# jandrewrfarrell/RUFUS

Hardware: AMD Instinct MI355X
Metric: reads/sec through k-mer count+filter at k=25 (higher is better)
Workload: dtype u64; 1 GPU; synthetic 30x WGS trio (BASELINE configs[2]): genome 3100000000 bp, 620000000/620000000/620000000 x 150 bp reads per sample, on each of 1 GPU(s) 19 resident blocks of the subject (92 GB of packed reads in HBM, generated on the device in 0.5 s), 1000 SNVs, seed 12345, k=25, -s 8G -L 2, MinCov 5, MaxHashDepth 1200, MinQ 15, thresh 1; 2 minimizer-shard pass(es) per step (per-shard (pos,key)-sorted re; parallelism=read-block shard x1, mutant_kmers=24567, pulled_pairs=11560, passes=2, hbm_total=309220868096, hbm_free_at_start=308400881664, resident_read_bytes=92219805240, read_blocks=compact, run_map_budget_bytes=39836680704, checked=False, hbm_mapped_bytes=271656681472

## Files before the change

include/rufus_hip.h:

```cpp
#ifndef RUFUS_HIP_H
#define RUFUS_HIP_H

#include <stddef.h>
#include <stdint.h>

#ifdef __cplusplus
extern "C" {
#endif

#define RFX_OK 0
#define RFX_E_NODEVICE (-1)
#define RFX_E_INVAL (-2)
#define RFX_E_NOMEM (-3)
#define RFX_E_FULL (-4)
#define RFX_E_HIP (-5)
#define RFX_E_MIXEDCASE (-6)
#define RFX_E_RANGE (-7)
#define RFX_E_FORMAT (-8)

#define RFX_HISTO_BINS 10002

typedef struct rfx_ctx rfx_ctx;
typedef struct rfx_reads rfx_reads;
typedef struct rfx_table rfx_table;
// ... 106 lines not shown
#define RFX_COUNT_MSP 3
int rfx_count_set_mode(rfx_table*, int mode);
int rfx_count_set_shard(rfx_table*, int shard, int n_shards);
int rfx_count_set_early(rfx_table*, int on);
int rfx_count_early_segments(const rfx_table*);
int rfx_count_adopt_early(rfx_table* next_shard, rfx_table* from);
typedef struct rfx_runmaps rfx_runmaps;
rfx_runmaps* rfx_runmaps_create(rfx_ctx*, uint64_t budget_bytes);
rfx_runmaps* rfx_runmaps_create_pooled(rfx_ctx*, uint64_t pool_bytes);
void rfx_runmaps_free(rfx_runmaps*);
uint64_t rfx_runmaps_bytes(const rfx_runmaps*);
int rfx_runmaps_blocks(const rfx_runmaps*);
int rfx_runmaps_drop(rfx_runmaps*, const rfx_reads*);
int rfx_runmaps_clear(rfx_runmaps*);
int rfx_count_set_runmaps(rfx_table*, rfx_runmaps*);
int rfx_count_prepare_maps(rfx_table*, rfx_reads* const* blocks, int n);
int rfx_count_prefetch_maps(rfx_table*, rfx_reads* const* blocks, int n);
uint64_t rfx_count_replayed(const rfx_table*);
int rfx_count_set_passes(rfx_table*, int passes);
int rfx_count_add(rfx_table*, const rfx_reads*);
typedef struct rfx_peers rfx_peers;
int rfx_ctx_allow_peers(rfx_ctx*, const int* devices, int n);
rfx_peers* rfx_peers_create(int n);
void rfx_peers_free(rfx_peers*);
int rfx_count_set_peers(rfx_table*, rfx_peers*, int index);
int rfx_count_add_pairs_dev(rfx_table*, const uint64_t* d_keys, const uint32_t* d_counts, uint64_t n);
int rfx_count_stats(rfx_table*, uint64_t* distinct, uint64_t* capacity, uint64_t* max_displacement);

int rfx_count_segments(rfx_table*);
int rfx_count_segment_get(rfx_table*, int i, const uint64_t** d_records, const uint64_t** d_bin_start, uint32_t* bins,
                          uint64_t* n_records);
int rfx_count_add_records_dev(rfx_table*, const uint64_t* d_records, uint64_t n_records, const uint64_t* d_bin_start,
                              uint32_t bins);
int rfx_count_adopt_records_dev(rfx_table*, const uint64_t* d_records, const uint32_t* d_ext, uint64_t n_records,
                                const uint64_t* d_bin_start, uint32_t bins);
int rfx_count_segment_ext(rfx_table*, int i, const uint32_t** d_ext);
int rfx_count_add_records_ext_dev(rfx_table*, const uint64_t* d_records, const uint32_t* d_ext, uint64_t n_records,
                                  const uint64_t* d_bin_start, uint32_t bins);
void rfx_count_free(rfx_table*);

rfx_records* rfx_count_finish(rfx_table*, uint64_t lower, uint64_t upper, uint64_t* histo );
typedef struct rfx_finish rfx_finish;
rfx_finish* rfx_count_finish_begin(rfx_table*, uint64_t lower, uint64_t upper, uint64_t* histo );
rfx_records* rfx_count_finish_end(rfx_finish*);

uint64_t rfx_records_size(const rfx_records*);
int rfx_records_k(const rfx_records*);
int rfx_records_lsize(const rfx_records*);
int rfx_records_payload(const rfx_records*, void* out, size_t cap_bytes, int counter_len);
int rfx_records_payload_range(const rfx_records*, uint64_t first, uint64_t n, void* out, size_t cap_bytes,
                              int counter_len);
int rfx_records_get(const rfx_records*, uint64_t* keys, uint32_t* counts, uint64_t* pos);
rfx_records* rfx_records_load(rfx_ctx*, int k, int lsize, const uint64_t* cols, const void* payload, uint64_t n,
                              int counter_len);
rfx_records* rfx_records_load_fd(rfx_ctx*, int k, int lsize, const uint64_t* cols, int fd, uint64_t offset, uint64_t n,
                                 int counter_len);
rfx_records* rfx_records_from_dev(rfx_ctx*, int k, int lsize, const uint64_t* cols, const uint64_t* d_keys,
                                  const uint32_t* d_counts, uint64_t n);
const uint64_t* rfx_records_dev_keys(const rfx_records*);
const uint32_t* rfx_records_dev_counts(const rfx_records*);
const uint64_t* rfx_records_dev_pos(const rfx_records*);
int rfx_records_histo(const rfx_records*, uint64_t* histo );
int rfx_records_verify(const rfx_records*, uint32_t min_count, uint32_t max_count, uint64_t out[4]);
int rfx_records_checksum(const rfx_records*, uint64_t out[2]);
void rfx_records_free(rfx_records*);

int rfx_merge_unique(rfx_ctx*, const rfx_records* const* files, int n_files, uint32_t min_count, uint64_t* keys_out,
                     uint32_t* counts_out, uint64_t cap, uint64_t* n_out);
int rfx_query(const rfx_records* db, const uint64_t* keys, uint64_t n, uint32_t* counts_out);
int rfx_unique_to_subject(rfx_ctx*, const rfx_records* subject, const rfx_records* const* others, int n_others,
                          uint32_t min_count, uint32_t min_cov, uint32_t max_cov, uint64_t* keys_out,
                          uint32_t* counts_out, uint64_t cap, uint64_t* n_out);
rfx_records* rfx_records_subtract(rfx_ctx*, const rfx_records* a, const rfx_records* const* others, int n_others,
                                  uint32_t min_count, uint32_t max_count);

typedef struct rfx_binned rfx_binned;
typedef struct rfx_candidates rfx_candidates;
rfx_binned* rfx_count_finish_binned(rfx_table*, uint64_t lower, uint64_t upper, uint64_t* histo );
uint64_t rfx_binned_size(const rfx_binned*);
int rfx_binned_bits(const rfx_binned*);
void rfx_binned_free(rfx_binned*);
rfx_candidates* rfx_binned_strike(rfx_ctx*, rfx_binned* subject, const rfx_binned* control, uint32_t min_count,
                                  uint32_t max_count);
int rfx_candidates_strike(rfx_candidates*, const rfx_binned* control);
uint64_t rfx_candidates_size(const rfx_candidates*);
int rfx_candidates_get(const rfx_candidates*, uint64_t* keys_out);
int rfx_candidates_get_counts(const rfx_candidates*, uint32_t* counts_out);
int rfx_candidates_strike_records(rfx_candidates*, const rfx_records* exclude);
void rfx_candidates_free(rfx_candidates*);
int rfx_binned_get(const rfx_binned*, uint64_t* keys_out, uint32_t* counts_out, uint32_t* bins_out, uint64_t* at_out,
                   uint64_t cap, uint64_t* n_out);
int rfx_binned_checksum(const rfx_binned*, uint64_t out[2]);
int rfx_binned_verify(const rfx_binned*, uint64_t lower, uint64_t upper, uint64_t out[5]);
int rfx_binned_query(const rfx_binned*, const uint64_t* canonical_keys, uint64_t n, uint32_t* counts_out);
const uint64_t* rfx_binned_dev_keys(const rfx_binned*);
const uint32_t* rfx_binned_dev_counts(const rfx_binned*);

rfx_set* rfx_set_build(rfx_ctx*, const uint64_t* fwd_keys, uint64_t n, int k);
uint64_t rfx_set_size(const rfx_set*);
void rfx_set_free(rfx_set*);
int rfx_filter(rfx_set*, const rfx_reads*, int thresh, int last_base_skipped, uint32_t* hits_out,
               uint64_t* hitmask_out, uint64_t* n_hit_reads);
int rfx_filter_many(rfx_set*, const rfx_reads* const* blocks, int n, int thresh, int last_base_skipped,
                    uint64_t* const* hitmask_out, uint64_t* n_hit_reads);

#define RFX_SELECT_READS 0
#define RFX_SELECT_PAIRS 1
rfx_reads* rfx_reads_select(rfx_ctx*, const rfx_reads* src, const uint64_t* hitmask , int mode);
int rfx_reads_origin(const rfx_reads*, uint32_t* block_out, uint32_t* read_out);
rfx_reads* rfx_filter_pull(rfx_set*, const rfx_reads* const* blocks, int n, int thresh, int last_base_skipped, int mode,
                           uint64_t* const* hitmask_out, uint64_t* n_hit_reads);

typedef struct rfx_model_params {
  double sc, stdev, factor, skew, power;
} rfx_model_params;
int rfx_model_residuals(rfx_ctx*, const int64_t* histo, uint32_t n, const rfx_model_params* cand, int n_cand,
                        int log_resid, int inflection, int max_copy, double* resid_out);
int rfx_model_tables(rfx_ctx*, uint32_t n, const rfx_model_params* model, uint32_t* n_cols, double* dist,
                     size_t dist_cap, double* rowtot);

#define RFX_OVL_SAM 0
#define RFX_OVL_CONTIG 1
#define RFX_OVL_REGION 2
int rfx_overlap_score(rfx_ctx*, const char* a, int alen, const char* const* b, const int* blen, int nb, float min_pct,
                      int min_ovl, int variant, int* out );
typedef struct rfx_ovl_pool rfx_ovl_pool;
rfx_ovl_pool* rfx_ovl_pool_create(rfx_ctx*, const char* const* seqs, const int* lens, int n);
int rfx_ovl_pool_set(rfx_ovl_pool*, int idx, const char* seq, int len);
int rfx_ovl_pool_score(rfx_ovl_pool*, int query, const char* a_explicit, int a_len, const int* cand, int nb,
                       float min_pct, int min_ovl, int variant, int strands, int* out);
void rfx_ovl_pool_free(rfx_ovl_pool*);
int rfx_annotate(rfx_set*, const rfx_reads*, uint32_t* cov_out);

#ifdef __cplusplus
}
#endif
#endif
```

profiles/summarize_pmc.py:

```python
#!/usr/bin/env python3
import collections
import csv
import json
import re
import sys


NOT_CHAIN = frozenset((
    "k_synth_reads", "k_copy16",
    "k_flag_absent", "k_flag_absent_tiled", "k_fa_bounds", "k_flag_gather", "k_flag_range", "k_flag_rank", "k_flag_present",
    "k_compact_count", "k_compact_scatter", "k_scan_u64", "k_query", "k_strike_bins", "k_strike_cands",
    "k_strike_query", "k_binned_sizes", "k_binned_scan", "k_binned_gather", "k_binned_checksum", "k_binned_verify", "k_binned_query",
    "k_filter", "k_filter_q", "k_filter_p", "k_filter_fast", "k_filter_big", "k_hits_mask", "k_mask_count", "k_set_bitmap",
    "k_set_bitmap_big", "k_set_bitmap_q", "k_set_bitmap_p",
    "k_set_insert", "k_set_bitmap_packed", "k_records_checksum", "k_records_verify", "k_check_sorted",
    "k_parse_records", "k_format_records", "k_txt_count", "k_txt_lines", "k_txt_reads", "k_txt_pack", "k_txt_nth", "k_bgzf_inflate", "k_reads_tile_count", "k_reads_tile_table", "k_reads_tile", "k_select_words", "k_select_table", "k_select_copy", "k_gather_sizes", "k_gather_table", "k_gather_copy", "k_compute_pos", "k_annotate", "k_overlap_pool", "k_overlap_score",
    "k_model_colsum", "k_model_dist", "k_model_rowtot", "k_model_sum", "k_model_terms", "k_model_weights",
))
CHAIN_KNOWN = frozenset((
    "k_msp_part1", "k_msp_replay", "k_msp_count", "k_col_sums", "k_bin_group_sums", "k_bin_offsets", "k_scan_tail", "k_scan_sums",
    "k_scan_apply", "k_part2", "k_flag_if_gt", "k_slice_tag", "k_bin_hist", "k_bin_hist_stamp", "k_bin_hist_multi", "k_msp_leaf",
    "k_surv_place", "k_surv_hist", "k_surv_sort", "k_histo_bins", "k_histo_staged", "k_bin_count", "k_part1", "k_leaf", "k_leaf_compact", "k_bin_scatter",
    "k_tmp_start", "k_split_bins", "k_coarse_counts", "k_histo", "k_count_reads", "k_count_pairs", "k_table_pairs", "k_tile_count",
    "k_tile_scan", "k_tile_emit",
))


def kname(s):
    m = re.search(r"(k_[a-z0-9_]+|__amd_rocclr_[A-Za-z]+)", s)
    return m.group(1) if m else s[:40]


def load(path, counter):
    agg = collections.defaultdict(lambda: [0, 0.0])
    for r in csv.DictReader(open(path)):
        if r["Counter_Name"] == counter:
            a = agg[kname(r["Kernel_Name"])]
            a[0] += 1
            a[1] += float(r["Counter_Value"])
    return {k: (n, v / n) for k, (n, v) in agg.items()}


def main():
    f, w = load(sys.argv[1], "FETCH_SIZE"), load(sys.argv[2], "WRITE_SIZE")
    out = {}
    for k in sorted(set(f) | set(w)):
        fn, fv = f.get(k, (0, 0.0))
        wn, wv = w.get(k, (0, 0.0))
        out[k] = {"launches": max(fn, wn), "FETCH_SIZE_KB_avg": round(fv, 1), "WRITE_SIZE_KB_avg": round(wv, 1),
                  "hbm_bytes_per_launch": int((2 * fv + wv) * 1024)}
    chain = [k for k in sorted(out) if k.startswith("k_") and k not in NOT_CHAIN]
    samples = int(sys.argv[4]) if len(sys.argv) > 4 else max(
        out.get("k_msp_part1", {}).get("launches", 0), out.get("k_part1", {}).get("launches", 0),
        out.get("k_bin_scatter", {}).get("launches", 0))
    if samples:
        tot = sum(out[k]["hbm_bytes_per_launch"] * out[k]["launches"] for k in chain if k in out)
        out["_chain"] = {"kernels": [k for k in chain if k in out], "samples": samples,
                         "hbm_bytes_per_sample": int(tot / samples),
                         "source": "rocprofv3 --pmc FETCH_SIZE / WRITE_SIZE (separate passes), (2*FETCH+WRITE)*1024, all "
                                   "launches of the count chain of the profiled bench command / sample chains"}
        if len(sys.argv) > 5:
            out["genome"] = int(sys.argv[5])
    import os
    sys.path.insert(0, os.path.dirname(os.path.dirname(os.path.abspath(__file__))))
    import bench
    out["kernel_sources_sha16"] = bench.kernel_source_fingerprint()
    out["commit"] = os.environ.get("RFX_COMMIT", "unknown (set RFX_COMMIT=$(git rev-parse HEAD) when profiling)")
    json.dump(out, open(sys.argv[3], "w"), indent=1, sort_keys=True)
    if "_chain" in out:
        print(f"count chain: {out['_chain']['hbm_bytes_per_sample'] / 1e6:.1f} MB per sample over {samples} samples")
    for k, v in sorted(((k, v) for k, v in out.items() if isinstance(v, dict) and "launches" in v), key=lambda kv: -kv[1]["hbm_bytes_per_launch"]):
        print(f"{k:26s} {v['launches']:4d} {v['FETCH_SIZE_KB_avg']:14.1f} {v['WRITE_SIZE_KB_avg']:14.1f} "
              f"{v['hbm_bytes_per_launch'] / 1e6:10.1f} MB")


if __name__ == "__main__":
    main()
```

rufus_amd/capi.py:

```python
from __future__ import annotations

import ctypes as C
import os
import sys

import numpy as np

_HERE = os.path.dirname(os.path.abspath(__file__))
LIB_PATH = os.environ.get("RFX_LIB") or os.path.join(_HERE, "librufus_hip.so")

HISTO_BINS = 10002
PACK_COUNT, PACK_FILTER = 1, 2
COUNT_AUTO, COUNT_TABLE, COUNT_P2L, COUNT_MSP = 0, 1, 2, 3
E_FULL, E_RANGE, E_MIXEDCASE = -4, -7, -6
E_INVAL, E_FORMAT = -2, -8
SELECT_READS, SELECT_PAIRS = 0, 1

u8p, u32p, u64p = C.POINTER(C.c_uint8), C.POINTER(C.c_uint32), C.POINTER(C.c_uint64)

SIGNATURES = {
    "rfx_version": (C.c_char_p, []),
    "rfx_strerror": (C.c_char_p, [C.c_int]),
    "rfx_last_error": (C.c_char_p, []),
    "rfx_jf_matrix": (C.c_int, [C.c_int, C.c_int, u64p]),
    "rfx_jf_pos": (C.c_uint64, [u64p, C.c_int, C.c_int, C.c_uint64]),
    "rfx_pack_words": (C.c_uint64, [u64p, C.c_uint32]),
    "rfx_pack_reads": (C.c_int, [C.c_char_p, C.c_char_p, u64p, C.c_uint32, C.c_int, C.c_int, u64p, u32p, u32p, u32p,
                                 u32p]),
    "rfx_pack_spans": (C.c_int, [C.c_void_p, u64p, u32p, u64p, C.c_uint32, C.c_int, C.c_int, u64p, u32p, u32p, u32p, u32p]),
    "rfx_hashlist_keys": (C.c_long, [C.c_char_p, C.c_size_t, C.c_int, C.c_int, u64p, C.c_size_t]),
    "rfx_jhash_header": (C.c_long, [C.c_int, C.c_int, u64p, C.c_int, C.c_int, C.c_int, C.POINTER(C.c_char_p),
                                    C.c_char_p, C.c_size_t]),
    "rfx_open": (C.c_void_p, [C.c_int, C.c_size_t]),
    "rfx_close": (None, [C.c_void_p]),
    "rfx_sync": (C.c_int, [C.c_void_p]),
    "rfx_host_alloc": (C.c_void_p, [C.c_size_t]),
    "rfx_host_alloc_lazy": (C.c_void_p, [C.c_size_t]),
    "rfx_host_pin": (C.c_int, [C.c_void_p]),
    "rfx_host_cpus": (C.c_uint, []),
    "rfx_host_free": (None, [C.c_void_p]),
    "rfx_stream": (C.c_void_p, [C.c_void_p]),
    "rfx_mem_stats": (C.c_int, [C.c_void_p, u64p, u64p, u64p]),
    "rfx_memcpy_dev": (C.c_int, [C.c_void_p, C.c_void_p, C.c_void_p, C.c_size_t]),
    "rfx_prof_enable": (C.c_int, [C.c_void_p, C.c_int]),
    "rfx_prof_filter": (C.c_int, [C.c_void_p, C.c_char_p]),
    "rfx_prof_reset": (C.c_int, [C.c_void_p]),
    "rfx_prof_query": (C.c_int, [C.c_void_p, C.c_char_p, C.POINTER(C.c_double), u64p]),
    "rfx_prof_names": (C.c_int, [C.c_void_p, C.c_char_p, C.c_size_t]),
    "rfx_reads_device_bytes": (C.c_uint64, [C.c_void_p]),
    "rfx_records_subtract": (C.c_void_p, [C.c_void_p, C.c_void_p, C.POINTER(C.c_void_p), C.c_int, C.c_uint32, C.c_uint32]),
    "rfx_count_finish_binned": (C.c_void_p, [C.c_void_p, C.c_uint64, C.c_uint64, u64p]),
    "rfx_binned_size": (C.c_uint64, [C.c_void_p]),
    "rfx_binned_bits": (C.c_int, [C.c_void_p]),
    "rfx_binned_free": (None, [C.c_void_p]),
    "rfx_binned_strike": (C.c_void_p, [C.c_void_p, C.c_void_p, C.c_void_p, C.c_uint32, C.c_uint32]),
    "rfx_candidates_strike": (C.c_int, [C.c_void_p, C.c_void_p]),
    "rfx_candidates_size": (C.c_uint64, [C.c_void_p]),
    "rfx_candidates_get": (C.c_int, [C.c_void_p, u64p]),
    "rfx_candidates_free": (None, [C.c_void_p]),
    "rfx_candidates_get_counts": (C.c_int, [C.c_void_p, u32p]),
    "rfx_candidates_strike_records": (C.c_int, [C.c_void_p, C.c_void_p]),
    "rfx_binned_get": (C.c_int, [C.c_void_p, u64p, u32p, u32p, u64p, C.c_uint64, u64p]),
    "rfx_binned_checksum": (C.c_int, [C.c_void_p, u64p]),
    "rfx_binned_verify": (C.c_int, [C.c_void_p, C.c_uint64, C.c_uint64, u64p]),
    "rfx_binned_query": (C.c_int, [C.c_void_p, u64p, C.c_uint64, u32p]),
    "rfx_binned_dev_keys": (C.c_void_p, [C.c_void_p]),
    "rfx_binned_dev_counts": (C.c_void_p, [C.c_void_p]),
    "rfx_reads_upload": (C.c_void_p, [C.c_void_p, u64p, u32p, u32p, u32p, u32p, C.c_uint32]),
    "rfx_reads_free": (None, [C.c_void_p]),
    "rfx_reads_count": (C.c_uint32, [C.c_void_p]),
    "rfx_reads_bases": (C.c_uint64, [C.c_void_p]),
    "rfx_reads_words": (C.c_uint64, [C.c_void_p]),
    "rfx_reads_get": (C.c_int, [C.c_void_p, u64p, u32p, u32p, u32p, u32p]),
    "rfx_tile_plan": (C.c_int, [C.c_uint64, C.c_int, C.c_uint32, u64p, u32p]),
    "rfx_reads_tile": (C.c_void_p, [C.c_void_p, C.c_void_p, C.c_int, C.c_uint32]),
    "rfx_reads_select": (C.c_void_p, [C.c_void_p, C.c_void_p, u64p, C.c_int]),
    "rfx_reads_origin": (C.c_int, [C.c_void_p, u32p, u32p]),
    "rfx_filter_pull": (C.c_void_p, [C.c_void_p, C.POINTER(C.c_void_p), C.c_int, C.c_int, C.c_int, C.c_int, C.POINTER(u64p), u64p]),
    "rfx_synth_reads": (C.c_void_p, [C.c_void_p, C.c_void_p, C.c_uint64, C.c_uint32, C.c_int, C.c_int]),
    "rfx_text_open": (C.c_void_p, [C.c_void_p, C.c_uint64]),
    "rfx_text_close": (None, [C.c_void_p]),
    "rfx_text_room": (C.c_uint64, [C.c_void_p]),
    "rfx_text_bytes": (C.c_uint64, [C.c_void_p]),
    "rfx_text_append": (C.c_long, [C.c_void_p, C.c_char_p, C.c_uint64]),
    "rfx_text_copied": (C.c_int, [C.c_void_p, C.c_long]),
    "rfx_text_wait": (C.c_int, [C.c_void_p, C.c_long]),
    "rfx_text_parse": (C.c_void_p, [C.c_void_p, C.c_int, C.c_int, C.POINTER(C.c_int)]),
    "rfx_text_fetch": (C.c_int, [C.c_void_p, C.c_char_p]),
    "rfx_text_reset": (None, [C.c_void_p]),
    "rfx_bgzf_scan": (C.c_int, [C.c_char_p, C.c_uint64, C.c_uint32, u32p, u64p, u64p]),
    "rfx_text_append_bgzf": (C.c_long, [C.c_void_p, C.c_char_p, C.c_uint64]),
    "rfx_text_settle": (C.c_int, [C.c_void_p, C.c_void_p, u64p]),
    "rfx_text_records": (C.c_int, [C.c_void_p, u64p]),
    "rfx_text_settle_records": (C.c_int, [C.c_void_p, C.c_void_p, C.c_uint64, u64p, u64p]),
    "rfx_text_gather": (C.c_int, [C.c_void_p, u64p, C.c_uint64, C.c_void_p, C.c_uint64, u64p, u64p]),
    "rfx_reads_of_length": (C.c_uint64, [C.c_void_p, C.c_uint32]),
    "rfx_synth_text": (C.c_int, [C.c_void_p, C.c_uint64, C.c_uint32, C.c_void_p, C.c_void_p]),
    "rfx_synth_snv": (C.c_int, [C.c_void_p, C.c_uint32, u64p, C.c_char_p, C.c_char_p]),
    "rfx_synth_genome": (C.c_int, [C.c_void_p, C.c_uint64, C.c_uint64, C.c_void_p]),
    "rfx_count_begin": (C.c_void_p, [C.c_void_p, C.c_int, C.c_int, C.c_int, C.c_uint64, C.c_uint64, C.c_uint64]),
    "rfx_count_set_mode": (C.c_int, [C.c_void_p, C.c_int]),
    "rfx_count_set_passes": (C.c_int, [C.c_void_p, C.c_int]),
    "rfx_count_add": (C.c_int, [C.c_void_p, C.c_void_p]),
    "rfx_count_add_pairs_dev": (C.c_int, [C.c_void_p, C.c_void_p, C.c_void_p, C.c_uint64]),
    "rfx_count_stats": (C.c_int, [C.c_void_p, u64p, u64p, u64p]),
    "rfx_count_finish_begin": (C.c_void_p, [C.c_void_p, C.c_uint64, C.c_uint64, u64p]),
    "rfx_count_finish_end": (C.c_void_p, [C.c_void_p]),
    "rfx_count_set_shard": (C.c_int, [C.c_void_p, C.c_int, C.c_int]),
    "rfx_count_set_early": (C.c_int, [C.c_void_p, C.c_int]),
    "rfx_count_early_segments": (C.c_int, [C.c_void_p]),
    "rfx_count_adopt_early": (C.c_int, [C.c_void_p, C.c_void_p]),
    "rfx_mem_reserve": (C.c_int, [C.c_void_p, C.c_uint64]),
    "rfx_runmaps_create": (C.c_void_p, [C.c_void_p, C.c_uint64]),
    "rfx_runmaps_create_pooled": (C.c_void_p, [C.c_void_p, C.c_uint64]),
    "rfx_runmaps_free": (None, [C.c_void_p]),
    "rfx_runmaps_bytes": (C.c_uint64, [C.c_void_p]),
    "rfx_runmaps_blocks": (C.c_int, [C.c_void_p]),
    "rfx_runmaps_drop": (C.c_int, [C.c_void_p, C.c_void_p]),
    "rfx_runmaps_clear": (C.c_int, [C.c_void_p]),
    "rfx_count_set_runmaps": (C.c_int, [C.c_void_p, C.c_void_p]),
    "rfx_count_prepare_maps": (C.c_int, [C.c_void_p, C.POINTER(C.c_void_p), C.c_int]),
    "rfx_count_prefetch_maps": (C.c_int, [C.c_void_p, C.POINTER(C.c_void_p), C.c_int]),
    "rfx_count_replayed": (C.c_uint64, [C.c_void_p]),
    "rfx_count_segments": (C.c_int, [C.c_void_p]),
    "rfx_count_segment_get": (C.c_int, [C.c_void_p, C.c_int, C.POINTER(C.c_void_p), C.POINTER(C.c_void_p),
                                        C.POINTER(C.c_uint32), u64p]),
    "rfx_count_add_records_dev": (C.c_int, [C.c_void_p, C.c_void_p, C.c_uint64, C.c_void_p, C.c_uint32]),
    "rfx_count_segment_ext": (C.c_int, [C.c_void_p, C.c_int, C.POINTER(C.c_void_p)]),
    "rfx_count_add_records_ext_dev": (C.c_int, [C.c_void_p, C.c_void_p, C.c_void_p, C.c_uint64, C.c_void_p, C.c_uint32]),
    "rfx_count_free": (None, [C.c_void_p]),
    "rfx_count_finish": (C.c_void_p, [C.c_void_p, C.c_uint64, C.c_uint64, u64p]),
    "rfx_records_size": (C.c_uint64, [C.c_void_p]),
    "rfx_records_k": (C.c_int, [C.c_void_p]),
    "rfx_records_lsize": (C.c_int, [C.c_void_p]),
    "rfx_records_payload": (C.c_int, [C.c_void_p, C.c_void_p, C.c_size_t, C.c_int]),
    "rfx_records_payload_range": (C.c_int, [C.c_void_p, C.c_uint64, C.c_uint64, C.c_void_p, C.c_size_t, C.c_int]),
    "rfx_records_get": (C.c_int, [C.c_void_p, u64p, u32p, u64p]),
    "rfx_records_load": (C.c_void_p, [C.c_void_p, C.c_int, C.c_int, u64p, C.c_void_p, C.c_uint64, C.c_int]),
# ... 120 lines not shown
                   carrier=1 if which == 0 else 0)

    def text(self, first_pair: int, n_pairs: int):
        seq = np.zeros((2 * n_pairs, self.read_len), dtype=np.uint8)
        qual = np.zeros_like(seq)
        _check(lib().rfx_synth_text(C.byref(self), first_pair, n_pairs, seq.ctypes.data, qual.ctypes.data),
               "rfx_synth_text")
        return seq, qual

    def snvs(self):
        out = []
        for i in range(self.n_snv):
            pos, ref, alt = C.c_uint64(0), C.create_string_buffer(1), C.create_string_buffer(1)
            _check(lib().rfx_synth_snv(C.byref(self), i, C.byref(pos), ref, alt), "rfx_synth_snv")
            out.append((pos.value, ref.raw, alt.raw))
        return out

    def genome(self, first: int, n: int) -> bytes:
        buf = np.zeros(max(n, 1), dtype=np.uint8)
        _check(lib().rfx_synth_genome(C.byref(self), first, n, buf.ctypes.data), "rfx_synth_genome")
        return buf[:n].tobytes()


def tile_plan(length: int, k: int, tile_len: int = 150):
    if length < 0 or not 0 <= tile_len < 2**32:
        raise RufusError(f"rfx_tile_plan: {lib().rfx_strerror(E_INVAL).decode()} (code {E_INVAL})")
    nt, step = C.c_uint64(0), C.c_uint32(0)
    _check(lib().rfx_tile_plan(length, k, tile_len, C.byref(nt), C.byref(step)), "rfx_tile_plan")
    return int(nt.value), int(step.value)


def bgzf_scan(data: bytes, max_blocks: int = 0xFFFFFFFF):
    nb, used, inf = C.c_uint32(0), C.c_uint64(0), C.c_uint64(0)
    _check(lib().rfx_bgzf_scan(data, len(data), max_blocks, C.byref(nb), C.byref(used), C.byref(inf)), "rfx_bgzf_scan")
    return int(nb.value), int(used.value), int(inf.value)


class PackedReads:

    def __init__(self, seq: bytes, off: np.ndarray, qual: bytes | None = None, min_q: int = 0,
                 flags: int = PACK_COUNT):
        off = np.ascontiguousarray(off, dtype=np.uint64)
        n = len(off) - 1
        L = lib()
        nw = int(L.rfx_pack_words(_p(off, u64p), n))
        self.n = n
        self.codes = np.zeros(max(nw, 1), dtype=np.uint64)
        self.acgt = np.zeros(max(nw, 1), dtype=np.uint32) if flags & PACK_COUNT else None
        self.good = np.zeros(max(nw, 1), dtype=np.uint32) if flags & PACK_FILTER else None
        self.word_off = np.zeros(n + 1, dtype=np.uint32)
        self.len = np.zeros(max(n, 1), dtype=np.uint32)
        _check(L.rfx_pack_reads(seq, qual, _p(off, u64p), n, min_q, flags, _p(self.codes, u64p), _p(self.acgt, u32p),
                                _p(self.good, u32p), _p(self.word_off, u32p), _p(self.len, u32p)), "rfx_pack_reads")

    @classmethod
    def from_reads(cls, seqs, quals=None, min_q: int = 0, flags: int = PACK_COUNT):
        lens = np.fromiter((len(s) for s in seqs), dtype=np.uint64, count=len(seqs))
        off = np.zeros(len(seqs) + 1, dtype=np.uint64)
        np.cumsum(lens, out=off[1:])
        q = None
        if quals is not None:
            q = b"".join((qq + b"\0" * (len(s) - len(qq)))[:len(s)] for s, qq in zip(seqs, quals))
        return cls(b"".join(seqs), off, q, min_q, flags)


class Context:
    def __init__(self, device: int = 0, hbm_budget: int = 0):
        self._h = lib().rfx_open(device, hbm_budget)
        if not self._h:
            raise RufusError("rfx_open failed (no CPU fallback): " + lib().rfx_last_error().decode())

    def close(self):
        if self._h:
            self._pin_arr = None
            for p in getattr(self, "_pin_ptrs", ()):
                lib().rfx_host_free(p)
            self._pin_ptrs = []
            lib().rfx_close(self._h)
            self._h = None

    def sync(self):
        _check(lib().rfx_sync(self._h), "rfx_sync")

    def mem_stats(self) -> dict:
        u, pk, m = C.c_uint64(0), C.c_uint64(0), C.c_uint64(0)
        _check(lib().rfx_mem_stats(self._h, C.byref(u), C.byref(pk), C.byref(m)), "rfx_mem_stats")
        return {"used": u.value, "peak": pk.value, "mapped": m.value}

    def memcpy_dev(self, dst: int, src: int, nbytes: int):
        _check(lib().rfx_memcpy_dev(self._h, dst, src, nbytes), "rfx_memcpy_dev")

    def prof(self, on: bool):
        _check(lib().rfx_prof_enable(self._h, int(on)), "rfx_prof_enable")

    def prof_filter(self, names=()):
        _check(lib().rfx_prof_filter(self._h, ",".join(names).encode()), "rfx_prof_filter")

    def prof_reset(self):
        _check(lib().rfx_prof_reset(self._h), "rfx_prof_reset")

    def prof_dict(self) -> dict:
        buf = C.create_string_buffer(8192)
        _check(lib().rfx_prof_names(self._h, buf, len(buf)), "rfx_prof_names")
        out = {}
        for name in buf.value.decode().split("\n"):
            if not name:
                continue
            ms, n = C.c_double(0), C.c_uint64(0)
            _check(lib().rfx_prof_query(self._h, name.encode(), C.byref(ms), C.byref(n)), "rfx_prof_query")
            out[name] = (ms.value, n.value)
        return out

    def upload(self, p: PackedReads) -> "ReadBlock":
        return ReadBlock(self, p)

    def synth_reads(self, sy: Synth, first_pair: int, n_pairs: int, min_q: int = 15, want_good: bool = True,
                    compact: bool = False):
        h = lib().rfx_synth_reads(self._h, C.byref(sy), first_pair, n_pairs, min_q, int(want_good) | (2 if compact else 0))
        if not h:
            raise RufusError("rfx_synth_reads failed: " + lib().rfx_last_error().decode())
        return ReadBlock.from_handle(self, h)

    def pinned_u64(self, n_words: int) -> np.ndarray:
        have = getattr(self, "_pin_arr", None)
        if have is None or len(have) < n_words:
            p = lib().rfx_host_alloc(max(n_words, 1) * 8)
            if not p:
                raise RufusError("rfx_host_alloc failed")
            self._pin_ptrs = getattr(self, "_pin_ptrs", []) + [p]
            self._pin_arr = np.ctypeslib.as_array((C.c_uint64 * max(n_words, 1)).from_address(p))
        return self._pin_arr[:max(n_words, 1)]

    def __enter__(self):
        return self

    def __exit__(self, *a):
        self.close()


class TextArena:

    def __init__(self, ctx: Context, cap_bytes: int):
        self.ctx = ctx
        self._h = lib().rfx_text_open(ctx._h, cap_bytes)
        if not self._h:
            raise RufusError("rfx_text_open failed: " + lib().rfx_last_error().decode())

    def append(self, data: bytes) -> int:
        t = lib().rfx_text_append(self._h, data, len(data))
        if t < 0:
            _check(int(t), "rfx_text_append")
        _check(lib().rfx_text_wait(self._h, t), "rfx_text_wait")
        return int(t)

    def append_bgzf(self, data: bytes) -> int:
        t = lib().rfx_text_append_bgzf(self._h, data, len(data))
        if t < 0:
            _check(int(t), "rfx_text_append_bgzf")
        _check(lib().rfx_text_wait(self._h, t), "rfx_text_wait")
        return int(t)

    def settle(self, next: "TextArena | None" = None) -> int:
        carried = C.c_uint64(0)
        _check(lib().rfx_text_settle(self._h, next._h if next is not None else None, C.byref(carried)), "rfx_text_settle")
        return int(carried.value)

# ... 254 lines not shown
        _check(lib().rfx_count_set_passes(self._h, passes), "rfx_count_set_passes")

    def set_peers(self, peers: int, index: int):
        _check(lib().rfx_count_set_peers(self._h, peers, index), "rfx_count_set_peers")

    def set_shard(self, shard: int, n_shards: int):
        _check(lib().rfx_count_set_shard(self._h, shard, n_shards), "rfx_count_set_shard")

    def set_early(self, on: bool = True):
        _check(lib().rfx_count_set_early(self._h, int(on)), "rfx_count_set_early")

    def early_segments(self) -> int:
        return int(lib().rfx_count_early_segments(self._h))

    def adopt_early(self, other: "CountTable"):
        _check(lib().rfx_count_adopt_early(self._h, other._h), "rfx_count_adopt_early")

    def set_runmaps(self, store: "RunMaps"):
        _check(lib().rfx_count_set_runmaps(self._h, store._h if store is not None else None), "rfx_count_set_runmaps")

    def prepare_maps(self, blocks) -> None:
        arr = (C.c_void_p * max(1, len(blocks)))(*[b._h for b in blocks])
        _check(lib().rfx_count_prepare_maps(self._h, arr, len(blocks)), "rfx_count_prepare_maps")

    def prefetch_maps(self, blocks) -> int:
        arr = (C.c_void_p * max(1, len(blocks)))(*[b._h for b in blocks])
        n = int(lib().rfx_count_prefetch_maps(self._h, arr, len(blocks)))
        if n < 0:
            _check(n, "rfx_count_prefetch_maps")
        return n

    def replayed(self) -> int:
        return int(lib().rfx_count_replayed(self._h))

    def segments(self):
        n = lib().rfx_count_segments(self._h)
        if n < 0:
            _check(n, "rfx_count_segments")
        out = []
        for i in range(n):
            dr, db, bins, nr = C.c_void_p(0), C.c_void_p(0), C.c_uint32(0), C.c_uint64(0)
            _check(lib().rfx_count_segment_get(self._h, i, C.byref(dr), C.byref(db), C.byref(bins), C.byref(nr)),
                   "rfx_count_segment_get")
            out.append((dr.value or 0, db.value or 0, bins.value, nr.value))
        return out

    def n_segments(self) -> int:
        n = lib().rfx_count_segments(self._h)
        if n < 0:
            _check(n, "rfx_count_segments")
        return n

    def segment(self, i: int):
        dr, db, bins, nr = C.c_void_p(0), C.c_void_p(0), C.c_uint32(0), C.c_uint64(0)
        _check(lib().rfx_count_segment_get(self._h, i, C.byref(dr), C.byref(db), C.byref(bins), C.byref(nr)),
               "rfx_count_segment_get")
        return (dr.value or 0, db.value or 0, bins.value, nr.value)

    def add_records_dev(self, d_records: int, n_records: int, d_bin_start: int, bins: int, d_ext: int = 0):
        _check(lib().rfx_count_add_records_ext_dev(self._h, d_records, d_ext or None, n_records, d_bin_start, bins),
               "rfx_count_add_records_dev")

    def adopt_records_dev(self, d_records: int, n_records: int, d_bin_start: int, bins: int, d_ext: int = 0):
        _check(lib().rfx_count_adopt_records_dev(self._h, d_records, d_ext or None, n_records, d_bin_start, bins),
               "rfx_count_adopt_records_dev")

    def segment_ext(self, i: int) -> int:
        p = C.c_void_p(0)
        _check(lib().rfx_count_segment_ext(self._h, i, C.byref(p)), "rfx_count_segment_ext")
        return p.value or 0

    def stats(self):
        d, c, m = C.c_uint64(0), C.c_uint64(0), C.c_uint64(0)
        _check(lib().rfx_count_stats(self._h, C.byref(d), C.byref(c), C.byref(m)), "rfx_count_stats")
        return {"distinct": d.value, "capacity": c.value, "max_displacement": m.value}

    def finish(self, lower: int = 0, upper: int = 2**64 - 1, want_histo: bool = False):
        h = np.zeros(HISTO_BINS, dtype=np.uint64) if want_histo else None
        rec = Records(self.ctx, lib().rfx_count_finish(self._h, lower, upper, _p(h, u64p)))
        return (rec, h) if want_histo else rec

    def finish_binned(self, lower: int = 0, upper: int = 2**64 - 1, want_histo: bool = False):
        h = np.zeros(HISTO_BINS, dtype=np.uint64) if want_histo else None
        b = Binned(self.ctx, lib().rfx_count_finish_binned(self._h, lower, upper, _p(h, u64p)))
        return (b, h) if want_histo else b

    def finish_begin(self, lower: int = 0, upper: int = 2**64 - 1, want_histo: bool = False):
        h = np.zeros(HISTO_BINS, dtype=np.uint64) if want_histo else None
        return (lib().rfx_count_finish_begin(self._h, lower, upper, _p(h, u64p)), h)

    def finish_end(self, handle):
        f, h = handle
        rec = Records(self.ctx, lib().rfx_count_finish_end(f))
        return (rec, h) if h is not None else rec

    def free(self):
        if self._h:
            lib().rfx_count_free(self._h)
            self._h = None


def merge_unique(ctx: Context, files, min_count: int = 5):
    arr = (C.c_void_p * len(files))(*[f._h for f in files])
    n = C.c_uint64(0)
    rc = lib().rfx_merge_unique(ctx._h, arr, len(files), min_count, None, None, 0, C.byref(n))
    if rc not in (0, E_RANGE):
        _check(rc, "rfx_merge_unique")
    keys, counts = np.zeros(max(n.value, 1), np.uint64), np.zeros(max(n.value, 1), np.uint32)
    _check(lib().rfx_merge_unique(ctx._h, arr, len(files), min_count, _p(keys, u64p), _p(counts, u32p), len(keys),
                                  C.byref(n)), "rfx_merge_unique")
    return keys[:n.value], counts[:n.value]


_uniq_buf = {}


def unique_to_subject(ctx: Context, subject: Records, others, min_cov: int, max_cov: int, min_count: int = 5):
    arr = (C.c_void_p * max(1, len(others)))(*[f._h for f in others])
    cap = _uniq_buf.get("cap", 1 << 16)
    while True:
        if _uniq_buf.get("cap") != cap or "k" not in _uniq_buf:
            _uniq_buf.update(cap=cap, k=np.zeros(cap, np.uint64), c=np.zeros(cap, np.uint32))
        keys, counts = _uniq_buf["k"], _uniq_buf["c"]
        n = C.c_uint64(0)
        rc = lib().rfx_unique_to_subject(ctx._h, subject._h, arr, len(others), min_count, min_cov, max_cov,
                                         _p(keys, u64p), _p(counts, u32p), cap, C.byref(n))
        if rc == E_RANGE and n.value > cap:
            cap = int(n.value)
            continue
        _check(rc, "rfx_unique_to_subject")
        return keys[:n.value].copy(), counts[:n.value].copy()


def records_subtract(ctx: Context, a: Records, others, min_count: int = 0, max_count: int = 0xFFFFFFFF) -> Records:
    arr = (C.c_void_p * max(1, len(others)))(*[f._h for f in others])
    return Records(ctx, lib().rfx_records_subtract(ctx._h, a._h, arr, len(others), min_count, max_count))


class Binned:

    def __init__(self, ctx: Context, handle):
        if not handle:
            raise RufusError("binned records: " + lib().rfx_last_error().decode())
        self.ctx, self._h = ctx, handle

    def __len__(self):
        return int(lib().rfx_binned_size(self._h))

    @property
    def bits(self):
        return lib().rfx_binned_bits(self._h)

    def _live(self):
        if not self._h:
            raise RufusError("binned records: freed")
        return self._h

    def get(self):
        h = self._live()
        n = len(self)
        keys, counts = np.zeros(n, np.uint64), np.zeros(n, np.uint32)
        bins, at = np.zeros(n, np.uint32), np.zeros(n, np.uint64)
        got = C.c_uint64(0)
        _check(lib().rfx_binned_get(h, _p(keys, u64p), _p(counts, u32p), _p(bins, u32p), _p(at, u64p), n, C.byref(got)),
               "rfx_binned_get")
        if got.value != n:
            raise RufusError(f"rfx_binned_get: {got.value} survivors in the bins, {n} counted by the finish")
        return keys, counts, bins, at

    def checksum(self) -> tuple:
        o = np.zeros(2, dtype=np.uint64)
        _check(lib().rfx_binned_checksum(self._live(), _p(o, u64p)), "rfx_binned_checksum")
        return int(o[0]), int(o[1])

    def verify(self, lower: int = 0, upper: int = 2**64 - 1) -> dict:
        if not 0 <= lower <= upper < 2**64:
            raise ValueError("verify: 0 <= lower <= upper < 2^64")
        o = np.zeros(5, dtype=np.uint64)
        _check(lib().rfx_binned_verify(self._live(), lower, upper, _p(o, u64p)), "rfx_binned_verify")
        return {"bad_bin": int(o[0]), "bad_count": int(o[1]), "not_canonical": int(o[2]), "duplicate": int(o[3]),
                "sum_counts": int(o[4])}

    def query(self, keys: np.ndarray) -> np.ndarray:
        keys = np.ascontiguousarray(keys, dtype=np.uint64)
        if keys.ndim != 1:
            raise ValueError("query: a flat array of keys")
        out = np.zeros(len(keys), dtype=np.uint32)
        _check(lib().rfx_binned_query(self._live(), _p(keys, u64p), len(keys), _p(out, u32p)), "rfx_binned_query")
        return out

    def dev_ptrs(self):
        L = lib()
        return L.rfx_binned_dev_keys(self._live()), L.rfx_binned_dev_counts(self._live())

    def free(self):
        if self._h:
            lib().rfx_binned_free(self._h)
            self._h = None


class Candidates:

    def __init__(self, ctx: Context, handle):
        if not handle:
            raise RufusError("candidates: " + lib().rfx_last_error().decode())
        self.ctx, self._h = ctx, handle

    def __len__(self):
        return int(lib().rfx_candidates_size(self._h))

    def strike(self, control: Binned):
        _check(lib().rfx_candidates_strike(self._h, control._h), "rfx_candidates_strike")

    def strike_records(self, records: "Records"):
        if not isinstance(records, Records) or not records._h:
            raise TypeError("strike_records: a live capi.Records")
        _check(lib().rfx_candidates_strike_records(self._h, records._h), "rfx_candidates_strike_records")

    def _raw_keys(self) -> np.ndarray:
        k = np.zeros(len(self), np.uint64)
        _check(lib().rfx_candidates_get(self._h, _p(k, u64p)), "rfx_candidates_get")
        return k

    def keys(self) -> np.ndarray:
        k = self._raw_keys()
        return k[k != np.uint64(0xFFFFFFFFFFFFFFFF)]

    def counts(self, raw_keys=None) -> np.ndarray:
        c = np.zeros(len(self), np.uint32)
        _check(lib().rfx_candidates_get_counts(self._h, _p(c, u32p)), "rfx_candidates_get_counts")
        k = self._raw_keys() if raw_keys is None else raw_keys
        return c[k != np.uint64(0xFFFFFFFFFFFFFFFF)]

    def keys_counts(self):
        k = self._raw_keys()
        return k[k != np.uint64(0xFFFFFFFFFFFFFFFF)], self.counts(k)

    def free(self):
        if self._h:
            lib().rfx_candidates_free(self._h)
            self._h = None


def binned_strike(ctx: Context, subject: Binned, control, min_count: int = 0, max_count: int = 0xFFFFFFFF) -> Candidates:
    return Candidates(ctx, lib().rfx_binned_strike(ctx._h, subject._h, control._h if control is not None else None,
                                                   min_count, max_count))


OVL_SAM, OVL_CONTIG, OVL_REGION = 0, 1, 2


def overlap_score(ctx: Context, a: bytes, cands, min_pct: float, min_ovl: int, variant: int = OVL_SAM) -> np.ndarray:
    nb = len(cands)
    arr = (C.c_char_p * max(nb, 1))(*cands)
    lens = (C.c_int * max(nb, 1))(*[len(x) for x in cands])
    out = np.zeros((max(nb, 1), 5), dtype=np.int32)
    _check(lib().rfx_overlap_score(ctx._h, a, len(a), arr, lens, nb, min_pct, min_ovl, variant,
                                   out.ctypes.data_as(C.POINTER(C.c_int))), "rfx_overlap_score")
    return out[:nb]


def model_residuals(ctx: Context, histo, cands, log_resid: bool, inflection: int, max_copy: int = 5) -> np.ndarray:
    histo = np.ascontiguousarray(histo, dtype=np.int64)
    cands = np.ascontiguousarray(cands, dtype=np.float64).reshape(-1, 5)
    out = np.zeros(len(cands), dtype=np.float64)
    _check(lib().rfx_model_residuals(ctx._h, _p(histo, C.POINTER(C.c_int64)), len(histo), cands.ctypes.data, len(cands),
                                     int(bool(log_resid)), inflection, max_copy, _p(out, C.POINTER(C.c_double))),
           "rfx_model_residuals")
    return out


def model_tables(ctx: Context, n: int, model):
    model = np.ascontiguousarray(model, dtype=np.float64).reshape(5)
    cols = C.c_uint32(0)
    rc = lib().rfx_model_tables(ctx._h, n, model.ctypes.data, C.byref(cols), None, 0, None)
    if rc != -7:
        _check(rc, "rfx_model_tables")
    dist = np.zeros((n, cols.value + 1), dtype=np.float64)
    rowtot = np.zeros(n, dtype=np.float64)
    _check(lib().rfx_model_tables(ctx._h, n, model.ctypes.data, C.byref(cols), _p(dist, C.POINTER(C.c_double)), dist.size,
# ... 62 lines not shown
```

rufus_amd/csrc/rfx_api.hip:

```cpp
#include <algorithm>
#include <condition_variable>
#include <mutex>
#include <cstdio>
#include <cstdlib>
#include <cstring>
#include <sys/mman.h>

#include <atomic>
#include <cerrno>
#include <chrono>
#include <queue>
#include <thread>
#include <vector>

#include <unistd.h>

#include "rfx_internal.h"

namespace {

thread_local char g_err[512] = "";

int hip_fail(hipError_t e, const char* what) {
  snprintf(g_err, sizeof g_err, "%s: %s", what, hipGetErrorString(e));
// ... 1641 lines not shown
  }
  rfxk::bin_totals(c, cnt, rows, P, bin_start);
  rfxk::part2(c, (const uint64_t*)buf_a0, inst, bin_start, fine_cur, P2, 32 - g.bin_bits, cur, (uint32_t)cap_a, nullptr, ext, cap_b,
              "k_part2", nullptr, 0, cap_b, g.rec_mode, t->k);
  rfxk::flag_if_gt(c, bin_start + P, cap_b, cur + g.ncur);
  drop();
  t->segs->push_back(rfx_segment{inst, cap_b, bin_start, (uint64_t)((double)g.windows * share) + 1, P, ext});
  t->seg_kind = RFX_COUNT_MSP;
  if (t->pend->empty()) c->pend_tables.push_back(t);
  t->pend->push_back(rfx_pending_add{r, cur, t->segs->size() - 1, g.ncur});
  return RFX_OK;
}

static int msp_settle(rfx_table* t, const std::vector<unsigned int>& flags) {
  rfx_ctx* c = t->ctx;
  int rc = RFX_OK;
  for (size_t i = 0; i < t->pend->size() && rc == RFX_OK; ++i) {
    if (!flags[i]) continue;
    const rfx_pending_add& p = (*t->pend)[i];
    rfx_segment& sg = (*t->segs)[p.seg];
    if (!sg.borrowed) dfree(c, sg.inst);
    dfree(c, sg.bin_start);
    if (!sg.borrowed) dfree(c, sg.ext);
    sg.inst = sg.bin_start = nullptr;
    sg.ext = nullptr;
    rfx_segment fresh{};
    rc = msp_partition_exact(t, p.r, &fresh);
    if (rc == RFX_OK) sg = fresh;
  }
  msp_forget_pending(t);
  return rc;
}

static int msp_resolve(rfx_table* t) {
  rfx_ctx* c = t->ctx;
  if (t->pend->empty()) return RFX_OK;
  std::vector<unsigned int> flags(t->pend->size(), 1u);
  for (size_t i = 0; i < t->pend->size(); ++i)
    if (queue_read(c, &flags[i], (*t->pend)[i].cur + (*t->pend)[i].ncur, 4) != hipSuccess) return RFX_E_HIP;
  if (ctx_sync(c) != hipSuccess) return RFX_E_HIP;
  return msp_settle(t, flags);
}

static void rfx_reads_release_pending(const rfx_reads* r) {
  rfx_ctx* c = r->ctx;
  std::vector<rfx_table*> hit;
  for (rfx_table* t : c->pend_tables)
    for (auto& p : *t->pend)
      if (p.r == r) {
        hit.push_back(t);
        break;
      }
  for (rfx_table* t : hit) {
    const int rc = msp_resolve(t);
    if (rc) t->pend_error = rc;
  }
}

constexpr size_t RFX_CUR_TAIL = 3;

struct rfx_finish {
  rfx_table* t = nullptr;
  uint32_t stage_extra = 0;
  uint64_t lower = 0, upper = 0;
  uint64_t* histo = nullptr;
  rfx_records* ready = nullptr;
  bool failed = false;
  bool queued = false;
  uint64_t cap = 0, room = 0, kmers = 0, total_out = 0;
  const uint64_t** d_inst = nullptr;
  uint64_t *aw = nullptr, *bw = nullptr, *bsq = nullptr, *bs1 = nullptr;
  uint32_t *ac = nullptr, *bc = nullptr;
  bool segs_dropped = false;
  uint32_t cb_lo = 0;
  rfx_records* big = nullptr;
  std::vector<const uint64_t*> h_ptrs;
  std::vector<uint32_t> h_cur;
  std::vector<unsigned int> pflags;
  bool binned = false;
  rfxk::msp_stage bstage;
  uint2* bin_at = nullptr;
  uint32_t bin_lo = 0, bin_hi = 0;
  int bin_bits = 0;
};

static uint64_t msp_surv_key(uint64_t lower, uint64_t kmers) { return (kmers >> 24) | ((uint64_t)(lower >= 2 ? 1 : 0) << 62); }
static double msp_surv_guess(rfx_ctx* c, uint64_t lower, uint64_t kmers, double margin = 1.3) {
  double seen = c->msp_surv_frac[lower >= 2 ? 1 : 0];
  if (kmers >= (1ull << 28)) {
    auto it = c->msp_surv_by_size.find(msp_surv_key(lower, kmers));
    if (it != c->msp_surv_by_size.end()) seen = it->second;
  }
  double frac = seen > 0 ? seen * margin : (lower >= 2 ? (kmers > (1ull << 32) ? 0.08 : 0.25) : 0.6);
  if (const char* ev = getenv("RFX_MSP_SURV_FRAC")) frac = atof(ev);
  return frac;
}

static int leaf_stage_alloc(rfx_ctx* c, uint32_t chunk, uint32_t n_chunks, uint32_t launches, rfxk::msp_stage* st,
                            bool binned = false) {
  const size_t n_fill = (size_t)n_chunks * (binned ? 2 : 1);
  st->chunk = chunk;
  st->n_chunks = n_chunks;
  st->keys = (uint64_t*)dmalloc(c, (size_t)n_chunks * chunk * 8);
  st->counts = (uint32_t*)dmalloc(c, (size_t)n_chunks * chunk * 4);
  st->fill = (uint32_t*)dmalloc(c, (n_fill + launches) * 4);
  st->more = st->fill ? st->fill + n_fill : nullptr;
  if (!st->keys || !st->counts || !st->fill) return RFX_E_NOMEM;
  HIPCHK(hipMemsetAsync(st->fill, 0, (n_fill + launches) * 4, c->stream));
  return RFX_OK;
}
static void leaf_stage_free(rfx_ctx* c, rfxk::msp_stage* st) {
  dfree(c, st->keys); dfree(c, st->counts); dfree(c, st->fill);
  *st = rfxk::msp_stage{};
}

static void msp_emit_drop(rfx_finish* f) {
  rfx_ctx* c = f->t->ctx;
  dfree(c, f->d_inst); dfree(c, f->aw); dfree(c, f->ac); dfree(c, f->bw); dfree(c, f->bc); dfree(c, f->bsq);
  dfree(c, f->bs1);
  f->d_inst = nullptr;
  f->aw = f->bw = f->bsq = f->bs1 = nullptr;
  f->ac = f->bc = nullptr;
  f->queued = false;
}

static int msp_leaf_refined(rfx_finish* f, int to_bits, const std::vector<std::vector<uint64_t>>& h_bs, int sel_bits,
                            uint32_t* cur, size_t ncur) {
  rfx_table* t = f->t;
  rfx_ctx* c = t->ctx;
  const int rec_mode = t->canonical ? 1 : 2;
  struct group {
    uint32_t b = 0;
    int from_bits = 0, f1bits = 0, f2bits = 0;
    std::vector<size_t> segs;
    uint64_t *cb1 = nullptr, *cb2 = nullptr, *fine1 = nullptr, *fine2 = nullptr;
    uint32_t *ce1 = nullptr, *ce2 = nullptr;
    uint64_t max_chunk = 0;
    const uint64_t** d_seg = nullptr;
  };
  const bool wide = rfxk::msp_wide(t->k);
  std::map<uint32_t, group> groups;
  uint64_t kmers = 0;
  for (size_t i = 0; i < t->segs->size(); ++i) {
    group& g = groups[(*t->segs)[i].bins];
    g.b = (*t->segs)[i].bins;
    g.segs.push_back(i);
    kmers += (*t->segs)[i].kmers;
  }
  const uint32_t bmin = groups.begin()->first;
  const uint32_t Ftot = (1u << to_bits) / bmin;
  for (auto& kv : groups) {
    group& g = kv.second;
    g.from_bits = ceil_log2(g.b);
    const int fbits = to_bits - g.from_bits;
    if (fbits > 16) {
      snprintf(g_err, sizeof g_err, "MSP: partition would need %d more bits", fbits);
      return RFX_E_FULL;
    }
    g.f1bits = std::min(8, fbits);
    g.f2bits = fbits - g.f1bits;
  }
  std::vector<uint64_t> sz(bmin, 0);
  uint64_t R = 0;
  for (auto& kv : groups)
    for (size_t si : kv.second.segs) {
      const uint32_t r = kv.second.b / bmin;
// ... 22 lines not shown
    for (auto& kv : groups) {
      dfree(c, kv.second.cb1); dfree(c, kv.second.cb2); dfree(c, kv.second.fine1); dfree(c, kv.second.fine2);
      dfree(c, kv.second.ce1); dfree(c, kv.second.ce2); dfree(c, kv.second.d_seg);
    }
  };
  size_t nleaf = 0;
  for (auto& kv : groups) {
    group& g = kv.second;
    if (g.f1bits == 0) {
      nleaf += g.segs.size();
      continue;
    }
    ++nleaf;
    const uint32_t r = g.b / bmin;
    for (size_t ci = 0; ci + 1 < cut.size(); ++ci) {
      uint64_t ch = 0;
      for (size_t si : g.segs) ch += h_bs[si][(size_t)cut[ci + 1] * r] - h_bs[si][(size_t)cut[ci] * r];
      g.max_chunk = std::max(g.max_chunk, ch);
    }
    const size_t n1max = (size_t)max_np * r << g.f1bits, n2max = (size_t)max_np * Ftot;
    g.cb1 = (uint64_t*)dmalloc(c, std::max<uint64_t>(g.max_chunk, 1) * 8);
    g.fine1 = (uint64_t*)dmalloc(c, (n1max + 1) * 8 + n1max * 4);
    if (wide) g.ce1 = (uint32_t*)dmalloc(c, std::max<uint64_t>(g.max_chunk, 1) * 4);
    if (g.f2bits) {
      g.cb2 = (uint64_t*)dmalloc(c, std::max<uint64_t>(g.max_chunk, 1) * 8);
      g.fine2 = (uint64_t*)dmalloc(c, (n2max + 1) * 8 + n2max * 4);
      if (wide) g.ce2 = (uint32_t*)dmalloc(c, std::max<uint64_t>(g.max_chunk, 1) * 4);
    }
    if (!g.cb1 || !g.fine1 || (g.f2bits && (!g.cb2 || !g.fine2)) || (wide && (!g.ce1 || (g.f2bits && !g.ce2)))) {
      drop();
      return RFX_E_NOMEM;
    }
    if (g.segs.size() > 1 && g.segs.size() <= (size_t)rfxk::part2_max_segs && !getenv("RFX_PART3_PER_SEG")) {
      const size_t ns = g.segs.size();
      std::vector<const uint64_t*> hp(3 * ns, nullptr);
      for (size_t x = 0; x < ns; ++x) {
        const rfx_segment& sg = (*t->segs)[g.segs[x]];
        hp[x] = sg.inst;
        hp[ns + x] = sg.bin_start;
        hp[2 * ns + x] = (const uint64_t*)sg.ext;
      }
      g.d_seg = (const uint64_t**)dmalloc(c, 3 * ns * sizeof(void*));
      if (!g.d_seg) { drop(); return RFX_E_NOMEM; }
      const hipError_t e = upload(c, g.d_seg, hp.data(), 3 * ns * sizeof(void*));
      if (e != hipSuccess) { drop(); return hip_fail(e, "msp_leaf_refined"); }
    }
  }
  const uint64_t** d_ptrs = (const uint64_t**)dmalloc(c, 3 * nleaf * sizeof(void*) * (cut.size() - 1));
  if (!d_ptrs) { drop(); return RFX_E_NOMEM; }
  int geo = (kmers * (uint64_t)(t->n_shards > 1 ? t->n_shards : 1)) >> to_bits <= 12288 ? 1 : 0;
  if (const char* ev = getenv("RFX_MSP_GEO")) geo = atoi(ev) != 0;
  uint64_t max_chunk_all = 0;
  for (size_t ci = 0; ci + 1 < cut.size(); ++ci) {
    uint64_t ch = 0;
    for (auto& kv : groups)
      for (size_t si : kv.second.segs)
        ch += h_bs[si][(size_t)cut[ci + 1] * (kv.second.b / bmin)] - h_bs[si][(size_t)cut[ci] * (kv.second.b / bmin)];
    max_chunk_all = std::max(max_chunk_all, ch);
  }
  uint32_t lgrid = 1, lchunk = 1, lpool = 1;
  const uint64_t est_surv = R ? (uint64_t)((double)kmers * msp_surv_guess(c, f->lower, kmers) * (double)max_chunk_all / (double)R) : 0;
  rfxk::msp_leaf_plan(c, (uint32_t)std::min<size_t>((size_t)max_np * Ftot, 1u << 30), geo, max_chunk_all, est_surv, f->stage_extra,
                      &lgrid, &lchunk, &lpool);
  if (f->binned) {
    lchunk = rfxk::msp_leaf_chunk_kept(lchunk);
    const uint64_t est_all = (uint64_t)((double)kmers * msp_surv_guess(c, f->lower, kmers, 1.12));
    uint64_t more = est_all / rfxk::msp_leaf_chunk_room(geo, lchunk) + 16 + f->stage_extra;
    if (getenv("RFX_LEAF_STAGE_TEST")) more = f->stage_extra;
    lpool = (uint32_t)std::min<uint64_t>((uint64_t)lgrid + more, 1u << 30);
    f->bin_bits = to_bits;
    f->bin_lo = p_first * Ftot;
    f->bin_hi = p_end * Ftot;
    const size_t at_bytes = ((size_t)(f->bin_hi - f->bin_lo) + lgrid) * 2 * sizeof(uint2);
    f->bin_at = (uint2*)dmalloc(c, at_bytes);
    if (!f->bin_at) { drop(); dfree(c, d_ptrs); return RFX_E_NOMEM; }
    HIPCHK(hipMemsetAsync(f->bin_at, 0xFF, at_bytes, c->stream));
  }
  rfxk::msp_stage stage;
  {
    const int src = leaf_stage_alloc(c, lchunk, lpool, f->binned ? 1 : (uint32_t)cut.size(), &stage, f->binned);
    if (src) { drop(); dfree(c, d_ptrs); leaf_stage_free(c, &stage); return src; }
  }
  if (f->binned) f->bstage = stage;
  for (size_t ci = 0; ci + 1 < cut.size(); ++ci) {
    const uint32_t p0 = cut[ci], np = cut[ci + 1] - cut[ci];
    const size_t n2 = (size_t)np * Ftot;
    std::vector<const uint64_t*> ptrs(3 * nleaf, nullptr);
    size_t li = 0;
    uint64_t chunk_all = 0;
    for (auto& kv : groups) {
      group& g = kv.second;
      const uint32_t r = g.b / bmin, gp0 = p0 * r, gnp = np * r;
      if (g.f1bits == 0) {
        for (size_t si : g.segs) {
          ptrs[li] = (*t->segs)[si].inst;
          ptrs[nleaf + li] = (*t->segs)[si].bin_start + gp0;
          ptrs[2 * nleaf + li] = (const uint64_t*)(*t->segs)[si].ext;
          ++li;
          chunk_all += h_bs[si][(size_t)gp0 + gnp] - h_bs[si][gp0];
        }
        continue;
      }
      uint64_t chunk = 0;
      for (size_t si : g.segs) chunk += h_bs[si][(size_t)gp0 + gnp] - h_bs[si][gp0];
      chunk_all += chunk;
      const uint32_t F1 = 1u << g.f1bits, F2 = 1u << g.f2bits;
      const int shift1 = 32 - (g.from_bits + g.f1bits), shift2 = 32 - to_bits;
      const size_t n1 = (size_t)gnp * F1;
      uint32_t* fcur1 = (uint32_t*)(g.fine1 + n1 + 1);
      HIPCHK(hipMemsetAsync(g.fine1, 0, (n1 + 1) * 8 + n1 * 4, c->stream));
      if (chunk) {
        if (g.d_seg) {
          const size_t ns = g.segs.size();
          bool planes = true;
          for (size_t si : g.segs) planes = planes && (*t->segs)[si].ext != nullptr;
          rfxk::bin_hist_multi(c, g.d_seg, g.d_seg + ns, planes ? (const uint32_t* const*)(g.d_seg + 2 * ns) : nullptr, (int)ns, gp0,
                               gnp, chunk, F1, shift1, rec_mode, t->k, g.fine1);
        } else {
          for (size_t si : g.segs)
            rfxk::bin_hist(c, (*t->segs)[si].inst, (*t->segs)[si].bin_start + gp0, gnp, chunk, F1, shift1, rec_mode, t->k,
                           g.fine1, (*t->segs)[si].ext);
        }
        rfxk::scan_tail(c, g.fine1, n1);
        if (g.d_seg) {
          const size_t ns = g.segs.size();
          rfxk::part2_multi(c, g.d_seg, g.d_seg + ns, wide ? (const uint32_t* const*)(g.d_seg + 2 * ns) : nullptr, (int)ns,
                            gp0, gnp, chunk, g.cb1, g.fine1, fcur1, F1, shift1, g.ce1, rec_mode, t->k, "k_part3");
        } else {
          for (size_t si : g.segs)
            rfxk::part2(c, (*t->segs)[si].inst, g.cb1, g.fine1, fcur1, F1, shift1, nullptr, 0, (*t->segs)[si].ext, g.ce1,
                        ~0ull, "k_part3", (*t->segs)[si].bin_start + gp0, gnp, 0, rec_mode, t->k);
        }
      }
      const uint64_t *leaf_src = g.cb1, *leaf_bs = g.fine1;
      const uint32_t* leaf_ext = g.ce1;
      if (g.f2bits) {
        uint32_t* fcur2 = (uint32_t*)(g.fine2 + n2 + 1);
        HIPCHK(hipMemsetAsync(g.fine2, 0, (n2 + 1) * 8 + n2 * 4, c->stream));
        if (chunk) {
          rfxk::bin_hist(c, g.cb1, g.fine1, (uint32_t)n1, chunk, F2, shift2, rec_mode, t->k, g.fine2, g.ce1);
          rfxk::scan_tail(c, g.fine2, n2);
          rfxk::part2(c, g.cb1, g.cb2, g.fine2, fcur2, F2, shift2, nullptr, 0, g.ce1, g.ce2, ~0ull, "k_part4", g.fine1,
                      (uint32_t)n1, 0, rec_mode, t->k);
        }
        leaf_src = g.cb2;
        leaf_bs = g.fine2;
        leaf_ext = g.ce2;
      }
      ptrs[li] = leaf_src;
      ptrs[nleaf + li] = leaf_bs;
      ptrs[2 * nleaf + li] = (const uint64_t*)leaf_ext;
      ++li;
    }
    if (!chunk_all) continue;
    const uint64_t** d = d_ptrs + 3 * nleaf * ci;
    const hipError_t e = upload(c, d, ptrs.data(), 3 * nleaf * sizeof(void*));
    if (e != hipSuccess) {
      drop();
      dfree(c, d_ptrs);
      if (!f->binned) leaf_stage_free(c, &stage);
      return hip_fail(e, "msp_leaf_refined");
    }
    rfxk::msp_leaf(c, d, d + nleaf, (int)nleaf, ptrs[0], ptrs[nleaf], (uint32_t)n2, t->k, t->canonical, t->lut_t, t->ntab,
                   sel_bits, 2 * t->k - 7, t->pos_lo, t->pos_hi, f->lower, f->upper, f->aw, f->ac, cur, (uint32_t)f->cap,
                   cur + ncur, cur + ncur + 1, cur + ncur + 2, geo, (const uint32_t* const*)(d + 2 * nleaf),
                   (const uint32_t*)ptrs[2 * nleaf], stage, (uint32_t)ci, std::min<uint32_t>(lgrid, (uint32_t)n2),
                   f->binned ? f->bin_at + 2 * ((size_t)p0 * Ftot - f->bin_lo) : nullptr);
  }
  if (getenv("RFX_STAGE_DEBUG")) {
    std::vector<uint32_t> more(cut.size(), 0);
    if (ctx_sync(c) == hipSuccess && hipMemcpy(more.data(), stage.more, cut.size() * 4, hipMemcpyDeviceToHost) == hipSuccess) {
      uint64_t tot = 0;
      for (uint32_t m : more) tot += m;
      fprintf(stderr, "[rfx stage] geo %d grid %u chunk %u pool %u launches %zu: extra chunks taken %llu (first launch %u), est survivors per launch %llu\n",
              geo, lgrid, lchunk, lpool, cut.size() - 1, (unsigned long long)tot, more[0], (unsigned long long)est_surv);
    }
  }
  drop();
  dfree(c, d_ptrs);
  if (!f->binned) leaf_stage_free(c, &stage);
  return RFX_OK;
}

static int msp_prepare_leaf(rfx_table* t, int* to_bits_out, bool* refine_out, std::vector<std::vector<uint64_t>>& h_bs,
                            uint64_t* kmers_out, bool force_refine) {
  rfx_ctx* c = t->ctx;
  uint64_t kmers = 0;
  uint32_t pmax = 0, pmin = ~0u;
  for (auto& sg : *t->segs) {
    kmers += sg.kmers;
    pmax = std::max(pmax, sg.bins);
    pmin = std::min(pmin, sg.bins);
  }
  int to_bits = ceil_log2(pmax);
  const uint64_t kfull = kmers * (uint64_t)(t->n_shards > 1 ? t->n_shards : 1);
  const uint64_t per_bin = 24576;
  while (to_bits < 28 && (kfull >> to_bits) > per_bin) ++to_bits;
  if (!getenv("RFX_MSP_NO_HALF") && pmin < (1u << to_bits) && to_bits < 28) {
    const int lo = ceil_log2(pmin), hi = ceil_log2(pmax);
    auto levels = [](int d) { return d <= 0 ? 0 : (d + 7) / 8; };
    if (levels(to_bits + 1 - lo) == levels(to_bits - lo) && levels(to_bits + 1 - hi) == std::max(levels(to_bits - hi), 1))
      ++to_bits;
  }
  if (getenv("RFX_MSP_REFINE_BITS")) to_bits = std::max(to_bits, atoi(getenv("RFX_MSP_REFINE_BITS")));
  const bool refine = force_refine || pmin < (1u << to_bits);
  h_bs.clear();
  if (refine) {
    int rc = msp_resolve(t);
    if (rc) return rc;
    h_bs.resize(t->segs->size());
    for (size_t i = 0; i < t->segs->size(); ++i) {
      const rfx_segment& sg = (*t->segs)[i];
      h_bs[i].assign((size_t)sg.bins + 1, 0);
      HIPCHK(hipMemcpyAsync(h_bs[i].data(), sg.bin_start, ((size_t)sg.bins + 1) * 8, hipMemcpyDeviceToHost, c->stream));
    }
    HIPCHK(ctx_sync(c));
  }
  *to_bits_out = to_bits;
  *refine_out = refine;
  *kmers_out = kmers;
  return RFX_OK;
}

static int msp_add(rfx_table* t, const rfx_reads* r);

struct rfx_peers {
  int n = 0;
  bool sharded = true;
  std::mutex mu;
  std::condition_variable cv;
  int arrived = 0;
  uint64_t gen = 0;
  bool failed = false;
  struct Seg {
    const uint64_t* inst = nullptr;
    const uint32_t* ext = nullptr;
    uint32_t bins = 0;
    uint64_t kmers = 0;
    std::vector<uint64_t> bs;
  };
  struct Slot {
    int device = 0;
    const uint64_t* aw = nullptr;
    const uint32_t* ac = nullptr;
    uint64_t cap = 0;
    std::vector<uint32_t> fill;
    int passes = 0;
    std::vector<Seg> segs;
  };
  std::vector<Slot> slot;
  bool barrier() {
    std::unique_lock<std::mutex> g(mu);
    if (failed) return false;
    const uint64_t my = gen;
    if (++arrived == n) {
      arrived = 0;
      ++gen;
      cv.notify_all();
      return true;
    }
    cv.wait(g, [&] { return gen != my || failed; });
    return gen != my;
// ... 575 lines not shown
  f->big = nullptr;
  if (e != hipSuccess) { hip_fail(e, "msp_emit"); rfx_records_free(big); return RFX_E_HIP; }
  bool redo = false;
  for (unsigned int x : f->pflags) redo |= x != 0;
  if (!t->pend->empty() && f->pflags.size() == t->pend->size()) {
    const int rc = msp_settle(t, f->pflags);
    if (rc) { rfx_records_free(big); return rc; }
  }
  if (redo) {
    rfx_records_free(big);
    return 1;
  }
  if (f->h_cur[ncur + 1]) {
    snprintf(g_err, sizeof g_err, "MSP: a bin could not be split far enough to fit LDS");
    rfx_records_free(big);
    return RFX_E_FULL;
  }
  if (f->h_cur[ncur]) {
    const uint64_t had = f->cap;
    f->cap = 1;
    for (uint32_t cb = 0; cb < P1; ++cb)
      f->cap = std::max<uint64_t>(f->cap, f->h_cur[(size_t)cb * rfxk::p1_cur_stride()]);
    if (const uint32_t short_by = f->h_cur[ncur + 2]) {
      f->stage_extra += short_by + short_by / 4 + 64;
      f->cap = std::max(f->cap, had);
    }
    rfx_records_free(big);
    return 1;
  }
  const uint64_t total_out = f->total_out;
  big->n = total_out;
  if (f->kmers) {
    c->msp_surv_frac[f->lower >= 2 ? 1 : 0] = (double)total_out / (double)f->kmers;
    if (c->msp_surv_by_size.size() > 256) c->msp_surv_by_size.clear();
    c->msp_surv_by_size[msp_surv_key(f->lower, f->kmers)] = (double)total_out / (double)f->kmers;
  }
  if ((f->room - total_out) * 20 > (2ull << 30)) {
    rfx_records* fit = records_alloc(c, t->k, t->lsize, t->cols, total_out);
    if (fit) {
      hipError_t e2 = rfxk::copy_bytes(c, fit->keys, big->keys, total_out * 8);
      if (e2 == hipSuccess) e2 = rfxk::copy_bytes(c, fit->counts, big->counts, total_out * 4);
      if (e2 == hipSuccess) e2 = rfxk::copy_bytes(c, fit->pos, big->pos, total_out * 8);
      if (e2 == hipSuccess) {
        rfx_records_free(big);
        big = fit;
      } else {
        rfx_records_free(fit);
      }
    }
  }
  *out = big;
  return 0;
}

static rfx_records* msp_emit_finish(rfx_finish* f) {
  rfx_records* rec = nullptr;
  for (int attempt = 0; attempt < 4; ++attempt) {
    if (!f->queued && msp_emit_queue(f) != RFX_OK) return nullptr;
    const int rc = msp_emit_collect(f, &rec);
    if (rc == 0) return rec;
    if (rc < 0) return nullptr;
  }
  snprintf(g_err, sizeof g_err, "MSP: emit did not converge (internal error)");
  return nullptr;
}

static rfx_records* msp_emit(rfx_table* t, uint64_t lower, uint64_t upper, uint64_t* histo) {
  rfx_finish f;
  f.t = t;
  f.lower = lower;
  f.upper = upper;
  f.histo = histo;
  return msp_emit_finish(&f);
}

struct rfx_binned {
  rfx_ctx* ctx = nullptr;
  int k = 0, canonical = 1;
  rfxk::msp_stage st;
  uint2* bin_at = nullptr;
  uint32_t bin_lo = 0, bin_hi = 0;
  int bits = 0;
  uint64_t n = 0;
};
struct rfx_candidates {
  rfx_ctx* ctx = nullptr;
  int k = 0, bits = 0;
  uint64_t* keys = nullptr;
  uint32_t* bins = nullptr;
  uint32_t* counts = nullptr;
  uint32_t n = 0;
};

static rfxk::binned_view binned_view_of(const rfx_binned* b) {
  rfxk::binned_view v;
  if (!b) return v;
  v.keys = b->st.keys;
  v.counts = b->st.counts;
  v.fill = b->st.fill;
  v.bin_at = b->bin_at;
  v.chunk = b->st.chunk;
  v.n_chunks = b->st.n_chunks;
  v.bin_lo = b->bin_lo;
  v.bin_hi = b->bin_hi;
  v.bits = b->bits;
  return v;
}

static void msp_binned_drop(rfx_finish* f) {
  rfx_ctx* c = f->t->ctx;
  leaf_stage_free(c, &f->bstage);
  dfree(c, f->bin_at);
  f->bin_at = nullptr;
  dfree(c, f->bsq);
  f->bsq = nullptr;
}

rfx_binned* rfx_count_finish_binned(rfx_table* t, uint64_t lower, uint64_t upper, uint64_t* histo) {
  if (!t) return nullptr;
  rfx_ctx* c = t->ctx;
  (void)hipSetDevice(c->device);
  if (t->pend_error) {
    snprintf(g_err, sizeof g_err, "a deferred MSP re-partition failed (%s); the table is incomplete", rfx_strerror(t->pend_error));
    return nullptr;
  }
  if (!t->table_active && t->segs->empty() && t->deferred->empty() && !t->peers) {
    rfx_binned* b = new rfx_binned();
    b->ctx = c;
    b->k = t->k;
    b->canonical = t->canonical;
    if (histo) memset(histo, 0, RFX_HISTO_BINS * 8);
    return b;
  }
  if (t->table_active || t->segs->empty() || t->seg_kind != RFX_COUNT_MSP || !t->deferred->empty() || t->peers ||
      t->pos_lo != 0 || t->pos_hi != (1ull << t->lsize)) {
    snprintf(g_err, sizeof g_err, "rfx_count_finish_binned: an MSP table with read blocks of its own, over all positions, on one device");
    return nullptr;
  }
  rfx_finish f;
  f.t = t;
  f.lower = lower;
  f.upper = upper;
  f.binned = true;
  const uint32_t P1 = (uint32_t)rfxk::p1_bins();
  const size_t ncur = (size_t)P1 * rfxk::p1_cur_stride();
  const rfx_ord_cfg cfg0 = ord_cfg(t, 7);
  for (int attempt = 0; attempt < 4; ++attempt) {
    int to_bits = 0;
    bool refine = false;
    uint64_t kmers = 0;
    std::vector<std::vector<uint64_t>> h_bs;
    if (msp_prepare_leaf(t, &to_bits, &refine, h_bs, &kmers, true) != RFX_OK) return nullptr;
    f.kmers = kmers;
    const size_t zero_bytes = ((size_t)RFX_HISTO_BINS + 1) * 8 + (ncur + RFX_CUR_TAIL) * 4;
    f.bsq = (uint64_t*)dmalloc(c, zero_bytes);
    if (!f.bsq) { snprintf(g_err, sizeof g_err, "rfx_count_finish_binned: out of device memory"); return nullptr; }
    unsigned long long* d_histo = (unsigned long long*)f.bsq;
    uint32_t* cur = (uint32_t*)(d_histo + RFX_HISTO_BINS + 1);
    hipError_t e = hipMemsetAsync(f.bsq, 0, zero_bytes, c->stream);
    if (e != hipSuccess) { hip_fail(e, "rfx_count_finish_binned"); msp_binned_drop(&f); return nullptr; }
    const int rc = msp_leaf_refined(&f, to_bits, h_bs, cfg0.sel_bits, cur, ncur);
    if (rc) {
      (void)ctx_sync(c);
      msp_binned_drop(&f);
      if (rc == RFX_E_NOMEM) snprintf(g_err, sizeof g_err, "rfx_count_finish_binned: out of device memory");
      return nullptr;
    }
    rfxk::histo_staged(c, f.bstage, d_histo, d_histo + RFX_HISTO_BINS);
    uint32_t tail[RFX_CUR_TAIL] = {0, 0, 0};
    uint64_t total = 0;
    std::vector<uint64_t> h(RFX_HISTO_BINS, 0);
    e = queue_read(c, tail, cur + ncur, sizeof tail);
    if (e == hipSuccess) e = queue_read(c, &total, d_histo + RFX_HISTO_BINS, 8);
    if (e == hipSuccess && histo) e = queue_read(c, h.data(), d_histo, RFX_HISTO_BINS * 8);
    if (e == hipSuccess) e = ctx_sync(c);
    if (e != hipSuccess) { hip_fail(e, "rfx_count_finish_binned"); (void)ctx_sync(c); msp_binned_drop(&f); return nullptr; }
    if (tail[1]) {
      msp_binned_drop(&f);
      snprintf(g_err, sizeof g_err, "MSP: a bin could not be split far enough to fit LDS");
      return nullptr;
    }
    if (tail[0]) {
      f.stage_extra += tail[2] + tail[2] / 4 + 64;
      msp_binned_drop(&f);
      continue;
    }
    rfx_binned* b = new rfx_binned();
    b->ctx = c;
    b->k = t->k;
    b->canonical = t->canonical;
    b->st = f.bstage;
    b->bin_at = f.bin_at;
    b->bin_lo = f.bin_lo;
    b->bin_hi = f.bin_hi;
    b->bits = f.bin_bits;
    b->n = total;
    f.bstage = rfxk::msp_stage{};
    f.bin_at = nullptr;
    msp_binned_drop(&f);
    if (histo) memcpy(histo, h.data(), RFX_HISTO_BINS * 8);
    if (kmers) {
      c->msp_surv_frac[lower >= 2 ? 1 : 0] = (double)total / (double)kmers;
      if (c->msp_surv_by_size.size() > 256) c->msp_surv_by_size.clear();
      c->msp_surv_by_size[msp_surv_key(lower, kmers)] = (double)total / (double)kmers;
    }
    uint64_t rec_bytes = 0;
    for (auto& sg : *t->segs) rec_bytes += sg.n * 8;
    if (rec_bytes > (4ull << 30)) p2l_drop_segments(t);
    return b;
  }
  snprintf(g_err, sizeof g_err, "MSP: the staging pool did not converge (internal error)");
  return nullptr;
}

uint64_t rfx_binned_size(const rfx_binned* b) { return b ? b->n : 0; }
int rfx_binned_bits(const rfx_binned* b) { return b ? b->bits : 0; }
void rfx_binned_free(rfx_binned* b) {
  if (!b) return;
  (void)hipSetDevice(b->ctx->device);
  leaf_stage_free(b->ctx, &b->st);
  dfree(b->ctx, b->bin_at);
  delete b;
}

rfx_candidates* rfx_binned_strike(rfx_ctx* c, rfx_binned* subject, const rfx_binned* control, uint32_t min_count,
                                  uint32_t max_count) {
  if (!c || !subject || subject->ctx != c || (control && (control->ctx != c || control->k != subject->k))) {
    snprintf(g_err, sizeof g_err, "rfx_binned_strike: bad argument");
    return nullptr;
  }
  (void)hipSetDevice(c->device);
  const rfxk::binned_view S = binned_view_of(subject), C = binned_view_of(control);
  uint64_t cap = std::max<uint64_t>(1u << 16, subject->n / 256);
  if (!control) cap = std::max<uint64_t>(cap, subject->n / 4);
  for (int attempt = 0; attempt < 2; ++attempt) {
    cap = std::min<uint64_t>(std::max<uint64_t>(cap, 1), 0xFFFFFFFFull);
    uint64_t* keys = (uint64_t*)dmalloc(c, cap * 8);
    uint32_t* bins = (uint32_t*)dmalloc(c, cap * 4);
    uint32_t* counts = (uint32_t*)dmalloc(c, cap * 4);
    uint32_t* d_n = (uint32_t*)dmalloc(c, 4);
    auto drop = [&] { dfree(c, keys); dfree(c, bins); dfree(c, counts); dfree(c, d_n); };
    if (!keys || !bins || !counts || !d_n) { drop(); snprintf(g_err, sizeof g_err, "rfx_binned_strike: out of device memory"); return nullptr; }
    hipError_t e = hipMemsetAsync(d_n, 0, 4, c->stream);
    uint32_t n = 0;
    if (e == hipSuccess) {
      rfxk::strike_bins(c, S, C, min_count, max_count, keys, bins, counts, (uint32_t)cap, d_n);
      e = queue_read(c, &n, d_n, 4);
    }
    if (e == hipSuccess) e = ctx_sync(c);
    if (e != hipSuccess) { hip_fail(e, "rfx_binned_strike"); (void)ctx_sync(c); drop(); return nullptr; }
    dfree(c, d_n);
    if (n > cap) {
      dfree(c, keys);
      dfree(c, bins);
      dfree(c, counts);
      cap = n;
      continue;
    }
    rfx_candidates* r = new rfx_candidates();
    r->ctx = c;
    r->k = subject->k;
    r->bits = subject->bits;
    r->keys = keys;
    r->bins = bins;
    r->counts = counts;
    r->n = n;
    return r;
  }
  snprintf(g_err, sizeof g_err, "rfx_binned_strike: the candidate list did not converge (internal error)");
  return nullptr;
}

int rfx_candidates_strike(rfx_candidates* a, const rfx_binned* control) {
  if (!a || !control || a->ctx != control->ctx || a->k != control->k) return RFX_E_INVAL;
  rfx_ctx* c = a->ctx;
  (void)hipSetDevice(c->device);
  rfxk::strike_cands(c, a->keys, a->bins, a->n, a->bits, binned_view_of(control));
  HIPCHK(ctx_sync(c));
  return RFX_OK;
}

uint64_t rfx_candidates_size(const rfx_candidates* a) { return a ? a->n : 0; }
int rfx_candidates_get(const rfx_candidates* a, uint64_t* keys_out) {
  if (!a || (a->n && !keys_out)) return RFX_E_INVAL;
  if (!a->n) return RFX_OK;
  (void)hipSetDevice(a->ctx->device);
  HIPCHK(ctx_sync(a->ctx));
  HIPCHK(hipMemcpy(keys_out, a->keys, (size_t)a->n * 8, hipMemcpyDeviceToHost));
  return RFX_OK;
}
int rfx_candidates_get_counts(const rfx_candidates* a, uint32_t* counts_out) {
  if (!a || (a->n && !counts_out)) return RFX_E_INVAL;
  if (!a->n) return RFX_OK;
  (void)hipSetDevice(a->ctx->device);
  HIPCHK(ctx_sync(a->ctx));
  HIPCHK(hipMemcpy(counts_out, a->counts, (size_t)a->n * 4, hipMemcpyDeviceToHost));
  return RFX_OK;
}

int rfx_candidates_strike_records(rfx_candidates* a, const rfx_records* exclude) {
  if (!a || !exclude || a->ctx != exclude->ctx) return RFX_E_INVAL;
  if (a->k != exclude->k) {
    snprintf(g_err, sizeof g_err, "rfx_candidates_strike_records: the records hold %d-mers, the candidates %d-mers", exclude->k, a->k);
    return RFX_E_FORMAT;
  }
  rfx_ctx* c = a->ctx;
  (void)hipSetDevice(c->device);
  rfxk::strike_query(c, a->keys, a->n, exclude->lut, exclude->ntab, exclude->keys, exclude->pos, exclude->n);
  HIPCHK(ctx_sync(c));
  return RFX_OK;
}

int rfx_binned_get(const rfx_binned* b, uint64_t* keys_out, uint32_t* counts_out, uint32_t* bins_out, uint64_t* at_out,
                   uint64_t cap, uint64_t* n_out) {
  if (!b || !n_out) return RFX_E_INVAL;
  *n_out = 0;
  const uint32_t nb = b->bin_hi - b->bin_lo;
  if (!b->bin_at || !nb) return RFX_OK;
  rfx_ctx* c = b->ctx;
  (void)hipSetDevice(c->device);
  const rfxk::binned_view v = binned_view_of(b);
  unsigned long long* d_offs = (unsigned long long*)dmalloc(c, ((size_t)nb + 1) * 8);
  if (!d_offs) return RFX_E_NOMEM;
  uint64_t n = 0;
  rfxk::binned_offsets(c, v, d_offs);
  hipError_t e = queue_read(c, &n, d_offs + nb, 8);
  if (e == hipSuccess) e = ctx_sync(c);
  if (e != hipSuccess) { (void)ctx_sync(c); dfree(c, d_offs); return hip_fail(e, "rfx_binned_get"); }
  *n_out = n;
// ... 1495 lines not shown
```

rufus_amd/csrc/rfx_internal.h:

```cpp
#pragma once
#include <hip/hip_runtime.h>
#include <stdint.h>

#include <atomic>
#include <map>
#include <string>
#include <vector>

#include "../../include/rufus_hip.h"

#define RFX_EMPTY 0xFFFFFFFFFFFFFFFFull
#define RFX_TILE 1024u
#define RFX_TABLE_MARGIN 65536u
#define RFX_PROBE_LIMIT 2048u

struct rfx_prof_span {
  std::string name;
  hipEvent_t e0, e1;
};
struct rfx_prof_acc {
  double ms = 0;
  uint64_t launches = 0;
};

struct rfx_hash_consts {
  uint64_t cols[64];
  int ntab = 0;
  uint64_t* lut = nullptr;
  uint64_t* lut_t = nullptr;
  uint64_t* lut_tinv = nullptr;
};

struct rfx_ctx {
  int device = 0;
  hipStream_t stream = nullptr;
  hipStream_t aux = nullptr;
  size_t budget = 0, used = 0;
  int n_cu = 256;
  bool prof = false;
  std::string prof_filter;
  std::vector<rfx_prof_span> spans;
  std::vector<hipEvent_t> free_events;
  std::map<std::string, rfx_prof_acc> acc;
  std::map<void*, size_t> allocs;
  std::multimap<size_t, void*> pool;
  char* arena = nullptr;
  size_t arena_reserved = 0, arena_mapped = 0, arena_gran = 0;
  std::vector<void*> arena_handles;
  std::map<size_t, size_t> arena_free;
  bool arena_off = false;
  size_t peak_used = 0;
  std::vector<int> peer_devices;
  uint32_t lds_opt_in = 0;
  hipError_t launch_error = hipSuccess;
  std::vector<struct rfx_table*> pend_tables;
  double msp_surv_frac[2] = {0, 0};
  std::map<uint64_t, double> msp_surv_by_size;
  char* pin = nullptr;
  size_t pin_cap = 0, pin_used = 0;
  uint8_t* load_pin[3] = {nullptr, nullptr, nullptr};
  size_t load_pin_bytes = 0;
  struct pin_read { void* dst; size_t off, n; };
  std::vector<pin_read> pin_reads;
  std::map<std::pair<int, uint64_t>, rfx_hash_consts> consts;
  std::map<int, std::vector<uint64_t>> std_cols;
};

struct rfx_table_stats {
  unsigned long long distinct;
  unsigned int max_disp;
  unsigned int overflow;
};

struct rfx_count_ctl {
  unsigned int ticket;
  unsigned int stop;
  unsigned int lost;
  unsigned int pad;
  unsigned long long ovf_n;
};

struct rfx_table_view {
  uint64_t* keys;
  uint32_t* counts;
  uint64_t slots;
  uint64_t cap;
  int rshift, lshift;
  uint64_t pos_lo, pos_hi;
  int ntab;
  int kshift;
};

struct rfx_ord_cfg {
  int c_bits;
  int sel_bits;
  int bin_shift;
};

struct rfx_segment {
  uint64_t* inst;
  uint64_t n;
  uint64_t* bin_start;
  uint64_t kmers;
  uint32_t bins;
  uint32_t* ext = nullptr;
  bool borrowed = false;
};

struct rfx_reads;
struct rfx_runmap_entry {
  void* map = nullptr;
  uint32_t* ovf = nullptr;
  uint32_t n_ovf = 0;
  uint32_t n_reads = 0;
  const uint64_t* codes = nullptr;
  uint64_t gen = 0;
  int k = 0, canonical = 0;
  size_t bytes = 0, map_bytes = 0, ovf_bytes = 0;
};
struct runmap_ahead;
struct rfx_runmaps {
  rfx_ctx* ctx = nullptr;
  runmap_ahead* ahead = nullptr;
  uint64_t budget = 0;
  uint64_t bytes = 0;
  uint64_t pending_bytes = 0;
  std::map<const rfx_reads*, rfx_runmap_entry> m;
  char* pool = nullptr;
  std::map<size_t, size_t> pool_free;
};
struct rfx_pending_add {
  const rfx_reads* r;
  uint32_t* cur;
  size_t seg;
  size_t ncur;
};

struct rfx_reads_view {
  const uint64_t* codes;
  const uint32_t* acgt;
// ... 171 lines not shown
void filter_big(rfx_ctx*, const rfx_reads_view&, const uint64_t* slots, int bits, int has_all_ones, const uint32_t* bm,
                int k, int thresh, int last_base_skipped, uint32_t* hits, uint64_t* hitmask, unsigned long long* d_nhit);
int filter_q_bits(uint64_t n_keys, int k);
void set_bitmap_q(rfx_ctx*, const uint64_t* keys, uint64_t n, uint32_t* bm , int bm_bits, int k);
void filter_q(rfx_ctx*, const rfx_reads_view&, const uint64_t* slots, int bits, int has_all_ones, const uint32_t* bm,
              int bm_bits, int k, int thresh, int last_base_skipped, uint32_t* hits, uint64_t* hitmask,
              unsigned long long* d_nhit);
int filter_p_applies(uint64_t n_keys, int k);
size_t filter_p_table_bytes();
void set_bitmap_p(rfx_ctx*, const uint64_t* keys, uint64_t n, uint32_t* bm , int k, int three);
void filter_p(rfx_ctx*, const rfx_reads_view&, const uint64_t* slots, int bits, int has_all_ones, const uint32_t* bm, int three,
              int k, int thresh, int last_base_skipped, uint32_t* hits , uint64_t* hitmask,
              unsigned long long* d_nhit);
void filter(rfx_ctx*, const rfx_reads_view&, const uint64_t* slots, int bits, int has_all_ones, const uint32_t* bm,
            int bm_bits, int bm_shift, int k, int thresh, int last_base_skipped, uint32_t* hits, uint64_t* hitmask,
            unsigned long long* d_nhit);
void overlap_score(rfx_ctx*, const char* d_a, int alen, const char* d_bcat, const uint32_t* d_boff, int nb, int max_blen,
                   float min_pct, int min_ovl, int strict3, int local_init, int* d_out );
void overlap_pool(rfx_ctx*, const char* arena, const uint64_t* off, const int* len, const char* a_explicit,
                  int a_explicit_len, int query, const int* cand, int nb, int strand_lo, int strand_hi, size_t lds,
                  float min_pct, int min_ovl, int strict3, int local_init, int* d_out);
void annotate(rfx_ctx*, const rfx_reads_view&, const uint64_t* slots, int bits, int has_all_ones, int k,
              const uint64_t* base_off, uint32_t* cov);
int p2l_grid(rfx_ctx*, uint32_t n_reads);
void bin_count(rfx_ctx*, const rfx_reads_view&, const uint64_t* lut, int ntab, int k, int canonical,
               const rfx_ord_cfg&, uint32_t P, uint64_t pos_lo, uint64_t pos_hi, int grid, uint32_t* cnt);
void bin_offsets(rfx_ctx*, uint32_t* cnt, uint32_t G, uint32_t P, uint32_t* gsum ,
                 uint64_t* bin_start );
void bin_totals(rfx_ctx*, const uint32_t* cnt, uint32_t G, uint32_t P, uint64_t* bin_start );
void bin_scatter(rfx_ctx*, const rfx_reads_view&, const uint64_t* lut, int ntab, int k, int canonical,
                 const rfx_ord_cfg&, uint32_t P, uint64_t pos_lo, uint64_t pos_hi, int grid, const uint32_t* rel,
                 const uint64_t* bin_start, uint64_t* inst);
int p1_bins();
int p1_cur_stride();
void coarse_counts(rfx_ctx*, const uint32_t* cnt, uint32_t G, uint32_t P, uint32_t P2, uint32_t* cnt1);
void part1(rfx_ctx*, const rfx_reads_view&, const uint64_t* lut, int ntab, int k, int canonical, const rfx_ord_cfg&,
           uint32_t P2, uint64_t pos_lo, uint64_t pos_hi, int grid, const uint32_t* rel1, const uint64_t* fine_start,
           uint64_t* buf_a);
void part1_fused(rfx_ctx*, const rfx_reads_view&, const uint64_t* lut, int ntab, int k, int canonical,
                 const rfx_ord_cfg&, uint32_t P2, uint64_t pos_lo, uint64_t pos_hi, int grid, uint64_t* buf_a,
                 uint32_t* coarse_cur, uint32_t cap_a, uint32_t* cnt_rows, unsigned int* flag);
void part2(rfx_ctx*, const uint64_t* buf_a, uint64_t* buf_b, const uint64_t* fine_start, uint32_t* fine_cur,
           uint32_t P2, int shift2, const uint32_t* coarse_cur, uint32_t cap_a, const uint32_t* pay_a,
           uint32_t* pay_b, uint64_t cap_b , const char* span,
           const uint64_t* coarse_start = nullptr , uint32_t n_coarse = 0,
           uint64_t n_hint = 0 ,
           int rec_mode = 0 ,
           int k = 0, uint64_t fine_base = 0 );
constexpr int part2_max_segs = 64;
void part2_multi(rfx_ctx*, const uint64_t* const* seg_a, const uint64_t* const* seg_cs, const uint32_t* const* seg_pay,
                 int nseg, uint32_t cs_off, uint32_t n_coarse, uint64_t n_hint, uint64_t* buf_b, const uint64_t* fine_start,
                 uint32_t* fine_cur, uint32_t P2, int shift2, uint32_t* pay_b, int rec_mode, int k, const char* span);
void bin_hist(rfx_ctx*, const uint64_t* src, const uint64_t* parent_start, uint32_t n_parents, uint64_t n_hint,
              uint32_t P2, int shift2, int rec_mode, int k, uint64_t* fine_tot,
              const uint32_t* ext = nullptr );
void bin_hist_multi(rfx_ctx*, const uint64_t* const* seg_src, const uint64_t* const* seg_ps, const uint32_t* const* seg_ext,
                    int nseg, uint32_t cs_off, uint32_t n_parents, uint64_t n_hint, uint32_t P2, int shift2, int rec_mode, int k,
                    uint64_t* fine_tot);
int msp_k_ok(int k);
int msp_part1_block();
int msp_nmax_of(int k);
int msp_window(int k);
int msp_wide(int k);
void msp_part1(rfx_ctx*, const rfx_reads_view&, int k, int canonical, int bin_bits, uint32_t bin_lo, uint32_t bin_hi,
               int hmode, int grid, void* rec_a, uint32_t* coarse_cur, uint32_t cap_a, uint32_t* cnt_rows,
               unsigned int* flag,
               int slab_log2 = 4 ,
               void* map_out = nullptr ,
               uint32_t* map_ovf = nullptr ,
               uint32_t map_ovf_cap = 0);
int msp_replay_grid(rfx_ctx*, uint32_t n_reads);
int msp_map_grid(rfx_ctx*, uint32_t n_reads);
void msp_replay(rfx_ctx*, const rfx_reads_view&, const void* map, int k, int canonical, int bin_bits, uint32_t bin_lo,
                uint32_t bin_hi, int grid, void* rec_a, uint32_t* coarse_cur, uint32_t cap_a, uint32_t* cnt_rows,
                unsigned int* flag, int slab_log2);
inline uint64_t msp_part1_slack(int grid, int slab_log2) { return (uint64_t)grid * 3u << slab_log2; }
struct msp_stage {
  uint64_t* keys = nullptr;
  uint32_t* counts = nullptr;
  uint32_t* fill = nullptr;
  uint32_t* more = nullptr;
  uint32_t chunk = 0, n_chunks = 0;
};
void msp_leaf(rfx_ctx*, const uint64_t* const* seg_inst, const uint64_t* const* seg_bs, int nseg,
              const uint64_t* inst0, const uint64_t* bs0, uint32_t P, int k, int canonical, const uint64_t* lut,
              int ntab, int sel_bits, int shift1, uint64_t pos_lo, uint64_t pos_hi, uint64_t lower, uint64_t upper,
              uint64_t* out_w, uint32_t* out_c, uint32_t* cur, uint32_t cap, unsigned int* flag, unsigned int* err,
              unsigned int* stage_short ,
              int geo ,
              const uint32_t* const* seg_ext, const uint32_t* ext0 , const msp_stage& st,
              uint32_t launch , uint32_t grid ,
              uint2* bin_at = nullptr );
struct binned_view {
  const uint64_t* keys = nullptr;
  uint32_t* counts = nullptr;
  const uint32_t* fill = nullptr;
  const uint2* bin_at = nullptr;
  uint32_t chunk = 0, n_chunks = 0, bin_lo = 0, bin_hi = 0;
  int bits = 0;
};
uint32_t msp_leaf_chunk_room(int geo, uint32_t chunk);
uint32_t msp_leaf_chunk_kept(uint32_t chunk);
void histo_staged(rfx_ctx*, const msp_stage&, unsigned long long* d_histo, unsigned long long* d_total);
void strike_bins(rfx_ctx*, const binned_view& S, const binned_view& C, uint32_t lo, uint32_t hi, uint64_t* out_k, uint32_t* out_b,
                 uint32_t* out_c, uint32_t cap, uint32_t* out_n);
void strike_cands(rfx_ctx*, uint64_t* keys, const uint32_t* bins, uint32_t n, int bits, const binned_view& C);
void binned_offsets(rfx_ctx*, const binned_view&, unsigned long long* d_offs);
void binned_gather(rfx_ctx*, const binned_view&, const unsigned long long* d_offs, uint64_t n, uint64_t* keys_out,
                   uint32_t* counts_out, uint32_t* bins_out, uint64_t* at_out);
void binned_checksum(rfx_ctx*, const msp_stage&, unsigned long long* d_out );
void binned_verify(rfx_ctx*, const binned_view&, int k, int canonical, uint64_t lower, uint64_t upper,
                   unsigned long long* d_out);
void binned_query(rfx_ctx*, const binned_view&, int k, int canonical, const uint64_t* qkeys, uint64_t nq, uint32_t* out);
void msp_leaf_plan(rfx_ctx*, uint32_t P, int geo, uint64_t n_records, uint64_t est_survivors, uint32_t extra, uint32_t* grid,
                   uint32_t* chunk, uint32_t* n_chunks);
void surv_hist(rfx_ctx*, const uint64_t* buf_a, const uint32_t* coarse_cur, uint32_t cap_a, uint32_t P2, int shift2,
               uint64_t* fine_tot, int rec_mode = 0 , int k = 0,
               uint64_t n_hint = 0);
void flag_if_gt(rfx_ctx*, const uint64_t* d_value, uint64_t limit, unsigned int* d_flag);
void histo_bins(rfx_ctx*, const uint32_t* counts, const uint32_t* coarse_cur, uint32_t cap, unsigned long long* d_histo);
void surv_sort(rfx_ctx*, const uint64_t* bw, const uint32_t* bc, const uint64_t* bs, uint32_t P, int bin_shift,
               const uint64_t* lut_inv, int ntab, int sel_bits, uint64_t* out_keys, uint32_t* out_counts,
               uint64_t* out_pos);
void tmp_start(rfx_ctx*, const uint64_t* const* seg_bs, int nseg, uint32_t P, uint64_t* out );
void leaf(rfx_ctx*, const uint64_t* const* seg_inst, const uint64_t* const* seg_bs, int nseg, const uint64_t* inst0,
          const uint64_t* bs0, uint32_t P, const rfx_ord_cfg&, uint64_t lower, uint64_t upper,
          const uint64_t* tmp_start, uint64_t* tmp_w, uint32_t* tmp_counts, uint64_t* n_surv, unsigned int* err);
void split_bins(rfx_ctx*, uint64_t* bs, uint32_t P, uint64_t n_own, uint64_t* bs2);
void scan_tail(rfx_ctx*, uint64_t* v, uint64_t n);
void bgzf_inflate(rfx_ctx*, hipStream_t stream, const uint8_t* stage, const struct bgzf_desc* desc, uint32_t n_blocks,
                  uint32_t first_index, uint8_t* arena, uint32_t* status, uint32_t* first_bad);
void leaf_compact(rfx_ctx*, const uint64_t* tmp_w, const uint32_t* tmp_counts, const uint64_t* tmp_start,
                  const uint64_t* out_off, uint32_t P, const uint64_t* lut_inv, int ntab, int sel_bits,
                  uint64_t* out_keys, uint32_t* out_counts, uint64_t* out_pos);
}

namespace rfxi {
void* dmalloc(rfx_ctx*, size_t bytes);
void dfree(rfx_ctx*, void*);
void set_error(const char* msg);
hipError_t sync(rfx_ctx*);
hipError_t queue_read(rfx_ctx*, void* dst, const void* d_src, size_t n);
bool lds_opt_in(rfx_ctx*, const void* fn, size_t bytes, int bit, const char* name);
rfx_reads* reads_tile(rfx_ctx*, const rfx_reads* src, int k, uint32_t tile_len, int* rc);
rfx_reads* reads_select_dev(rfx_ctx*, const rfx_reads* const* blocks, const uint64_t* const* d_masks, int n_blocks, int mode,
                            const char* who);
int text_ready(rfx_text* t, rfx_ctx** c, const uint8_t** arena, uint64_t* used);
hipError_t text_count_lines(rfx_ctx*, const uint8_t* arena, uint64_t n, uint64_t* tile_off);
hipError_t text_line_starts(rfx_ctx*, const uint8_t* arena, uint64_t n, const uint64_t* tile_off, uint32_t* line_start,
                            uint64_t max_lines);
}

struct rfx_span {
  rfx_ctx* c;
  hipStream_t st;
  rfx_prof_span s;
  bool on;
  rfx_span(rfx_ctx* ctx, const char* name, hipStream_t stream = nullptr)
      : c(ctx), st(stream ? stream : ctx->stream),
        on(ctx->prof && (ctx->prof_filter.empty() ||
                         ctx->prof_filter.find(std::string(",") + name + ",") != std::string::npos)) {
    if (on) {
      s.name = name;
      auto get = [&](hipEvent_t& e) {
        if (c->free_events.empty()) (void)hipEventCreate(&e);
        else {
          e = c->free_events.back();
          c->free_events.pop_back();
        }
      };
      get(s.e0);
      get(s.e1);
      (void)hipEventRecord(s.e0, st);
    }
  }
  ~rfx_span() {
    if (on) {
      (void)hipEventRecord(s.e1, st);
      c->spans.push_back(s);
    }
  }
};
```

rufus_amd/csrc/rfx_msp.hip:

```cpp
#include <algorithm>
#include <type_traits>

#include "rfx_devutil.h"
#include "rfx_internal.h"

#ifdef RFX_TIMING
__device__ unsigned long long g_tm[2048][32];
#define TM_ROW g_tm[blockIdx.x & 2047u]
#define TM_DECL unsigned long long tm_prev = __builtin_amdgcn_s_memtime()
#define TM(i) do { if (threadIdx.x == 0) { const unsigned long long tm_now = __builtin_amdgcn_s_memtime(); atomicAdd(&TM_ROW[i], tm_now - tm_prev); tm_prev = tm_now; } } while (0)
extern "C" int rfx_debug_timing(unsigned long long* out, int reset) {
  static unsigned long long h[2048][32];
  if (out) {
    if (hipMemcpyFromSymbol(h, HIP_SYMBOL(g_tm), sizeof(g_tm)) != hipSuccess) return -1;
    for (int i = 0; i < 32; ++i) {
      out[i] = 0;
      for (int w = 0; w < 2048; ++w) out[i] += h[w][i];
    }
  }
  if (reset) {
    void* p = nullptr;
    if (hipGetSymbolAddress(&p, HIP_SYMBOL(g_tm)) != hipSuccess || hipMemset(p, 0, sizeof(g_tm)) != hipSuccess) return -1;
  }
  return 0;
// ... 671 lines not shown
          if (slot[u] < 2 * SLAB) {
            const uint64_t sb = s_slab[slot[u] >> slab_log2][coarse];
            msp_rec12_store(rec_a, sb + (slot[u] & (SLAB - 1)), w, x);
          } else {
            const uint32_t at = atomicAdd(&coarse_cur[coarse * P1_CUR_STRIDE], 1u);
            if (at < cap_a) msp_rec12_store(rec_a, (uint64_t)coarse * cap_a + at, w, x);
            else atomicExch(flag, 1u);
          }
          ++n_emit;
          const uint32_t fb = run_bin[u] - bin_lo;
          atomicAdd(&s_fine[fb >> 2], 1u << ((fb & 3u) * 8));
        }
      }
    }
    }
    __syncthreads();
    if (threadIdx.x < P1_BINS) {
      uint32_t f = s_fill[threadIdx.x];
      if (f >= SLAB) {
        if (f >= 2 * SLAB) {
          s_slab[0][threadIdx.x] = slab_at(threadIdx.x, pending);
          s_slab[1][threadIdx.x] = slab_at(threadIdx.x, reserve_raw(threadIdx.x));
          f = 0;
        } else {
          s_slab[0][threadIdx.x] = s_slab[1][threadIdx.x];
          s_slab[1][threadIdx.x] = slab_at(threadIdx.x, pending);
          f -= SLAB;
        }
        pending = reserve_raw(threadIdx.x);
        s_fill[threadIdx.x] = f;
      }
    }
    __syncthreads();
  }
  if (threadIdx.x < P1_BINS) s_slab[2][threadIdx.x] = slab_at(threadIdx.x, pending);
  if (threadIdx.x == 0) s_sum = s_emit = 0;
  __syncthreads();
  for (uint32_t i = threadIdx.x; i < 3u * P1_BINS * SLAB; i += blockDim.x) {
    const uint32_t o = i & (SLAB - 1), bw = i >> slab_log2, b = bw & (P1_BINS - 1), which = bw >> 7;
    const uint64_t sb = s_slab[which][b];
    if (sb != ~0ull && (which == 2 || which * SLAB + o >= s_fill[b])) msp_rec12_store(rec_a, sb + o, MSP_EMPTY, 0u);
  }
  uint32_t sum = 0;
  for (uint32_t b = threadIdx.x; b < P; b += blockDim.x) {
    const uint32_t fb = b - bin_lo;
    const uint32_t v = fb < bin_hi - bin_lo ? (s_fine[fb >> 2] >> ((fb & 3u) * 8)) & 0xFFu : 0u;
    cnt_rows[(uint64_t)blockIdx.x * P + b] = v;
    sum += v;
  }
  atomicAdd(&s_sum, sum);
  atomicAdd(&s_emit, n_emit);
  __syncthreads();
  if (threadIdx.x == 0 && s_sum != s_emit) atomicExch(flag, 1u);
}

__device__ __forceinline__ uint32_t split_hash(uint64_t key) {
  return (uint32_t)((key * 0xD6E8FEB86659FD93ull) >> 32);
}

#ifndef RFX_LEAF_BLK
#define RFX_LEAF_BLK 768
#endif
constexpr uint32_t MSP_LEAF_BLK(int geo) { return geo ? (uint32_t)RFX_LEAF_BLK : 1024u; }
#ifndef RFX_LEAF_WPE
#define RFX_LEAF_WPE (2 * RFX_LEAF_BLK / 256)
#endif
constexpr int MSP_LEAF_WPE(int geo) { return geo ? RFX_LEAF_WPE : 4; }
constexpr uint32_t MSP_LEAF_PASS_MAX(int geo) { return (geo ? 4096u : 8192u) * 3 / 4 + MSP_LEAF_BLK(geo); }
constexpr uint32_t MSP_LEAF_CHUNK(int geo, bool big) { return big ? (geo ? 16384u : 32768u) : MSP_LEAF_PASS_MAX(geo) + 512u; }
#ifndef MSP_ILP_OVERRIDE
#define MSP_ILP_OVERRIDE 3
#endif
constexpr int MSP_ILP = MSP_ILP_OVERRIDE;
#ifndef RFX_RC_PROBES
#define RFX_RC_PROBES 16
#endif
#ifndef RFX_RC_SHRINK
#define RFX_RC_SHRINK 2
#endif
constexpr int MSP_RC_PROBES = RFX_RC_PROBES;
constexpr unsigned long long MSP_RK_MUL = 0x9E3779B97F4A7C15ull;
constexpr uint32_t MSP_RC_UNLISTED = 0x80000000u;

template <bool CANON, int GEO>
__global__ __launch_bounds__(MSP_LEAF_BLK(GEO)) __attribute__((amdgpu_waves_per_eu(MSP_LEAF_WPE(GEO), MSP_LEAF_WPE(GEO)))) void k_msp_leaf(
    const uint64_t* const* __restrict__ seg_inst, const uint64_t* const* __restrict__ seg_bs, int nseg,
    const uint64_t* __restrict__ inst0, const uint64_t* __restrict__ bs0, const uint32_t* const* __restrict__ seg_ext,
    const uint32_t* __restrict__ ext0, uint32_t P, int k, uint64_t lower, uint64_t upper,
    uint64_t* __restrict__ stage_k, uint32_t* __restrict__ stage_c, uint32_t CH, uint32_t* __restrict__ stage_fill,
    uint32_t* __restrict__ stage_more, uint32_t n_chunks, unsigned int* __restrict__ flag, unsigned int* __restrict__ err,
    unsigned int* __restrict__ stage_short, int force_mixed, uint2* __restrict__ bin_at) {
  constexpr int TBL_LOG2 = GEO ? 12 : 13, TBL = 1 << TBL_LOG2, BLK = (int)MSP_LEAF_BLK(GEO), FILL = TBL * 3 / 4;
  static_assert(MSP_LEAF_PASS_MAX(GEO) >= (uint32_t)(FILL + BLK) && FILL + BLK <= TBL, "what a pass can leave behind fits the chunk and the table");
  constexpr int RC_LOG2 = TBL_LOG2 - (GEO ? RFX_RC_SHRINK : 2), RC = 1 << RC_LOG2, KMAP = TBL;
  static_assert(RC <= 8192, "a k-mer map entry is slot << 3 | pair in 16 bits");
  __shared__ __attribute__((aligned(16))) unsigned long long s_keys[TBL];
  __shared__ uint32_t s_cnt[TBL];
  __shared__ unsigned long long s_rk[RC];
  __shared__ uint32_t s_rc[RC], s_rmin[RC], s_rmax[RC];
  __shared__ uint32_t s_mixed[2];
  __shared__ __attribute__((aligned(16))) uint16_t s_kmap[KMAP];
  __shared__ uint32_t s_chunk;
  __shared__ uint32_t s_nd[2], s_ovf[2], s_nk[2], s_ns[2];

  uint64_t pre[MSP_ILP];
  uint32_t prex[MSP_ILP];
  uint64_t pre_a = 0, pre_e = 0;
  uint64_t nx_a = blockIdx.x < P ? bs0[blockIdx.x] : 0, nx_e = blockIdx.x < P ? bs0[blockIdx.x + 1] : 0;
  auto prefetch = [&](uint32_t b) {
    if (b >= P) return;
    pre_a = nx_a;
    pre_e = nx_e;
    if (b + gridDim.x < P) {
      nx_a = bs0[b + gridDim.x];
      nx_e = bs0[b + gridDim.x + 1];
    }
#pragma unroll
    for (int u = 0; u < MSP_ILP; ++u) {
      const uint64_t i = pre_a + threadIdx.x + (uint64_t)u * BLK;
      pre[u] = i < pre_e ? inst0[i] : MSP_EMPTY;
      prex[u] = i < pre_e ? ext0[i] : 0u;
    }
  };
  prefetch(blockIdx.x);
  for (int i = threadIdx.x; i < TBL; i += BLK) {
    s_keys[i] = RFX_EMPTY;
    s_cnt[i] = 0;
  }
  for (int i = threadIdx.x; i < RC; i += BLK) {
    s_rk[i] = MSP_EMPTY;
    s_rc[i] = 0;
    s_rmin[i] = ~0u;
    s_rmax[i] = 0;
  }
  if (threadIdx.x < 2) s_nd[threadIdx.x] = s_ovf[threadIdx.x] = s_nk[threadIdx.x] = s_ns[threadIdx.x] = s_mixed[threadIdx.x] = 0;
  if (threadIdx.x == 0) {
    uint32_t ch0 = blockIdx.x;
    if (bin_at) {
      const uint2 at0 = bin_at[2 * (size_t)blockIdx.x];
      if (at0.x < n_chunks) {
        ch0 = at0.x;
        s_ns[0] = at0.y;
      } else {
        ch0 = atomicAdd(stage_more, 1u);
        if (ch0 >= n_chunks) {
          atomicExch(flag, 1u);
          atomicMax(stage_short, ch0 - n_chunks + 1u);
          ch0 = 0;
        }
        bin_at[2 * (size_t)blockIdx.x] = make_uint2(ch0, 0u);
      }
    }
    s_chunk = ch0;
  }
  uint32_t used = 0;
  uint32_t X = 0;
  __syncthreads();

  for (uint32_t bin = blockIdx.x; bin < P; bin += gridDim.x) {
    const uint64_t a0 = pre_a, e0 = pre_e;
    bool prefetched_next = false;
    int r = 0;
    uint32_t j = 0;
    bool failed = false, nocache = false;
    TM_DECL;
    for (;;) {
      TM(15);
      auto insert_fwd = [&](uint64_t fwd, uint32_t mult) {
        uint64_t key = fwd;
        if (CANON) {
          const uint64_t rc = revcomp_bases(fwd, k);
          key = rc < fwd ? rc : fwd;
        }
        if (r > 0 && (split_hash(key) >> (32 - r)) != j) return;
        if (__hip_atomic_load(&s_nd[X], __ATOMIC_RELAXED, __HIP_MEMORY_SCOPE_WORKGROUP) >= (uint32_t)FILL) {
          s_ovf[X] = 1;
          return;
        }
        const uint32_t hk = leaf_hash32(key);
        uint32_t slot = hk >> (32 - TBL_LOG2);
        const uint32_t step = ((hk >> 3) | 1u) & (TBL - 1);
        bool fresh = false;
        for (;;) {
          const unsigned long long old = atomicCAS(&s_keys[slot], (unsigned long long)RFX_EMPTY, (unsigned long long)key);
          fresh = old == RFX_EMPTY;
          if (fresh || old == key) break;
          slot = (slot + step) & (TBL - 1);
        }
        atomicAdd(&s_cnt[slot], mult);
        if (fresh) atomicAdd(&s_nd[X], 1u);
      };
      auto insert_record = [&](uint64_t x, uint32_t xe, uint32_t mult) {
        uint64_t lo, hi;
        msp_record_run(x, xe, k, lo, hi);
        const int n = msp_record_n(x);
        for (int q = 0; q < n; ++q) insert_fwd(msp_run_kmer(lo, hi, k, n, q), mult);
      };
      for (int sg = 0; sg < nseg; ++sg) {
        const uint64_t a = sg == 0 ? a0 : seg_bs[sg][bin], e = sg == 0 ? e0 : seg_bs[sg][bin + 1];
        const uint64_t* __restrict__ src = sg == 0 ? inst0 : seg_inst[sg];
        const uint32_t* __restrict__ srcx = sg == 0 ? ext0 : seg_ext[sg];
        for (uint64_t base = a; base < e; base += (uint64_t)MSP_ILP * BLK) {
          uint64_t rec[MSP_ILP];
          uint32_t recx[MSP_ILP];
          if (sg == 0 && base == a && !prefetched_next) {
#pragma unroll
            for (int u = 0; u < MSP_ILP; ++u) {
              rec[u] = pre[u];
              recx[u] = prex[u];
            }
          } else {
#pragma unroll
            for (int u = 0; u < MSP_ILP; ++u) {
              const uint64_t i = base + threadIdx.x + (uint64_t)u * BLK;
              rec[u] = i < e ? src[i] : MSP_EMPTY;
              recx[u] = i < e ? srcx[i] : 0u;
            }
          }
#pragma unroll
          for (int u = 0; u < MSP_ILP; ++u) {
            const uint64_t x = rec[u];
            const uint32_t xe = msp_plane_bits(recx[u], k);
            if (x == MSP_EMPTY) continue;
            uint32_t h = (uint32_t)x ^ (uint32_t)(x >> 23) ^ (uint32_t)(x >> 41) ^ (xe * 0x85EBCA6Bu);
            h *= 0x9E3779B1u;
            const uint32_t hstep = ((h >> 5) | 1u) & (RC - 1);
            h >>= 32 - RC_LOG2;
            int state = 0;
            const unsigned long long ck = x ^ ((unsigned long long)xe * MSP_RK_MUL);
            if (!nocache && ck != MSP_EMPTY) {
              for (int p = 0; p < MSP_RC_PROBES; ++p) {
                const unsigned long long old = atomicCAS(&s_rk[h], (unsigned long long)MSP_EMPTY, ck);
                if (old == MSP_EMPTY || old == ck) {
                  state = old == ck ? 2 : 1;
                  break;
                }
                h = (h + hstep) & (RC - 1);
              }
            }
            if (state) {
              atomicAdd(&s_rc[h], 1u);
              atomicMin(&s_rmin[h], xe);
              atomicMax(&s_rmax[h], xe);
            }
            TMC(22, 1);
            TMC(23, state == 0);
            if (state == 1) {
              const uint32_t np = ((uint32_t)msp_record_n(x) + 1u) >> 1;
              const uint32_t kb = atomicAdd(&s_nk[X], np);
              if (kb + np <= (uint32_t)KMAP) {
#pragma unroll
                for (uint32_t q = 0; q < 8; ++q)
                  if (q < np) s_kmap[kb + q] = (uint16_t)((h << 3) | q);
              } else {
                for (uint32_t q = kb; q < (uint32_t)KMAP; ++q) s_kmap[q] = 0xFFFFu;
                atomicOr(&s_rc[h], MSP_RC_UNLISTED);
              }
            }
            if (state == 0) insert_record(x, xe, 1u);
          }
        }
      }
      if (!prefetched_next) {
        prefetch(bin + gridDim.x);
        prefetched_next = true;
      }
      TM(16);
      __syncthreads();
      TM(9);
      if (threadIdx.x == 0) s_nd[X ^ 1] = s_ovf[X ^ 1] = s_nk[X ^ 1] = s_ns[X ^ 1] = s_mixed[X ^ 1] = 0;
      const uint32_t nk_all = s_nk[X], nk = min(nk_all, (uint32_t)KMAP);
      for (uint32_t i = threadIdx.x; i < nk; i += BLK) {
        const uint32_t e = s_kmap[i];
        if (e == 0xFFFFu) continue;
        const uint32_t slot = e >> 3, q = (e & 7u) << 1;
        const uint32_t xe = s_rmax[slot];
        const uint64_t x = s_rk[slot] ^ ((uint64_t)xe * MSP_RK_MUL);
        if (q == 0 && s_rmin[slot] != xe) s_mixed[X] = 1;
        uint64_t lo, hi;
        msp_record_run(x, xe, k, lo, hi);
        const int n = msp_record_n(x);
        const uint32_t mult = s_rc[slot];
        insert_fwd(msp_run_kmer(lo, hi, k, n, (int)q), mult);
        if ((int)q + 1 < n) insert_fwd(msp_run_kmer(lo, hi, k, n, (int)q + 1), mult);
      }
      if (nk_all > (uint32_t)KMAP) {
        for (int i = threadIdx.x; i < RC; i += BLK) {
          const uint32_t c = s_rc[i];
          if (c & MSP_RC_UNLISTED) {
            const uint32_t xe = s_rmax[i];
            if (s_rmin[i] != xe) s_mixed[X] = 1;
            insert_record(s_rk[i] ^ ((uint64_t)xe * MSP_RK_MUL), xe, c & ~MSP_RC_UNLISTED);
          }
        }
      }
      TM(17);
      __syncthreads();
      TM(11);
      const bool mixed = s_mixed[X] != 0 || (force_mixed && !nocache && bin % 3u == 1u);
      const bool ovf = s_ovf[X] != 0 || mixed;
      const bool split = s_ovf[X] != 0 && !mixed;
      TMC(20, split);
      TMC(24, mixed);
      TMC(21, 1);
      uint64_t* const stk = stage_k + (size_t)s_chunk * CH;
      uint32_t* const stc = stage_c + (size_t)s_chunk * CH;
      for (int i = threadIdx.x; i < TBL; i += BLK) {
        const uint64_t key = s_keys[i];
        if (key == RFX_EMPTY) continue;
        const uint32_t c = s_cnt[i];
        s_keys[i] = RFX_EMPTY;
        s_cnt[i] = 0;
        if (!ovf && c >= lower && c <= upper) {
          const uint32_t o = used + atomicAdd(&s_ns[X], 1u);
          stk[o] = key;
          stc[o] = c;
        }
      }
      for (int i = threadIdx.x; i < RC; i += BLK) {
        s_rk[i] = MSP_EMPTY;
        s_rc[i] = 0;
        s_rmin[i] = ~0u;
        s_rmax[i] = 0;
      }
      TM(18);
      __syncthreads();
      TM(12);
      used += s_ns[X];
      X ^= 1u;
      if (used > CH && threadIdx.x == 0) atomicExch(err, 1u);
      if (used > CH - MSP_LEAF_PASS_MAX(GEO)) {
        if (threadIdx.x == 0) {
          const uint32_t mine = s_chunk;
          stage_fill[mine] = used;
          uint32_t nx = (bin_at ? 0u : gridDim.x) + atomicAdd(stage_more, 1u);
          if (nx >= n_chunks) {
            atomicExch(flag, 1u);
            atomicMax(stage_short, nx - n_chunks + 1u);
            nx = mine;
          }
          if (bin_at) stage_fill[n_chunks + mine] = nx;
          s_chunk = nx;
        }
        used = 0;
        TM(13);
      }
      if (mixed) {
        nocache = true;
        continue;
      }
      if (split) {
        if (r >= LEAF_RMAX) {
          failed = true;
          break;
        }
        ++r;
        j <<= 1;
      } else {
        while (r > 0 && (j & 1u)) {
          j >>= 1;
          --r;
        }
        if (r == 0) break;
        ++j;
      }
    }
    if (failed && threadIdx.x == 0) atomicExch(err, 1u);
    if (bin_at && threadIdx.x == 0) {
      const uint2 at = make_uint2(s_chunk, used);
      bin_at[2 * (size_t)bin + 1] = at;
      bin_at[2 * ((size_t)bin + gridDim.x)] = at;
    }
  }
  if (threadIdx.x == 0) stage_fill[s_chunk] = used;
}

#ifndef RFX_SP_BLK
#define RFX_SP_BLK 512
#endif
#ifndef RFX_SP_NE
#define RFX_SP_NE 8
#endif
constexpr int SP_BLK = RFX_SP_BLK, SP_NE = RFX_SP_NE, SP_N = SP_BLK * SP_NE;
__global__ __launch_bounds__(SP_BLK) void k_surv_place(const uint64_t* __restrict__ stage_k, const uint32_t* __restrict__ stage_c,
                                                       uint32_t CH, uint32_t* __restrict__ stage_fill,
                                                       uint32_t* __restrict__ stage_more, uint32_t n_first, uint32_t n_chunks,
                                                       const uint64_t* __restrict__ g_lut, int ntab, int sel_bits, int shift1,
                                                       uint64_t pos_lo, uint64_t pos_hi, uint64_t* __restrict__ out_w,
                                                       uint32_t* __restrict__ out_c, uint32_t* __restrict__ cur, uint32_t cap,
                                                       unsigned int* __restrict__ flag) {
  __shared__ uint64_t s_lut[8 * 256];
  __shared__ uint64_t s_w[SP_N];
  __shared__ uint32_t s_c[SP_N];
  __shared__ uint32_t s_pc[P1_BINS], s_pst[P1_BINS], s_nfl;
  __shared__ uint64_t s_pbase[P1_BINS];
  static_assert(P1_BINS == 128, "the scan below is two waves wide");
  for (int i = threadIdx.x; i < ntab * 256; i += SP_BLK) s_lut[i] = g_lut[i];
  if (threadIdx.x < P1_BINS) s_pc[threadIdx.x] = 0;
  __syncthreads();
  const uint32_t n_used = min(n_first + *stage_more, n_chunks);
  uint32_t ch = blockIdx.x, base = 0;
  uint32_t used = ch < n_used ? min(stage_fill[ch], CH) : 0u;
  uint32_t ch_n = ch + gridDim.x;
  uint32_t used_n = ch_n < n_used ? min(stage_fill[ch_n], CH) : 0u;
  auto settle = [&]() {
    while (ch < n_used && base >= used) {
      if (threadIdx.x == 0 && used) stage_fill[ch] = 0;
      ch = ch_n;
      used = used_n;
      base = 0;
      ch_n += gridDim.x;
      used_n = ch_n < n_used ? min(stage_fill[ch_n], CH) : 0u;
    }
  };
  uint64_t nk[SP_NE];
  uint32_t nc[SP_NE];
  auto fetch = [&]() {
    const bool any = ch < n_used;
    const uint32_t n_in = any ? min((uint32_t)SP_N, used - base) : 0u;
    const uint64_t* const stk = stage_k + (size_t)(any ? ch : 0u) * CH + base;
    const uint32_t* const stc = stage_c + (size_t)(any ? ch : 0u) * CH + base;
#pragma unroll
    for (int u = 0; u < SP_NE; ++u) {
      const uint32_t i = threadIdx.x + (uint32_t)u * SP_BLK;
      nk[u] = i < n_in ? stk[i] : RFX_EMPTY;
      nc[u] = i < n_in ? stc[i] : 0u;
    }
  };
  settle();
  fetch();
  while (ch < n_used) {
    uint64_t kv[SP_NE];
    uint32_t cv[SP_NE];
#pragma unroll
    for (int u = 0; u < SP_NE; ++u) {
      kv[u] = nk[u];
      cv[u] = nc[u];
    }
    base += (uint32_t)SP_N;
    settle();
    fetch();
#pragma unroll
    for (int u = 0; u < SP_NE; ++u) {
      if (kv[u] == RFX_EMPTY) continue;
      uint64_t w = 0;
#pragma unroll
      for (int t = 0; t < 8; ++t)
        if (t < ntab) w ^= s_lut[t * 256 + (uint32_t)((kv[u] >> (8 * t)) & 255u)];
      const uint64_t pos = w >> sel_bits;
      if (pos >= pos_lo && pos < pos_hi) atomicAdd(&s_pc[(uint32_t)(w >> shift1)], 1u);
      else w = RFX_EMPTY;
      kv[u] = w;
    }
    __syncthreads();
    if (threadIdx.x < P1_BINS) {
// ... 89 lines not shown
    const uint32_t c = counts[i];
    atomicAdd(&s_h[c > 10001u ? 10001u : c], 1u);
  }
  __syncthreads();
  for (int b = threadIdx.x; b < RFX_HISTO_BINS; b += blockDim.x)
    if (s_h[b]) atomicAdd(&g_histo[b], (unsigned long long)s_h[b]);
}

constexpr int SS_BLOCK = 512;
constexpr int SS_CAP = 2048;

__global__ __launch_bounds__(SS_BLOCK) void k_surv_sort(const uint64_t* __restrict__ bw,
                                                         const uint32_t* __restrict__ bc,
                                                         const uint64_t* __restrict__ bs, uint32_t P, int bin_shift,
                                                         const uint64_t* __restrict__ g_lut_inv, int ntab, int sel_bits,
                                                         uint64_t* __restrict__ out_keys,
                                                         uint32_t* __restrict__ out_counts,
                                                         uint64_t* __restrict__ out_pos) {
  __shared__ uint64_t s_lut[8 * 256];
  __shared__ uint64_t s_w2[SS_CAP];
  __shared__ uint32_t s_c2[SS_CAP];
  __shared__ uint32_t s_bstart[LEAF_BUCKETS + 1], s_bfill[LEAF_BUCKETS];
  for (int i = threadIdx.x; i < ntab * 256; i += blockDim.x) s_lut[i] = g_lut_inv[i];
  const int bsh = bin_shift > 8 ? bin_shift - 8 : 0;
  for (uint32_t bin = blockIdx.x; bin < P; bin += gridDim.x) {
    const uint64_t a = bs[bin];
    const uint64_t n = bs[bin + 1] - a;
    __syncthreads();
    if (n == 0) continue;
    if (n > (uint64_t)SS_CAP) {
      for (uint64_t i = threadIdx.x; i < n; i += SS_BLOCK) {
        const uint64_t wi = bw[a + i];
        uint64_t rank = 0;
        for (uint64_t q = 0; q < n; ++q) rank += bw[a + q] < wi;
        out_keys[a + rank] = gf2_mul(s_lut, wi, ntab);
        out_counts[a + rank] = bc[a + i];
        out_pos[a + rank] = wi >> sel_bits;
      }
      continue;
    }
    if (threadIdx.x < LEAF_BUCKETS) s_bfill[threadIdx.x] = 0;
    __syncthreads();
    constexpr int PER = SS_CAP / SS_BLOCK;
    uint64_t rw[PER];
    uint32_t rc[PER];
#pragma unroll
    for (int u = 0; u < PER; ++u) {
      const uint32_t i = threadIdx.x + (uint32_t)u * SS_BLOCK;
      rw[u] = i < (uint32_t)n ? bw[a + i] : 0;
      rc[u] = i < (uint32_t)n ? bc[a + i] : 0;
    }
#pragma unroll
    for (int u = 0; u < PER; ++u)
      if (threadIdx.x + (uint32_t)u * SS_BLOCK < (uint32_t)n)
        atomicAdd(&s_bfill[(uint32_t)(rw[u] >> bsh) & (LEAF_BUCKETS - 1)], 1u);
    __syncthreads();
    if (threadIdx.x < 64) wave_scan256(s_bfill, s_bstart, LEAF_BUCKETS);
    __syncthreads();
    if (threadIdx.x < LEAF_BUCKETS) s_bfill[threadIdx.x] = 0;
    __syncthreads();
#pragma unroll
    for (int u = 0; u < PER; ++u)
      if (threadIdx.x + (uint32_t)u * SS_BLOCK < (uint32_t)n) {
        const uint32_t bk = (uint32_t)(rw[u] >> bsh) & (LEAF_BUCKETS - 1);
        const uint32_t p = s_bstart[bk] + atomicAdd(&s_bfill[bk], 1u);
        s_w2[p] = rw[u];
        s_c2[p] = rc[u];
      }
    __syncthreads();
    for (uint32_t i = threadIdx.x; i < (uint32_t)n; i += SS_BLOCK) {
      const uint64_t wi = s_w2[i];
      const uint32_t bk = (uint32_t)(wi >> bsh) & (LEAF_BUCKETS - 1);
      const uint32_t b0 = s_bstart[bk], b1 = s_bstart[bk + 1];
      uint32_t rank = b0;
      for (uint32_t q = b0; q < b1; ++q) rank += s_w2[q] < wi;
      out_keys[a + rank] = gf2_mul(s_lut, wi, ntab);
      out_counts[a + rank] = s_c2[i];
      out_pos[a + rank] = wi >> sel_bits;
    }
  }
}


__device__ __forceinline__ uint4 binned_marks(const rfxk::binned_view& v, uint32_t gbin) {
  if (!v.bin_at || gbin < v.bin_lo || gbin >= v.bin_hi) return make_uint4(~0u, ~0u, ~0u, ~0u);
  return reinterpret_cast<const uint4*>(v.bin_at)[gbin - v.bin_lo];
}
template <class F>
__device__ __forceinline__ void binned_segments(const rfxk::binned_view& v, const uint4 m, F&& fn) {
  const uint2 a = make_uint2(m.x, m.y), e = make_uint2(m.z, m.w);
  if (e.x >= v.n_chunks) return;
  uint32_t ch = a.x, o = a.y;
  for (uint32_t hops = 0; hops <= v.n_chunks && ch < v.n_chunks; ++hops) {
    const bool last = ch == e.x;
    const uint32_t end = min(last ? e.y : v.fill[ch], v.chunk);
    if (end > o) fn((size_t)ch * v.chunk, o, end);
    if (last) break;
    ch = v.fill[v.n_chunks + ch];
    o = 0;
  }
}
template <class F>
__device__ __forceinline__ void binned_segments(const rfxk::binned_view& v, uint32_t gbin, F&& fn) {
  binned_segments(v, binned_marks(v, gbin), fn);
}
template <class F>
__device__ __forceinline__ void binned_range(const rfxk::binned_view& v, uint32_t b0, uint32_t b1, const uint4 first, F&& fn) {
  for (uint32_t b = b0; b < b1; ++b)
    binned_segments(v, b == b0 ? first : binned_marks(v, b), [&](size_t f0, uint32_t o, uint32_t e) { fn(b, f0, o, e); });
}

__device__ __forceinline__ void cand_append(bool surv, uint64_t key, uint32_t bin, uint32_t count, uint64_t* __restrict__ out_k,
                                            uint32_t* __restrict__ out_b, uint32_t* __restrict__ out_c, uint32_t cap,
                                            uint32_t* __restrict__ out_n) {
  const unsigned long long m = __ballot(surv);
  if (!m) return;
  const uint32_t lane = threadIdx.x & 63u, leader = (uint32_t)__ffsll(m) - 1u;
  uint32_t base = 0;
  if (lane == leader) base = atomicAdd(out_n, (uint32_t)__popcll(m));
  base = __shfl(base, (int)leader, 64);
  if (surv) {
    const uint32_t at = base + (uint32_t)__popcll(m & ((1ull << lane) - 1ull));
    if (at < cap) {
      out_k[at] = key;
      out_b[at] = bin;
      out_c[at] = count;
    }
  }
}

constexpr int SB_BLK = 128, SB_SET_LOG2 = 11, SB_SET = 1 << SB_SET_LOG2, SB_TILE = SB_SET / 2;
__device__ __forceinline__ uint32_t sb_hash(uint64_t key) { return (uint32_t)((key * 0x9E3779B97F4A7C15ull) >> 40); }

__global__ __launch_bounds__(SB_BLK) void k_strike_bins(const rfxk::binned_view S, const rfxk::binned_view C, int ubits, uint32_t u_lo,
                                                        uint32_t u_hi, uint32_t lo, uint32_t hi, uint64_t* __restrict__ out_k,
                                                        uint32_t* __restrict__ out_b, uint32_t* __restrict__ out_c, uint32_t cap,
                                                        uint32_t* __restrict__ out_n) {
  __shared__ unsigned long long s_set[SB_SET];
  const int ds = S.bits - ubits, dc = C.bin_at ? C.bits - ubits : 0;
  for (uint32_t u = u_lo + blockIdx.x; u < u_hi; u += gridDim.x) {
    uint32_t n_s = 0, n_c = 0;
    const uint32_t s0 = u << ds, s1 = (u + 1u) << ds, c0 = u << dc, c1 = C.bin_at ? (u + 1u) << dc : c0;
    const uint4 ms = binned_marks(S, s0), mc = binned_marks(C, c0);
    binned_range(S, s0, s1, ms, [&](uint32_t, size_t, uint32_t o, uint32_t e) { n_s += e - o; });
    if (!n_s) continue;
    binned_range(C, c0, c1, mc, [&](uint32_t, size_t, uint32_t o, uint32_t e) { n_c += e - o; });
    const uint32_t tiles = n_c ? (n_c + SB_TILE - 1u) / SB_TILE : 1u;
    const bool single = tiles == 1u;
    for (uint32_t t = 0; t < tiles; ++t) {
      const uint32_t t0 = t * SB_TILE, t1 = min(t0 + (uint32_t)SB_TILE, n_c);
      uint32_t lg = 8;
      while ((1u << lg) < 2u * (t1 - t0)) ++lg;
      const uint32_t mask = (1u << lg) - 1u;
      for (uint32_t i = threadIdx.x; i <= mask; i += SB_BLK) s_set[i] = RFX_EMPTY;
      __syncthreads();
      if (t1 > t0) {
        uint32_t idx0 = 0;
        binned_range(C, c0, c1, mc, [&](uint32_t, size_t first, uint32_t o, uint32_t e) {
            const uint32_t from = max(idx0, t0), to = min(idx0 + (e - o), t1);
            for (uint32_t i = from + threadIdx.x; i < to; i += SB_BLK) {
              const unsigned long long key = C.keys[first + o + (i - idx0)];
              uint32_t h = sb_hash(key) & mask;
              for (;;) {
                const unsigned long long old = atomicCAS(&s_set[h], (unsigned long long)RFX_EMPTY, key);
                if (old == RFX_EMPTY || old == key) break;
                h = (h + 1u) & mask;
              }
            }
            idx0 += e - o;
          });
      }
      __syncthreads();
      binned_range(S, s0, s1, ms, [&](uint32_t b, size_t first, uint32_t o, uint32_t e) {
          for (uint32_t i0 = o; i0 < e; i0 += SB_BLK) {
            const uint32_t i = i0 + threadIdx.x;
            uint64_t key = 0;
            uint32_t c = 0;
            if (i < e) {
              c = S.counts[first + i];
              key = S.keys[first + i];
              bool drop = false;
              if (t == 0 && c && (c < lo || c > hi)) drop = true;
              if (c && !drop && t1 > t0) {
                uint32_t h = sb_hash(key) & mask;
                for (;;) {
                  const unsigned long long v = s_set[h];
                  if (v == key) drop = true;
                  if (v == key || v == RFX_EMPTY) break;
                  h = (h + 1u) & mask;
                }
              }
              if (drop) {
                c = 0;
                if (!single) S.counts[first + i] = 0;
              }
            }
            if (single) cand_append(c != 0, key, b, c, out_k, out_b, out_c, cap, out_n);
          }
        });
      __syncthreads();
    }
    if (!single)
      binned_range(S, s0, s1, ms, [&](uint32_t b, size_t first, uint32_t o, uint32_t e) {
          for (uint32_t i0 = o; i0 < e; i0 += SB_BLK) {
            const uint32_t i = i0 + threadIdx.x;
            const uint32_t c = i < e ? S.counts[first + i] : 0u;
            cand_append(c != 0, c ? S.keys[first + i] : 0ull, b, c, out_k, out_b, out_c, cap, out_n);
          }
        });
  }
}

__global__ __launch_bounds__(256) void k_strike_cands(uint64_t* __restrict__ keys, const uint32_t* __restrict__ bins, uint32_t n,
                                                      int bits, const rfxk::binned_view C) {
  const uint32_t lane = threadIdx.x & 63u, wave = (blockIdx.x * 256u + threadIdx.x) >> 6, n_waves = gridDim.x * 4u;
  for (uint32_t i = wave; i < n; i += n_waves) {
    const uint64_t key = keys[i];
    if (key == RFX_EMPTY) continue;
    const uint32_t sb = bins[i];
    const uint32_t b0 = C.bits >= bits ? sb << (C.bits - bits) : sb >> (bits - C.bits);
    const uint32_t b1 = C.bits >= bits ? (sb + 1u) << (C.bits - bits) : b0 + 1u;
    bool found = false;
    for (uint32_t b = b0; b < b1; ++b)
      binned_segments(C, b, [&](size_t first, uint32_t o, uint32_t e) {
        for (uint32_t j = o + lane; j < e; j += 64u) found |= C.keys[first + j] == key;
      });
    if (__ballot(found) && lane == 0) keys[i] = RFX_EMPTY;
  }
}

__global__ __launch_bounds__(256) void k_histo_staged(const uint32_t* __restrict__ counts, const uint32_t* __restrict__ fill,
                                                       const uint32_t* __restrict__ more, uint32_t CH, uint32_t n_chunks,
                                                       unsigned long long* __restrict__ g_histo,
                                                       unsigned long long* __restrict__ g_total) {
  __shared__ uint32_t s_h[RFX_HISTO_BINS];
  for (int i = threadIdx.x; i < RFX_HISTO_BINS; i += 256) s_h[i] = 0;
  __syncthreads();
  const uint32_t n_used = min(*more, n_chunks);
  unsigned long long total = 0;
  for (uint32_t ch = blockIdx.x; ch < n_used; ch += gridDim.x) {
    const uint32_t n = min(fill[ch], CH);
    const uint32_t* const src = counts + (size_t)ch * CH;
    total += n;
    uint32_t i = threadIdx.x;
    for (; i + 3u * 256u < n; i += 4u * 256u) {
      uint32_t c[4];
#pragma unroll
      for (int q = 0; q < 4; ++q) c[q] = src[i + q * 256];
#pragma unroll
      for (int q = 0; q < 4; ++q) atomicAdd(&s_h[c[q] > 10001u ? 10001u : c[q]], 1u);
    }
    for (; i < n; i += 256u) {
      const uint32_t c = src[i];
      atomicAdd(&s_h[c > 10001u ? 10001u : c], 1u);
    }
  }
  __syncthreads();
  for (int b = threadIdx.x; b < RFX_HISTO_BINS; b += 256)
    if (s_h[b]) atomicAdd(&g_histo[b], (unsigned long long)s_h[b]);
  if (threadIdx.x == 0 && total) atomicAdd(g_total, total);
}



__global__ __launch_bounds__(256) void k_binned_sizes(const rfxk::binned_view v, unsigned long long* __restrict__ sizes) {
  const uint32_t nb = v.bin_hi - v.bin_lo;
  for (uint64_t i = (uint64_t)blockIdx.x * 256u + threadIdx.x; i < nb; i += (uint64_t)gridDim.x * 256u) {
    unsigned long long n = 0;
    binned_segments(v, v.bin_lo + (uint32_t)i, [&](size_t, uint32_t o, uint32_t e) { n += e - o; });
    sizes[i] = n;
  }
}

constexpr int BSC_BLK = 1024;
__global__ __launch_bounds__(BSC_BLK) void k_binned_scan(unsigned long long* __restrict__ a, uint32_t nb) {
  __shared__ unsigned long long s_sum[BSC_BLK];
  const uint64_t per = ((uint64_t)nb + BSC_BLK - 1) / BSC_BLK;
  const uint64_t lo = min((uint64_t)threadIdx.x * per, (uint64_t)nb), hi = min(lo + per, (uint64_t)nb);
  unsigned long long sum = 0;
  for (uint64_t i = lo; i < hi; ++i) sum += a[i];
  s_sum[threadIdx.x] = sum;
  __syncthreads();
  if (threadIdx.x == 0) {
    unsigned long long run = 0;
    for (int i = 0; i < BSC_BLK; ++i) {
      const unsigned long long t = s_sum[i];
      s_sum[i] = run;
      run += t;
    }
    a[nb] = run;
  }
  __syncthreads();
  unsigned long long run = s_sum[threadIdx.x];
  for (uint64_t i = lo; i < hi; ++i) {
    const unsigned long long t = a[i];
    a[i] = run;
    run += t;
  }
}

__global__ __launch_bounds__(256) void k_binned_gather(const rfxk::binned_view v, const unsigned long long* __restrict__ offs,
                                                        unsigned long long n_total, uint64_t* __restrict__ keys_out,
                                                        uint32_t* __restrict__ counts_out, uint32_t* __restrict__ bins_out,
                                                        uint64_t* __restrict__ at_out) {
  const uint32_t nb = v.bin_hi - v.bin_lo;
  for (uint32_t bi = blockIdx.x; bi < nb; bi += gridDim.x) {
    unsigned long long d0 = offs[bi];
    binned_segments(v, v.bin_lo + bi, [&](size_t first, uint32_t o, uint32_t e) {
      for (uint32_t j = o + threadIdx.x; j < e; j += 256u) {
        const unsigned long long d = d0 + (j - o);
        if (d >= n_total) continue;
        if (keys_out) keys_out[d] = v.keys[first + j];
        if (counts_out) counts_out[d] = v.counts[first + j];
        if (bins_out) bins_out[d] = v.bin_lo + bi;
        if (at_out) at_out[d] = first + j;
      }
      d0 += e - o;
    });
  }
}

__global__ __launch_bounds__(256) void k_binned_checksum(const uint64_t* __restrict__ keys, const uint32_t* __restrict__ counts,
                                                          const uint32_t* __restrict__ fill, const uint32_t* __restrict__ more,
                                                          uint32_t CH, uint32_t n_chunks, unsigned long long* __restrict__ out) {
  const uint32_t n_used = min(*more, n_chunks);
  unsigned long long a = 0, b = 0;
  for (uint32_t ch = blockIdx.x; ch < n_used; ch += gridDim.x) {
    const uint32_t n = min(fill[ch], CH);
    const size_t first = (size_t)ch * CH;
    for (uint32_t i = threadIdx.x; i < n; i += 256u) {
      const uint64_t m = checksum_mix(keys[first + i]);
      a += m * counts[first + i];
      b += m;
    }
  }
#pragma unroll
  for (int o = 32; o; o >>= 1) {
    a += __shfl_xor(a, o);
    b += __shfl_xor(b, o);
  }
  if ((threadIdx.x & 63u) == 0) {
    atomicAdd(&out[0], a);
    atomicAdd(&out[1], b);
  }
}
// ... 98 lines not shown

void msp_part1(rfx_ctx* c, const rfx_reads_view& rv, int k, int canonical, int bin_bits, uint32_t bin_lo, uint32_t bin_hi,
               int hmode, int grid, void* rec_a, uint32_t* coarse_cur, uint32_t cap_a, uint32_t* cnt_rows,
               unsigned int* flag, int slab_log2, void* map_out, uint32_t* map_ovf, uint32_t map_ovf_cap) {
  rfx_span sp(c, hmode == 1 ? "k_msp_count" : hmode == 4 ? "k_msp_map" : "k_msp_part1");
#define RFX_MSP_P1(CANON, HM, WL)                                                                             \
  hipLaunchKernelGGL((k_msp_part1<CANON, HM, WL>), dim3(grid), dim3(MP1_BLOCK), 0, c->stream, rv, k, bin_bits, \
                     bin_lo, bin_hi, (msp_rec12*)rec_a, coarse_cur, cap_a, cnt_rows, flag, slab_log2, (uint4*)map_out, \
                     map_ovf, map_ovf_cap)
#define RFX_MSP_P1_HM(CANON, WL)          \
  do {                                          \
    if (hmode == 0) RFX_MSP_P1(CANON, 0, WL);      \
    else if (hmode == 1) RFX_MSP_P1(CANON, 1, WL); \
    else if (hmode == 3) RFX_MSP_P1(CANON, 3, WL); \
    else if (hmode == 4) RFX_MSP_P1(CANON, 4, WL); \
    else RFX_MSP_P1(CANON, 2, WL);                 \
  } while (0)
#define RFX_MSP_P1_WL(WL)                      \
  case WL:                                     \
    if (canonical) RFX_MSP_P1_HM(true, WL);    \
    else RFX_MSP_P1_HM(false, WL);             \
    break
  switch (msp_wl(k)) {
    RFX_MSP_P1_WL(11);
    RFX_MSP_P1_WL(12);
    RFX_MSP_P1_WL(13);
    RFX_MSP_P1_WL(14);
    RFX_MSP_P1_WL(15);
    default:
      if (canonical) RFX_MSP_P1_HM(true, MSP_WL_WIDE);
      else RFX_MSP_P1_HM(false, MSP_WL_WIDE);
  }
#undef RFX_MSP_P1_WL
#undef RFX_MSP_P1_HM
#undef RFX_MSP_P1
}

int msp_map_grid(rfx_ctx* c, uint32_t n_reads) {
  const uint32_t chunks = (n_reads + MP1_BLOCK - 1) / MP1_BLOCK;
  return (int)std::max<uint32_t>(8, std::min<uint32_t>((uint32_t)c->n_cu * 3, (chunks + 7) & ~7u));
}

int msp_replay_grid(rfx_ctx* c, uint32_t n_reads) {
  const uint32_t chunks = (n_reads + MP1_BLOCK - 1) / MP1_BLOCK;
  return (int)std::max<uint32_t>(8, std::min<uint32_t>((uint32_t)c->n_cu * 2, (chunks + 7) & ~7u));
}

void msp_replay(rfx_ctx* c, const rfx_reads_view& rv, const void* map, int k, int canonical, int bin_bits, uint32_t bin_lo,
                uint32_t bin_hi, int grid, void* rec_a, uint32_t* coarse_cur, uint32_t cap_a, uint32_t* cnt_rows,
                unsigned int* flag, int slab_log2) {
  rfx_span sp(c, "k_msp_replay");
  static const bool queued = getenv("RFX_REPLAY_OLD") == nullptr;
#define RFX_REPLAY(CANON, Q)                                                                                                  \
  hipLaunchKernelGGL((k_msp_replay<CANON, Q>), dim3(grid), dim3(MP1_BLOCK), 0, c->stream, rv, (const uint4*)map, k, bin_bits, \
                     bin_lo, bin_hi, (msp_rec12*)rec_a, coarse_cur, cap_a, cnt_rows, flag, slab_log2)
  if (canonical) {
    if (queued) RFX_REPLAY(true, true);
    else RFX_REPLAY(true, false);
  } else {
    if (queued) RFX_REPLAY(false, true);
    else RFX_REPLAY(false, false);
  }
#undef RFX_REPLAY
}

void msp_leaf_plan(rfx_ctx* c, uint32_t P, int geo, uint64_t n_records, uint64_t est_survivors, uint32_t extra, uint32_t* grid,
                   uint32_t* chunk, uint32_t* n_chunks) {
  const uint32_t per_cu = geo ? 8 : 4;
  uint64_t g = std::min<uint64_t>(P, (uint64_t)c->n_cu * per_cu);
  g = std::min<uint64_t>(g, std::max<uint64_t>(1, n_records >> 12));
  *grid = (uint32_t)std::max<uint64_t>(g, 1);
  *chunk = MSP_LEAF_CHUNK(geo, n_records >= (1ull << 24));
  const uint64_t per = *chunk - MSP_LEAF_PASS_MAX(geo);
  uint64_t more = (est_survivors + est_survivors / 2) / per + 16 + extra;
  if (getenv("RFX_LEAF_STAGE_TEST")) more = extra;
  *n_chunks = (uint32_t)std::min<uint64_t>((uint64_t)*grid + more, 1u << 30);
}

void msp_leaf(rfx_ctx* c, const uint64_t* const* seg_inst, const uint64_t* const* seg_bs, int nseg,
              const uint64_t* inst0, const uint64_t* bs0, uint32_t P, int k, int canonical, const uint64_t* lut,
              int ntab, int sel_bits, int shift1, uint64_t pos_lo, uint64_t pos_hi, uint64_t lower, uint64_t upper,
              uint64_t* out_w, uint32_t* out_c, uint32_t* cur, uint32_t cap, unsigned int* flag, unsigned int* err,
              unsigned int* stage_short, int geo, const uint32_t* const* seg_ext, const uint32_t* ext0, const msp_stage& st,
              uint32_t launch, uint32_t grid, uint2* bin_at) {
  const int force_mixed = getenv("RFX_LEAF_FORCE_MIXED") != nullptr;
  uint32_t* const more = st.more + (bin_at ? 0u : launch);
  {
    rfx_span sp(c, "k_msp_leaf");
#define RFX_MSP_LEAF(CANON, GEO)                                                                                        \
  hipLaunchKernelGGL((k_msp_leaf<CANON, GEO>), dim3(grid), dim3(MSP_LEAF_BLK(GEO)), 0, c->stream, seg_inst, seg_bs, nseg, \
                     inst0, bs0, seg_ext, ext0, P, k, lower, upper, st.keys, st.counts, st.chunk, st.fill, more,           \
                     st.n_chunks, flag, err, stage_short, force_mixed, bin_at)
    if (canonical) {
      if (geo) RFX_MSP_LEAF(true, 1);
      else RFX_MSP_LEAF(true, 0);
    } else {
      if (geo) RFX_MSP_LEAF(false, 1);
      else RFX_MSP_LEAF(false, 0);
    }
#undef RFX_MSP_LEAF
  }
  if (!bin_at) {
    rfx_span sp(c, "k_surv_place");
    const uint32_t pg = std::min<uint32_t>(st.n_chunks, (uint32_t)c->n_cu * (uint32_t)std::max(1, 160 * 1024 / (16 * 1024 + SP_N * 12 + 2048)));
    hipLaunchKernelGGL(k_surv_place, dim3(pg), dim3(SP_BLK), 0, c->stream, st.keys, st.counts, st.chunk, st.fill, more, grid,
                       st.n_chunks, lut, ntab, sel_bits, shift1, pos_lo, pos_hi, out_w, out_c, cur, cap, flag);
  }
}

uint32_t msp_leaf_chunk_room(int geo, uint32_t chunk) { return chunk - MSP_LEAF_PASS_MAX(geo); }
uint32_t msp_leaf_chunk_kept(uint32_t chunk) { return chunk >= 16384u ? 65536u : chunk; }

void histo_staged(rfx_ctx* c, const msp_stage& st, unsigned long long* d_histo, unsigned long long* d_total) {
  rfx_span sp(c, "k_histo");
  const uint32_t grid = std::max<uint32_t>(1, std::min<uint32_t>(st.n_chunks, (uint32_t)c->n_cu * 4));
  hipLaunchKernelGGL(k_histo_staged, dim3(grid), dim3(256), 0, c->stream, st.counts, st.fill, st.more, st.chunk, st.n_chunks,
                     d_histo, d_total);
}

void strike_bins(rfx_ctx* c, const binned_view& S, const binned_view& C, uint32_t lo, uint32_t hi, uint64_t* out_k,
                 uint32_t* out_b, uint32_t* out_c, uint32_t cap, uint32_t* out_n) {
  rfx_span sp(c, "k_strike_bins");
  const int ubits = C.bin_at ? std::min(S.bits, C.bits) : S.bits;
  const int ds = S.bits - ubits;
  const uint32_t u_lo = S.bin_lo >> ds, u_hi = (uint32_t)((((uint64_t)S.bin_hi + (1u << ds) - 1)) >> ds);
  if (u_hi <= u_lo) return;
  const uint32_t grid = std::min<uint32_t>(u_hi - u_lo, (uint32_t)c->n_cu * 10);
  hipLaunchKernelGGL(k_strike_bins, dim3(grid), dim3(SB_BLK), 0, c->stream, S, C, ubits, u_lo, u_hi, lo, hi, out_k, out_b, out_c,
                     cap, out_n);
}

void strike_cands(rfx_ctx* c, uint64_t* keys, const uint32_t* bins, uint32_t n, int bits, const binned_view& C) {
  if (!n) return;
  rfx_span sp(c, "k_strike_cands");
  const uint32_t grid = std::min<uint32_t>((n + 3) / 4, (uint32_t)c->n_cu * 8);
  hipLaunchKernelGGL(k_strike_cands, dim3(grid), dim3(256), 0, c->stream, keys, bins, n, bits, C);
}

void binned_offsets(rfx_ctx* c, const binned_view& v, unsigned long long* d_offs) {
  rfx_span sp(c, "k_binned_get");
  const uint32_t nb = v.bin_hi - v.bin_lo;
  if (nb) {
    const uint32_t grid = std::max<uint32_t>(1, std::min<uint32_t>((nb + 255u) / 256u, (uint32_t)c->n_cu * 8));
    hipLaunchKernelGGL(k_binned_sizes, dim3(grid), dim3(256), 0, c->stream, v, d_offs);
  }
  hipLaunchKernelGGL(k_binned_scan, dim3(1), dim3(BSC_BLK), 0, c->stream, d_offs, nb);
}

void binned_gather(rfx_ctx* c, const binned_view& v, const unsigned long long* d_offs, uint64_t n, uint64_t* keys_out,
                   uint32_t* counts_out, uint32_t* bins_out, uint64_t* at_out) {
  const uint32_t nb = v.bin_hi - v.bin_lo;
  if (!nb || !n) return;
  rfx_span sp(c, "k_binned_get");
  const uint32_t grid = std::min<uint32_t>(nb, (uint32_t)c->n_cu * 8);
  hipLaunchKernelGGL(k_binned_gather, dim3(grid), dim3(256), 0, c->stream, v, d_offs, (unsigned long long)n, keys_out, counts_out,
                     bins_out, at_out);
}

void binned_checksum(rfx_ctx* c, const msp_stage& st, unsigned long long* d_out) {
  if (!st.n_chunks) return;
  rfx_span sp(c, "k_binned_checksum");
  const uint32_t grid = std::max<uint32_t>(1, std::min<uint32_t>(st.n_chunks, (uint32_t)c->n_cu * 4));
  hipLaunchKernelGGL(k_binned_checksum, dim3(grid), dim3(256), 0, c->stream, st.keys, st.counts, st.fill, st.more, st.chunk,
                     st.n_chunks, d_out);
}

void binned_verify(rfx_ctx* c, const binned_view& v, int k, int canonical, uint64_t lower, uint64_t upper,
                   unsigned long long* d_out) {
  const uint32_t nb = v.bin_hi - v.bin_lo;
  if (!nb) return;
  rfx_span sp(c, "k_binned_verify");
  const uint32_t grid = std::min<uint32_t>(nb, (uint32_t)c->n_cu * 8);
  hipLaunchKernelGGL(k_binned_verify, dim3(grid), dim3(BV_BLK), 0, c->stream, v, k, canonical, (unsigned long long)lower,
                     (unsigned long long)upper, d_out);
}

void binned_query(rfx_ctx* c, const binned_view& v, int k, int canonical, const uint64_t* qkeys, uint64_t nq, uint32_t* out) {
  if (!nq) return;
  rfx_span sp(c, "k_binned_query");
  const uint32_t grid = (uint32_t)std::min<uint64_t>((nq + 3) / 4, (uint64_t)c->n_cu * 8);
  hipLaunchKernelGGL(k_binned_query, dim3(grid), dim3(256), 0, c->stream, v, k, canonical, qkeys, nq, out);
}

void surv_hist(rfx_ctx* c, const uint64_t* buf_a, const uint32_t* coarse_cur, uint32_t cap_a, uint32_t P2, int shift2,
               uint64_t* fine_tot, int rec_mode, int k, uint64_t n_hint) {
  rfx_span sp(c, rec_mode ? "k_rec_hist" : "k_surv_hist");
  uint32_t W = 8;
  if (n_hint > (1ull << 27)) W = (uint32_t)c->n_cu * 2 / P1_BINS * 4;
#define RFX_SH(MODE)                                                                                                \
  hipLaunchKernelGGL(k_surv_hist<MODE>, dim3(P1_BINS * W), dim3(L2_BLOCK), 0, c->stream, buf_a, coarse_cur, cap_a, P2, \
                     shift2, W, k, (unsigned long long*)fine_tot)
  if (rec_mode == 0) RFX_SH(0);
  else if (rec_mode == 1) RFX_SH(1);
  else RFX_SH(2);
#undef RFX_SH
}

void flag_if_gt(rfx_ctx* c, const uint64_t* d_value, uint64_t limit, unsigned int* d_flag) {
  hipLaunchKernelGGL(k_flag_if_gt, dim3(1), dim3(1), 0, c->stream, d_value, limit, d_flag);
}

void histo_bins(rfx_ctx* c, const uint32_t* counts, const uint32_t* coarse_cur, uint32_t cap,
                unsigned long long* d_histo) {
  rfx_span sp(c, "k_histo");
  const uint32_t W = 16;
  hipLaunchKernelGGL(k_histo_bins, dim3(P1_BINS * W), dim3(256), 0, c->stream, counts, coarse_cur, cap, W, d_histo);
}

void surv_sort(rfx_ctx* c, const uint64_t* bw, const uint32_t* bc, const uint64_t* bs, uint32_t P, int bin_shift,
               const uint64_t* lut_inv, int ntab, int sel_bits, uint64_t* out_keys, uint32_t* out_counts,
               uint64_t* out_pos) {
  rfx_span sp(c, "k_surv_sort");
// ... 7 lines not shown
```

rufus_amd/wgs.py:

```python
from __future__ import annotations

import os
import time

import numpy as np

from . import capi
from .dist import revcomp_keys


class _DevMem32:

    def __init__(self, ptr: int, n: int):
        self.__cuda_array_interface__ = {"shape": (n,), "typestr": "<i4", "data": (ptr, False), "version": 3,
                                         "strides": None}


def _device_view32(ptr: int, n: int, device):
    import torch
    return torch.as_tensor(_DevMem32(ptr, n), device=device)


class _LibraryCall:

# ... 5 lines not shown
    def _run(self, fn, args):
        try:
            fn(*args)
        except Exception as e:
            self.err = e

    def start(self):
        self._t.start()

    def join(self):
        self._t.join()


class GroupFailure(capi.RufusError):

    def __init__(self, msg: str, retry: bool):
        super().__init__(msg)
        self.retry = retry


def _is_out_of_memory(e: BaseException) -> bool:
    return "memory" in str(e).lower() or type(e).__name__ == "OutOfMemoryError"


def shard_cut(q: int, n: int) -> int:
    return -(-q * 256 // n)

_EVEN = np.uint64(0x5555555555555555)


def pulled_pairs(mask: np.ndarray, n_reads: int) -> int:
    m = mask[:(n_reads + 63) // 64]
    return int(np.bitwise_count((m | (m >> np.uint64(1))) & _EVEN).sum())


def plan_passes(n_reads_total: int, read_len: int, k: int, resident_bytes: int, hbm_bytes: int, n_samples: int = 3,
                coverage_hint: float = 30.0, world: int = 1, wide: bool = False) -> int:
    windows = n_reads_total * max(read_len - k + 1, 0)
    distinct = windows / max(coverage_hint * (read_len - k + 1) / read_len, 1.0)
    for s in range(1, 257 // world):
        share = s * world
        records = (1.6 if wide else 2.2) * windows / share * (2.0 if world > 1 else 1.0)
        transient = records * 1.125 + 12.0 * distinct / share * 1.3 + (20.0 if n_samples > 1 else 0.0) * distinct / share
        if resident_bytes + transient < 0.90 * hbm_bytes:
            return s
    return max(1, 256 // world)


def plan_steps(passes: int, n_samples: int, use_maps: bool, keep_shard_records: bool) -> list:
    P, ns = passes, n_samples
    if use_maps and ns > 2:
        return [(sh, si) for sh in range(P) for si in (0, 1)] + [(sh, si) for si in range(2, ns) for sh in range(P)]
    return [(sh, si) for sh in range(P)
            for si in (list(range(ns)) if sh % 2 == 0 or keep_shard_records else [0] + list(range(ns - 1, 0, -1)))]


def plan_maps_ahead(steps) -> dict:
    first, last_of = {}, {}
    for i, (_, si) in enumerate(steps):
        first.setdefault(si, i)
        last_of[si] = i
    order = sorted(first, key=first.get)
    ahead = {}
    for n, si in enumerate(order[1:], 1):
        at = first[si] - 1
        if n >= 2 and at <= last_of[order[n - 2]]:
            continue
        ahead[steps[at]] = si
    return ahead


class _BinnedCandidates:
    entry_bytes = 12

    def __init__(self, ctx, store, min_count: int, max_count: int):
        self.ctx, self._h, self._range = ctx, store, (min_count, max_count)

    def __len__(self):
        return len(self._h)

    @property
    def raw_bytes(self) -> int:
        return len(self._h) * self.entry_bytes if self._range else 0

    def _becomes(self, struck):
        self._h.free()
        self._h, self._range = struck, None

    def strike(self, control):
        if self._range:
            self._becomes(capi.binned_strike(self.ctx, self._h, control, *self._range))
        else:
            self._h.strike(control)

    def finish(self, exclude):
        if self._range:
            self.strike(None)
        for ex in exclude:
            self._h.strike_records(ex)
        out = self._h.keys_counts()
        self.free()
        return out

    def free(self):
        if self._h is not None:
            self._h.free()
            self._h = None


class _SortedCandidates(_BinnedCandidates):
    entry_bytes = 20

    def strike(self, *controls):
        self._becomes(capi.records_subtract(self.ctx, self._h, list(controls), *(self._range or ())))

    def finish(self, exclude):
        if self._range:
            self.strike()
        if exclude:
            self.strike(*exclude)
        out = self._h.get()[:2]
        self.free()
        return out


class _Attempt:

    def __init__(self, n_samples: int, passes: int, verify):
        self.histos, self.n_rec = [np.zeros(capi.HISTO_BINS, dtype=np.uint64) for _ in range(n_samples)], [0] * n_samples
        self.keys, self.kcounts = [], []
        self.recs = {sh: [] for sh in range(passes)}
        self.cands, self.kept = {}, []
        self.ver = {"bad_order": 0, "bad_pos": 0, "bad_count": 0, "sum_counts": [0] * n_samples,
                    "probe_found": [0] * n_samples, "probe_count_out_of_range": 0,
                    "checksum": [[0, 0] for _ in range(n_samples)]}
        if verify == "binned":
            self.ver.update(bad_bin=0, duplicate=0, not_canonical=0)

    def release(self):
        held = [r for recs in list(self.recs.values()) + self.kept for r in recs] + list(self.cands.values())
        self.recs, self.kept, self.cands = {}, [], {}
        for r in held:
            r.free()


class WgsTrio:

    def __init__(self, ctx: capi.Context, k: int, size: int, lower: int, min_cov: int, max_cov: int, thresh: int,
                 passes: int = 1, group=None):
        self.ctx, self.k, self.size = ctx, k, size
        self.lsize = capi.ceil_log2(size)
        self.cols = capi.jf_matrix(self.lsize, k)
        self.lower, self.min_cov, self.max_cov, self.thresh = lower, min_cov, max_cov, thresh
        self.passes = passes
        self.group = group
        self.early_budget = 0
        self._early, self._early_left, self._early_cost = {}, 0, 0
        self._injected = False
        self.map_budget = 0
        self._store = None
        self._ahead = {}
        self.maps_ahead = 0
        self.count_wall_s = 0.0
        self.masks_are_views = False
        self.replayed_blocks = 0
        self.binned_counts = 0
# ... 250 lines not shown
                    lo = vb[me] * sper
                    full[lo:lo + off_rl[src]] = loc
                    full[lo + off_rl[src]:] = loc[-1]
                    full = full.to(dev, non_blocking=True)
                    run = rr[ro:ro + recv_l[src]]
                    run_e = re_[ro:ro + recv_l[src]] if wide else None
                    todo.append((run, full, run_e, sbins, recv_l[src]))
                    ro += recv_l[src]
                    bo += off_rl[src]
                torch.cuda.synchronize(dev)
                try:
                    for run, full, run_e, sbins, n_run in todo:
                        if n_run:
                            own.adopt_records_dev(run.data_ptr(), run.numel(), full.data_ptr(), sbins,
                                                  run_e.data_ptr() if wide else 0)
                        keep.append((run, full, run_e))
                except Exception as e:
                    err = e
                del rr
                t_ = lap("import", t_)
            if trace:
                print("[wgs] exchange of shard %d: " % shard + ", ".join(f"{k_} {v * 1e3:.0f} ms" for k_, v in tt.items()), flush=True)
            part.free()
            out = None
            if err is None:
                try:
                    self._inject("finish", shard)
                    out = own.finish(self.lower, want_histo=True)
                    self.ctx.sync()
                except Exception as e:
                    err = e
            keep.clear()
            self.checkpoint(err)
            return out
        finally:
            if helper is not None:
                helper.join()
            own.free()

    def _verify_store(self, ver, rec, si: int, probe_keys):
        v = rec.verify(self.lower)
        for k_ in v:
            if k_ != "sum_counts":
                ver[k_] += v[k_]
        ver["sum_counts"][si] += v["sum_counts"]
        ver["checksum"][si] = [(a + b) % (1 << 64) for a, b in zip(ver["checksum"][si], rec.checksum())]
        if probe_keys is not None and len(probe_keys):
            got = rec.query(np.asarray(probe_keys, dtype=np.uint64))
            ver["probe_found"][si] += int((got > 0).sum())
            if si == 0:
                ver["probe_count_out_of_range"] += int(((got > 0) & ((got < max(5, self.min_cov)) |
                                                                     (got > self.max_cov))).sum())

    def pos_of(self, keys: np.ndarray) -> np.ndarray:
        keys = np.asarray(keys, dtype=np.uint64)
        pos = np.zeros(len(keys), dtype=np.uint64)
        c = 2 * self.k
        for b in range(c):
            pos ^= np.where((keys >> np.uint64(b)) & np.uint64(1), self.cols[c - 1 - b], np.uint64(0))
        return pos & np.uint64((1 << self.lsize) - 1) if self.lsize < 64 else pos

    def _attempt(self, st, samples, keep_shard_records, verify, probe_keys, exclude, lap):
        self._drop_early()
        self._early_left = int(self.early_budget) if self.world == 1 and not keep_shard_records else 0
        self.replayed_blocks = self.binned_counts = self.maps_ahead = self.exchange_sent = self.exchange_received = 0
        self.count_wall_s = 0.0
        binned = verify == "binned" or (self._local() and not verify and not keep_shard_records and
                                        not os.environ.get("RFX_TRIO_SORTED"))
        candidates = _BinnedCandidates if binned else _SortedCandidates
        use_maps = self.map_budget > 0 and self.world == 1 and self.passes > 1 and not keep_shard_records
        if not use_maps:
            self._drop_store()
        elif self._store is None:
            try:
                self._store = capi.RunMaps(self.ctx, int(self.map_budget), pooled=True)
            except capi.RufusError:
                self.map_budget, use_maps = 0, False
        steps = plan_steps(self.passes, len(samples), use_maps, keep_shard_records)
        last_step = {sh: i for i, (sh, _) in enumerate(steps)}
        self._ahead = ({step: samples[si] for step, si in plan_maps_ahead(steps).items()}
                       if use_maps and os.environ.get("RFX_MAP_AHEAD") else {})
        for i_step, (sh, si) in enumerate(steps):
            t_c = time.perf_counter()
            rec, h = self.count_shard(samples[si], sh, si, binned)
            self.count_wall_s += time.perf_counter() - t_c
            st.recs[sh].append(rec)
            st.histos[si] += h
            st.n_rec[si] += len(rec)
            lap(f"pass {sh} sample {si} count ({len(rec)} records)")
            err = None
            try:
                if verify:
                    self._verify_store(st.ver, rec, si, probe_keys)
                    lap(f"pass {sh} sample {si} verify")
                if si == 0 and not keep_shard_records:
                    st.cands[sh] = candidates(self.ctx, st.recs[sh].pop(), max(5, self.min_cov), self.max_cov)
                    lap(f"pass {sh} sample {si} kept ({len(rec)})")
                elif not keep_shard_records:
                    cand = st.cands[sh]
                    room = cand.raw_bytes if self.passes == 2 and sh == 0 and self.early_budget > 0 else 0
                    cand.strike(rec)
                    self._early_left += room
                    st.recs[sh].pop().free()
                    lap(f"pass {sh} sample {si} candidates ({len(cand)})")
            except Exception as e:
                err = e
            self.checkpoint(err)
            if i_step != last_step[sh]:
                continue
            if keep_shard_records:
                recs = st.recs[sh]
                k_, c_ = capi.unique_to_subject(self.ctx, recs[0], recs[1:] + exclude, self.min_cov, self.max_cov)
                st.kept.append(st.recs.pop(sh))
            else:
                k_, c_ = st.cands[sh].finish(exclude)
                del st.cands[sh]
            lap(f"pass {sh} set difference ({len(k_)} k-mers)")
            st.keys.append(k_)
            st.kcounts.append(c_)

    def _gather(self, st):
        keys = np.concatenate(st.keys) if st.keys else np.zeros(0, np.uint64)
        kcounts = np.concatenate(st.kcounts).astype(np.uint32) if st.kcounts else np.zeros(0, np.uint32)
        if self.world == 1:
            return keys, kcounts, st.histos, st.n_rec
        import torch
        from .dist import all_gather_keys
        dev = torch.device("cuda", torch.cuda.current_device())
        kcounts = all_gather_keys(kcounts.astype(np.uint64), dev, self.group).astype(np.uint32)
        keys = all_gather_keys(keys, dev, self.group)
        histos = [x.astype(np.uint64) for x in self._group_sum(np.stack(st.histos))]
        return keys, kcounts, histos, self._group_sum(st.n_rec).tolist()

    def _group_sum(self, values) -> np.ndarray:
        values = np.asarray(values, dtype=np.int64)
        if self.world == 1:
            return values
        import torch
        import torch.distributed as dist
        from .dist import _wire
        t = _wire(torch.from_numpy(values).to(torch.device("cuda", torch.cuda.current_device())), self.group)
        dist.all_reduce(t, op=dist.ReduceOp.SUM, group=self.group)
        return t.cpu().numpy()

    def _filter(self, blocks, keys, pull: bool = False):
        n_pulled, masks, pulled = 0, [], None
        if len(keys) or pull:
            mset = capi.MutantSet(self.ctx, np.concatenate([keys, revcomp_keys(keys, self.k)]), self.k)
            try:
                if not len(keys):
                    pulled, res = mset.pull_many([], self.thresh, last_base_skipped=True, pairs=True)[0], []
                elif pull:
                    pulled, res = mset.pull_many(blocks, self.thresh, last_base_skipped=True, pairs=True)
                else:
                    res = mset.filter_many(blocks, self.thresh, last_base_skipped=True)
                for b, (mask, _) in zip(blocks, res):
                    n_pulled += pulled_pairs(mask, b.n)
                    masks.append(mask if self.masks_are_views else mask.copy())
            finally:
                mset.free()
        return n_pulled, masks, pulled

    def run(self, samples, keep_shard_records: bool = False, verify=False, probe_keys=None, exclude=(), pull: bool = False):
        if verify == "binned" and (not self._local() or keep_shard_records):
            raise ValueError('verify="binned": one device, no kept shard records')
        trace = os.environ.get("RFX_WGS_TRACE")
        t_last = time.perf_counter()
# ... 168 lines not shown
```

Baseline: 1.109 billion reads/s.

## Fuse subject strike into control leaf count kernel

```diff
diff --git a/include/rufus_hip.h b/include/rufus_hip.h
--- a/include/rufus_hip.h
+++ b/include/rufus_hip.h
@@ -212,6 +212,7 @@
 void rfx_binned_free(rfx_binned*);
 rfx_candidates* rfx_binned_strike(rfx_ctx*, rfx_binned* subject, const rfx_binned* control, uint32_t min_count,
                                   uint32_t max_count);
+int rfx_ctx_announce_strike(rfx_ctx*, rfx_binned* subject);
 int rfx_candidates_strike(rfx_candidates*, const rfx_binned* control);
 uint64_t rfx_candidates_size(const rfx_candidates*);
 int rfx_candidates_get(const rfx_candidates*, uint64_t* keys_out);
diff --git a/profiles/summarize_pmc.py b/profiles/summarize_pmc.py
--- a/profiles/summarize_pmc.py
+++ b/profiles/summarize_pmc.py
@@ -9,7 +9,7 @@
 NOT_CHAIN = frozenset((
     "k_synth_reads", "k_copy16",
     "k_flag_absent", "k_flag_absent_tiled", "k_fa_bounds", "k_flag_gather", "k_flag_range", "k_flag_rank", "k_flag_present",
-    "k_compact_count", "k_compact_scatter", "k_scan_u64", "k_query", "k_strike_bins", "k_strike_cands",
+    "k_compact_count", "k_compact_scatter", "k_scan_u64", "k_query", "k_strike_bins", "k_strike_list", "k_strike_cands",
     "k_strike_query", "k_binned_sizes", "k_binned_scan", "k_binned_gather", "k_binned_checksum", "k_binned_verify", "k_binned_query",
     "k_filter", "k_filter_q", "k_filter_p", "k_filter_fast", "k_filter_big", "k_hits_mask", "k_mask_count", "k_set_bitmap",
     "k_set_bitmap_big", "k_set_bitmap_q", "k_set_bitmap_p",
diff --git a/rufus_amd/capi.py b/rufus_amd/capi.py
--- a/rufus_amd/capi.py
+++ b/rufus_amd/capi.py
@@ -54,6 +54,7 @@
     "rfx_binned_bits": (C.c_int, [C.c_void_p]),
     "rfx_binned_free": (None, [C.c_void_p]),
     "rfx_binned_strike": (C.c_void_p, [C.c_void_p, C.c_void_p, C.c_void_p, C.c_uint32, C.c_uint32]),
+    "rfx_ctx_announce_strike": (C.c_int, [C.c_void_p, C.c_void_p]),
     "rfx_candidates_strike": (C.c_int, [C.c_void_p, C.c_void_p]),
     "rfx_candidates_size": (C.c_uint64, [C.c_void_p]),
     "rfx_candidates_get": (C.c_int, [C.c_void_p, u64p]),
@@ -340,6 +341,16 @@
     def sync(self):
         _check(lib().rfx_sync(self._h), "rfx_sync")
 
+    @property
+    def strike_next(self):
+        return getattr(self, "_strike_next", None)
+
+    @strike_next.setter
+    def strike_next(self, subject):
+        _check(lib().rfx_ctx_announce_strike(self._h, subject._live() if subject is not None else None),
+               "rfx_ctx_announce_strike")
+        self._strike_next = subject
+
     def mem_stats(self) -> dict:
         u, pk, m = C.c_uint64(0), C.c_uint64(0), C.c_uint64(0)
         _check(lib().rfx_mem_stats(self._h, C.byref(u), C.byref(pk), C.byref(m)), "rfx_mem_stats")
@@ -760,7 +771,9 @@
 
     def finish_binned(self, lower: int = 0, upper: int = 2**64 - 1, want_histo: bool = False):
         h = np.zeros(HISTO_BINS, dtype=np.uint64) if want_histo else None
-        b = Binned(self.ctx, lib().rfx_count_finish_binned(self._h, lower, upper, _p(h, u64p)))
+        handle = lib().rfx_count_finish_binned(self._h, lower, upper, _p(h, u64p))
+        self.ctx._strike_next = None
+        b = Binned(self.ctx, handle)
         return (b, h) if want_histo else b
 
     def finish_begin(self, lower: int = 0, upper: int = 2**64 - 1, want_histo: bool = False):
@@ -874,6 +887,8 @@
     def free(self):
         if self._h:
             lib().rfx_binned_free(self._h)
+            if getattr(self.ctx, "_strike_next", None) is self:
+                self.ctx._strike_next = None
             self._h = None
 
 
diff --git a/rufus_amd/csrc/rfx_api.hip b/rufus_amd/csrc/rfx_api.hip
--- a/rufus_amd/csrc/rfx_api.hip
+++ b/rufus_amd/csrc/rfx_api.hip
@@ -1747,6 +1747,8 @@
   uint2* bin_at = nullptr;
   uint32_t bin_lo = 0, bin_hi = 0;
   int bin_bits = 0;
+  const rfxk::binned_view* strike_S = nullptr;
+  bool struck = false;
 };
 
 static uint64_t msp_surv_key(uint64_t lower, uint64_t kmers) { return (kmers >> 24) | ((uint64_t)(lower >= 2 ? 1 : 0) << 62); }
@@ -1935,6 +1937,20 @@
     if (src) { drop(); dfree(c, d_ptrs); leaf_stage_free(c, &stage); return src; }
   }
   if (f->binned) f->bstage = stage;
+  rfxk::leaf_strike* d_strike = nullptr;
+  f->struck = false;
+  if (f->binned && f->strike_S && f->strike_S->bin_at && f->strike_S->bits == to_bits) {
+    std::vector<rfxk::leaf_strike> hs(cut.size() - 1);
+    for (size_t ci = 0; ci + 1 < cut.size(); ++ci) {
+      hs[ci].S = *f->strike_S;
+      hs[ci].bin0 = cut[ci] * Ftot;
+    }
+    d_strike = (rfxk::leaf_strike*)dmalloc(c, hs.size() * sizeof(rfxk::leaf_strike));
+    if (!d_strike) { drop(); dfree(c, d_ptrs); return RFX_E_NOMEM; }
+    const hipError_t e = upload(c, d_strike, hs.data(), hs.size() * sizeof(rfxk::leaf_strike));
+    if (e != hipSuccess) { drop(); dfree(c, d_ptrs); dfree(c, d_strike); return hip_fail(e, "msp_leaf_refined"); }
+    f->struck = true;
+  }
   for (size_t ci = 0; ci + 1 < cut.size(); ++ci) {
     const uint32_t p0 = cut[ci], np = cut[ci + 1] - cut[ci];
     const size_t n2 = (size_t)np * Ftot;
@@ -2011,6 +2027,7 @@
     if (e != hipSuccess) {
       drop();
       dfree(c, d_ptrs);
+      dfree(c, d_strike);
       if (!f->binned) leaf_stage_free(c, &stage);
       return hip_fail(e, "msp_leaf_refined");
     }
@@ -2018,7 +2035,7 @@
                    sel_bits, 2 * t->k - 7, t->pos_lo, t->pos_hi, f->lower, f->upper, f->aw, f->ac, cur, (uint32_t)f->cap,
                    cur + ncur, cur + ncur + 1, cur + ncur + 2, geo, (const uint32_t* const*)(d + 2 * nleaf),
                    (const uint32_t*)ptrs[2 * nleaf], stage, (uint32_t)ci, std::min<uint32_t>(lgrid, (uint32_t)n2),
-                   f->binned ? f->bin_at + 2 * ((size_t)p0 * Ftot - f->bin_lo) : nullptr);
+                   f->binned ? f->bin_at + 2 * ((size_t)p0 * Ftot - f->bin_lo) : nullptr, d_strike ? d_strike + ci : nullptr);
   }
   if (getenv("RFX_STAGE_DEBUG")) {
     std::vector<uint32_t> more(cut.size(), 0);
@@ -2031,6 +2048,7 @@
   }
   drop();
   dfree(c, d_ptrs);
+  dfree(c, d_strike);
   if (!f->binned) leaf_stage_free(c, &stage);
   return RFX_OK;
 }
@@ -2772,7 +2790,10 @@
   uint32_t bin_lo = 0, bin_hi = 0;
   int bits = 0;
   uint64_t n = 0;
+  int shard = 0, n_shards = 1;
+  uint64_t id = 0, struck_by = 0;
 };
+static std::atomic<uint64_t> g_binned_serial{0};
 struct rfx_candidates {
   rfx_ctx* ctx = nullptr;
   int k = 0, bits = 0;
@@ -2810,6 +2831,13 @@
   if (!t) return nullptr;
   rfx_ctx* c = t->ctx;
   (void)hipSetDevice(c->device);
+  struct announced {
+    rfx_ctx* c;
+    rfx_binned* S;
+    explicit announced(rfx_ctx* ctx) : c(ctx), S(ctx->strike_next) {}
+    ~announced() { c->strike_next = nullptr; }
+  } ann(c);
+  const int t_shard = t->n_shards > 1 ? t->shard : 0, t_nshards = t->n_shards > 1 ? t->n_shards : 1;
   if (t->pend_error) {
     snprintf(g_err, sizeof g_err, "a deferred MSP re-partition failed (%s); the table is incomplete", rfx_strerror(t->pend_error));
     return nullptr;
@@ -2819,6 +2847,9 @@
     b->ctx = c;
     b->k = t->k;
     b->canonical = t->canonical;
+    b->shard = t_shard;
+    b->n_shards = t_nshards;
+    b->id = ++g_binned_serial;
     if (histo) memset(histo, 0, RFX_HISTO_BINS * 8);
     return b;
   }
@@ -2832,6 +2863,15 @@
   f.lower = lower;
   f.upper = upper;
   f.binned = true;
+  rfxk::binned_view ann_S;
+  {
+    const char* ev = getenv("RFX_STRIKE_FUSED");
+    if (ann.S && ann.S->ctx == c && ann.S->bin_at && ann.S->k == t->k && ann.S->canonical == t->canonical &&
+        ann.S->shard == t_shard && ann.S->n_shards == t_nshards && !(ev && atoi(ev) == 0)) {
+      ann_S = binned_view_of(ann.S);
+      f.strike_S = &ann_S;
+    }
+  }
   const uint32_t P1 = (uint32_t)rfxk::p1_bins();
   const size_t ncur = (size_t)P1 * rfxk::p1_cur_stride();
   const rfx_ord_cfg cfg0 = ord_cfg(t, 7);
@@ -2885,6 +2925,10 @@
     b->bin_hi = f.bin_hi;
     b->bits = f.bin_bits;
     b->n = total;
+    b->shard = t_shard;
+    b->n_shards = t_nshards;
+    b->id = ++g_binned_serial;
+    if (f.struck) ann.S->struck_by = b->id;
     f.bstage = rfxk::msp_stage{};
     f.bin_at = nullptr;
     msp_binned_drop(&f);
@@ -2903,11 +2947,18 @@
   return nullptr;
 }
 
+int rfx_ctx_announce_strike(rfx_ctx* c, rfx_binned* subject) {
+  if (!c || (subject && subject->ctx != c)) return RFX_E_INVAL;
+  c->strike_next = subject;
+  return RFX_OK;
+}
+
 uint64_t rfx_binned_size(const rfx_binned* b) { return b ? b->n : 0; }
 int rfx_binned_bits(const rfx_binned* b) { return b ? b->bits : 0; }
 void rfx_binned_free(rfx_binned* b) {
   if (!b) return;
   (void)hipSetDevice(b->ctx->device);
+  if (b->ctx->strike_next == b) b->ctx->strike_next = nullptr;
   leaf_stage_free(b->ctx, &b->st);
   dfree(b->ctx, b->bin_at);
   delete b;
@@ -2921,6 +2972,7 @@
   }
   (void)hipSetDevice(c->device);
   const rfxk::binned_view S = binned_view_of(subject), C = binned_view_of(control);
+  const bool listed = control && subject->struck_by != 0 && subject->struck_by == control->id;
   uint64_t cap = std::max<uint64_t>(1u << 16, subject->n / 256);
   if (!control) cap = std::max<uint64_t>(cap, subject->n / 4);
   for (int attempt = 0; attempt < 2; ++attempt) {
@@ -2934,7 +2986,11 @@
     hipError_t e = hipMemsetAsync(d_n, 0, 4, c->stream);
     uint32_t n = 0;
     if (e == hipSuccess) {
-      rfxk::strike_bins(c, S, C, min_count, max_count, keys, bins, counts, (uint32_t)cap, d_n);
+      if (listed)
+        rfxk::strike_list(c, subject->st, subject->k, subject->canonical, subject->bits, min_count, max_count, keys, bins, counts,
+                          (uint32_t)cap, d_n);
+      else
+        rfxk::strike_bins(c, S, C, min_count, max_count, keys, bins, counts, (uint32_t)cap, d_n);
       e = queue_read(c, &n, d_n, 4);
     }
     if (e == hipSuccess) e = ctx_sync(c);
diff --git a/rufus_amd/csrc/rfx_internal.h b/rufus_amd/csrc/rfx_internal.h
--- a/rufus_amd/csrc/rfx_internal.h
+++ b/rufus_amd/csrc/rfx_internal.h
@@ -56,6 +56,7 @@
   std::vector<struct rfx_table*> pend_tables;
   double msp_surv_frac[2] = {0, 0};
   std::map<uint64_t, double> msp_surv_by_size;
+  struct rfx_binned* strike_next = nullptr;
   char* pin = nullptr;
   size_t pin_cap = 0, pin_used = 0;
   uint8_t* load_pin[3] = {nullptr, nullptr, nullptr};
@@ -393,6 +394,7 @@
   uint32_t* more = nullptr;
   uint32_t chunk = 0, n_chunks = 0;
 };
+struct leaf_strike;
 void msp_leaf(rfx_ctx*, const uint64_t* const* seg_inst, const uint64_t* const* seg_bs, int nseg,
               const uint64_t* inst0, const uint64_t* bs0, uint32_t P, int k, int canonical, const uint64_t* lut,
               int ntab, int sel_bits, int shift1, uint64_t pos_lo, uint64_t pos_hi, uint64_t lower, uint64_t upper,
@@ -401,7 +403,8 @@
               int geo ,
               const uint32_t* const* seg_ext, const uint32_t* ext0 , const msp_stage& st,
               uint32_t launch , uint32_t grid ,
-              uint2* bin_at = nullptr );
+              uint2* bin_at = nullptr ,
+              const leaf_strike* d_strike = nullptr );
 struct binned_view {
   const uint64_t* keys = nullptr;
   uint32_t* counts = nullptr;
@@ -410,6 +413,12 @@
   uint32_t chunk = 0, n_chunks = 0, bin_lo = 0, bin_hi = 0;
   int bits = 0;
 };
+struct leaf_strike {
+  binned_view S;
+  uint32_t bin0 = 0;
+};
+void strike_list(rfx_ctx*, const msp_stage&, int k, int canonical, int bits, uint32_t lo, uint32_t hi, uint64_t* out_k,
+                 uint32_t* out_b, uint32_t* out_c, uint32_t cap, uint32_t* out_n);
 uint32_t msp_leaf_chunk_room(int geo, uint32_t chunk);
 uint32_t msp_leaf_chunk_kept(uint32_t chunk);
 void histo_staged(rfx_ctx*, const msp_stage&, unsigned long long* d_histo, unsigned long long* d_total);
diff --git a/rufus_amd/csrc/rfx_msp.hip b/rufus_amd/csrc/rfx_msp.hip
--- a/rufus_amd/csrc/rfx_msp.hip
+++ b/rufus_amd/csrc/rfx_msp.hip
@@ -777,14 +777,34 @@
 constexpr unsigned long long MSP_RK_MUL = 0x9E3779B97F4A7C15ull;
 constexpr uint32_t MSP_RC_UNLISTED = 0x80000000u;
 
-template <bool CANON, int GEO>
+__device__ __forceinline__ uint4 binned_marks(const rfxk::binned_view& v, uint32_t gbin) {
+  if (!v.bin_at || gbin < v.bin_lo || gbin >= v.bin_hi) return make_uint4(~0u, ~0u, ~0u, ~0u);
+  return reinterpret_cast<const uint4*>(v.bin_at)[gbin - v.bin_lo];
+}
+template <class F>
+__device__ __forceinline__ void binned_segments(const rfxk::binned_view& v, const uint4 m, F&& fn) {
+  const uint2 a = make_uint2(m.x, m.y), e = make_uint2(m.z, m.w);
+  if (e.x >= v.n_chunks) return;
+  uint32_t ch = a.x, o = a.y;
+  for (uint32_t hops = 0; hops <= v.n_chunks && ch < v.n_chunks; ++hops) {
+    const bool last = ch == e.x;
+    const uint32_t end = min(last ? e.y : v.fill[ch], v.chunk);
+    if (end > o) fn((size_t)ch * v.chunk, o, end);
+    if (last) break;
+    ch = v.fill[v.n_chunks + ch];
+    o = 0;
+  }
+}
+
+template <bool CANON, int GEO, bool STRIKE>
 __global__ __launch_bounds__(MSP_LEAF_BLK(GEO)) __attribute__((amdgpu_waves_per_eu(MSP_LEAF_WPE(GEO), MSP_LEAF_WPE(GEO)))) void k_msp_leaf(
     const uint64_t* const* __restrict__ seg_inst, const uint64_t* const* __restrict__ seg_bs, int nseg,
     const uint64_t* __restrict__ inst0, const uint64_t* __restrict__ bs0, const uint32_t* const* __restrict__ seg_ext,
     const uint32_t* __restrict__ ext0, uint32_t P, int k, uint64_t lower, uint64_t upper,
     uint64_t* __restrict__ stage_k, uint32_t* __restrict__ stage_c, uint32_t CH, uint32_t* __restrict__ stage_fill,
     uint32_t* __restrict__ stage_more, uint32_t n_chunks, unsigned int* __restrict__ flag, unsigned int* __restrict__ err,
-    unsigned int* __restrict__ stage_short, int force_mixed, uint2* __restrict__ bin_at) {
+    unsigned int* __restrict__ stage_short, int force_mixed, uint2* __restrict__ bin_at,
+    const rfxk::leaf_strike* __restrict__ strike) {
   constexpr int TBL_LOG2 = GEO ? 12 : 13, TBL = 1 << TBL_LOG2, BLK = (int)MSP_LEAF_BLK(GEO), FILL = TBL * 3 / 4;
   static_assert(MSP_LEAF_PASS_MAX(GEO) >= (uint32_t)(FILL + BLK) && FILL + BLK <= TBL, "what a pass can leave behind fits the chunk and the table");
   constexpr int RC_LOG2 = TBL_LOG2 - (GEO ? RFX_RC_SHRINK : 2), RC = 1 << RC_LOG2, KMAP = TBL;
@@ -802,6 +822,52 @@
   uint32_t prex[MSP_ILP];
   uint64_t pre_a = 0, pre_e = 0;
   uint64_t nx_a = blockIdx.x < P ? bs0[blockIdx.x] : 0, nx_e = blockIdx.x < P ? bs0[blockIdx.x + 1] : 0;
+  constexpr uint32_t SUB_WALK = ~0u;
+  rfxk::binned_view S;
+  uint32_t sub_bin0 = 0;
+  if (STRIKE) {
+    S = strike->S;
+    sub_bin0 = strike->bin0;
+  }
+  size_t sub_first = 0, nsub_first = 0;
+  uint32_t sub_n = 0, nsub_n = 0;
+  uint64_t sub_k = 0;
+  uint32_t sub_c = 0;
+  auto sub_marks = [&](uint32_t b) { return b < P ? binned_marks(S, sub_bin0 + b) : make_uint4(~0u, ~0u, ~0u, ~0u); };
+  auto sub_first_lane = [](uint4 m) {
+    m.x = __builtin_amdgcn_readfirstlane(m.x);
+    m.y = __builtin_amdgcn_readfirstlane(m.y);
+    m.z = __builtin_amdgcn_readfirstlane(m.z);
+    m.w = __builtin_amdgcn_readfirstlane(m.w);
+    return m;
+  };
+  uint4 sub_nx = STRIKE ? sub_marks(blockIdx.x) : make_uint4(~0u, ~0u, ~0u, ~0u);
+  auto sub_fetch = [&](uint32_t b_after) {
+    const uint4 m = sub_first_lane(sub_nx);
+    sub_nx = sub_marks(b_after);
+    sub_c = 0;
+    nsub_first = 0;
+    nsub_n = 0;
+    if (m.z < S.n_chunks) {
+      if (m.x == m.z) {
+        const uint32_t e = min(m.w, S.chunk);
+        if (e > m.y) {
+          nsub_first = (size_t)m.x * S.chunk + m.y;
+          nsub_n = e - m.y;
+          if (threadIdx.x < nsub_n) {
+            sub_c = S.counts[nsub_first + threadIdx.x];
+            sub_k = S.keys[nsub_first + threadIdx.x];
+          }
+        }
+      } else {
+        nsub_n = SUB_WALK;
+      }
+    }
+  };
+  auto sub_take = [&]() {
+    sub_first = nsub_first;
+    sub_n = nsub_n;
+  };
   auto prefetch = [&](uint32_t b) {
     if (b >= P) return;
     pre_a = nx_a;
@@ -818,6 +884,10 @@
     }
   };
   prefetch(blockIdx.x);
+  if (STRIKE) {
+    sub_fetch(blockIdx.x + gridDim.x);
+    sub_take();
+  }
   for (int i = threadIdx.x; i < TBL; i += BLK) {
     s_keys[i] = RFX_EMPTY;
     s_cnt[i] = 0;
@@ -855,6 +925,7 @@
   for (uint32_t bin = blockIdx.x; bin < P; bin += gridDim.x) {
     const uint64_t a0 = pre_a, e0 = pre_e;
     bool prefetched_next = false;
+    bool sub_mine = STRIKE;
     int r = 0;
     uint32_t j = 0;
     bool failed = false, nocache = false;
@@ -998,6 +1069,40 @@
       TMC(20, split);
       TMC(24, mixed);
       TMC(21, 1);
+      if (STRIKE) {
+        if (!ovf) {
+          auto held = [&](uint64_t key) -> bool {
+            const uint32_t hk = leaf_hash32(key);
+            uint32_t slot = hk >> (32 - TBL_LOG2);
+            const uint32_t step = ((hk >> 3) | 1u) & (TBL - 1);
+            for (;;) {
+              const unsigned long long v = s_keys[slot];
+              if (v == RFX_EMPTY) return false;
+              if (v == key) {
+                const uint32_t c = s_cnt[slot];
+                return c >= lower && c <= upper;
+              }
+              slot = (slot + step) & (TBL - 1);
+            }
+          };
+          if (sub_n != SUB_WALK) {
+            const size_t first = sub_first;
+            if (sub_mine && sub_c && held(sub_k)) S.counts[first + threadIdx.x] = 0;
+            for (uint32_t i = threadIdx.x + (sub_mine ? (uint32_t)BLK : 0u); i < sub_n; i += BLK)
+              if (S.counts[first + i] && held(S.keys[first + i])) S.counts[first + i] = 0;
+          } else {
+            binned_segments(S, sub_first_lane(sub_marks(bin)), [&](size_t first, uint32_t o, uint32_t e) {
+              for (uint32_t i = o + threadIdx.x; i < e; i += BLK)
+                if (S.counts[first + i] && held(S.keys[first + i])) S.counts[first + i] = 0;
+            });
+          }
+        }
+        if (sub_mine) {
+          sub_fetch(bin + 2 * gridDim.x);
+          sub_mine = false;
+        }
+        __syncthreads();
+      }
       uint64_t* const stk = stage_k + (size_t)s_chunk * CH;
       uint32_t* const stc = stage_c + (size_t)s_chunk * CH;
       for (int i = threadIdx.x; i < TBL; i += BLK) {
@@ -1066,6 +1171,7 @@
       bin_at[2 * (size_t)bin + 1] = at;
       bin_at[2 * ((size_t)bin + gridDim.x)] = at;
     }
+    if (STRIKE) sub_take();
   }
   if (threadIdx.x == 0) stage_fill[s_chunk] = used;
 }
@@ -1321,24 +1427,6 @@
 }
 
 
-__device__ __forceinline__ uint4 binned_marks(const rfxk::binned_view& v, uint32_t gbin) {
-  if (!v.bin_at || gbin < v.bin_lo || gbin >= v.bin_hi) return make_uint4(~0u, ~0u, ~0u, ~0u);
-  return reinterpret_cast<const uint4*>(v.bin_at)[gbin - v.bin_lo];
-}
-template <class F>
-__device__ __forceinline__ void binned_segments(const rfxk::binned_view& v, const uint4 m, F&& fn) {
-  const uint2 a = make_uint2(m.x, m.y), e = make_uint2(m.z, m.w);
-  if (e.x >= v.n_chunks) return;
-  uint32_t ch = a.x, o = a.y;
-  for (uint32_t hops = 0; hops <= v.n_chunks && ch < v.n_chunks; ++hops) {
-    const bool last = ch == e.x;
-    const uint32_t end = min(last ? e.y : v.fill[ch], v.chunk);
-    if (end > o) fn((size_t)ch * v.chunk, o, end);
-    if (last) break;
-    ch = v.fill[v.n_chunks + ch];
-    o = 0;
-  }
-}
 template <class F>
 __device__ __forceinline__ void binned_segments(const rfxk::binned_view& v, uint32_t gbin, F&& fn) {
   binned_segments(v, binned_marks(v, gbin), fn);
@@ -1500,6 +1588,34 @@
   if (threadIdx.x == 0 && total) atomicAdd(g_total, total);
 }
 
+constexpr int SL_BLK = 256, SL_ILP = 4;
+__global__ __launch_bounds__(SL_BLK) void k_strike_list(const uint64_t* __restrict__ keys, const uint32_t* __restrict__ counts,
+                                                        const uint32_t* __restrict__ fill, const uint32_t* __restrict__ more,
+                                                        uint32_t CH, uint32_t n_chunks, int k, int canon, int bits, uint32_t lo,
+                                                        uint32_t hi, uint64_t* __restrict__ out_k, uint32_t* __restrict__ out_b,
+                                                        uint32_t* __restrict__ out_c, uint32_t cap, uint32_t* __restrict__ out_n) {
+  const uint32_t n_used = min(*more, n_chunks);
+  for (uint32_t ch = blockIdx.x; ch < n_used; ch += gridDim.x) {
+    const uint32_t n = min(fill[ch], CH);
+    const uint32_t* const src = counts + (size_t)ch * CH;
+    const uint64_t* const srck = keys + (size_t)ch * CH;
+    for (uint32_t i0 = 0; i0 < n; i0 += SL_ILP * SL_BLK) {
+      uint32_t c[SL_ILP];
+#pragma unroll
+      for (int q = 0; q < SL_ILP; ++q) {
+        const uint32_t i = i0 + q * SL_BLK + threadIdx.x;
+        c[q] = i < n ? src[i] : 0u;
+      }
+#pragma unroll
+      for (int q = 0; q < SL_ILP; ++q) {
+        const bool surv = c[q] != 0 && c[q] >= lo && c[q] <= hi;
+        if (!__ballot(surv)) continue;
+        const uint64_t key = surv ? srck[i0 + q * SL_BLK + threadIdx.x] : 0ull;
+        cand_append(surv, key, surv ? msp_key_bin(key, k, canon != 0, bits) : 0u, c[q], out_k, out_b, out_c, cap, out_n);
+      }
+    }
+  }
+}
 
 
 __global__ __launch_bounds__(256) void k_binned_sizes(const rfxk::binned_view v, unsigned long long* __restrict__ sizes) {
@@ -1764,21 +1880,29 @@
               int ntab, int sel_bits, int shift1, uint64_t pos_lo, uint64_t pos_hi, uint64_t lower, uint64_t upper,
               uint64_t* out_w, uint32_t* out_c, uint32_t* cur, uint32_t cap, unsigned int* flag, unsigned int* err,
               unsigned int* stage_short, int geo, const uint32_t* const* seg_ext, const uint32_t* ext0, const msp_stage& st,
-              uint32_t launch, uint32_t grid, uint2* bin_at) {
+              uint32_t launch, uint32_t grid, uint2* bin_at, const leaf_strike* d_strike) {
   const int force_mixed = getenv("RFX_LEAF_FORCE_MIXED") != nullptr;
   uint32_t* const more = st.more + (bin_at ? 0u : launch);
   {
     rfx_span sp(c, "k_msp_leaf");
-#define RFX_MSP_LEAF(CANON, GEO)                                                                                        \
-  hipLaunchKernelGGL((k_msp_leaf<CANON, GEO>), dim3(grid), dim3(MSP_LEAF_BLK(GEO)), 0, c->stream, seg_inst, seg_bs, nseg, \
-                     inst0, bs0, seg_ext, ext0, P, k, lower, upper, st.keys, st.counts, st.chunk, st.fill, more,           \
-                     st.n_chunks, flag, err, stage_short, force_mixed, bin_at)
-    if (canonical) {
-      if (geo) RFX_MSP_LEAF(true, 1);
-      else RFX_MSP_LEAF(true, 0);
+#define RFX_MSP_LEAF(CANON, GEO, STRIKE)                                                                                    \
+  hipLaunchKernelGGL((k_msp_leaf<CANON, GEO, STRIKE>), dim3(grid), dim3(MSP_LEAF_BLK(GEO)), 0, c->stream, seg_inst, seg_bs, \
+                     nseg, inst0, bs0, seg_ext, ext0, P, k, lower, upper, st.keys, st.counts, st.chunk, st.fill, more,     \
+                     st.n_chunks, flag, err, stage_short, force_mixed, bin_at, d_strike)
+    if (d_strike) {
+      if (canonical) {
+        if (geo) RFX_MSP_LEAF(true, 1, true);
+        else RFX_MSP_LEAF(true, 0, true);
+      } else {
+        if (geo) RFX_MSP_LEAF(false, 1, true);
+        else RFX_MSP_LEAF(false, 0, true);
+      }
+    } else if (canonical) {
+      if (geo) RFX_MSP_LEAF(true, 1, false);
+      else RFX_MSP_LEAF(true, 0, false);
     } else {
-      if (geo) RFX_MSP_LEAF(false, 1);
-      else RFX_MSP_LEAF(false, 0);
+      if (geo) RFX_MSP_LEAF(false, 1, false);
+      else RFX_MSP_LEAF(false, 0, false);
     }
 #undef RFX_MSP_LEAF
   }
@@ -1810,6 +1934,15 @@
   const uint32_t grid = std::min<uint32_t>(u_hi - u_lo, (uint32_t)c->n_cu * 10);
   hipLaunchKernelGGL(k_strike_bins, dim3(grid), dim3(SB_BLK), 0, c->stream, S, C, ubits, u_lo, u_hi, lo, hi, out_k, out_b, out_c,
                      cap, out_n);
+}
+
+void strike_list(rfx_ctx* c, const msp_stage& st, int k, int canonical, int bits, uint32_t lo, uint32_t hi, uint64_t* out_k,
+                 uint32_t* out_b, uint32_t* out_c, uint32_t cap, uint32_t* out_n) {
+  if (!st.n_chunks) return;
+  rfx_span sp(c, "k_strike_list");
+  const uint32_t grid = std::max<uint32_t>(1, std::min<uint32_t>(st.n_chunks, (uint32_t)c->n_cu * 8));
+  hipLaunchKernelGGL(k_strike_list, dim3(grid), dim3(SL_BLK), 0, c->stream, st.keys, st.counts, st.fill, st.more, st.chunk,
+                     st.n_chunks, k, canonical, bits, lo, hi, out_k, out_b, out_c, cap, out_n);
 }
 
 void strike_cands(rfx_ctx* c, uint64_t* keys, const uint32_t* bins, uint32_t n, int bits, const binned_view& C) {
diff --git a/rufus_amd/wgs.py b/rufus_amd/wgs.py
--- a/rufus_amd/wgs.py
+++ b/rufus_amd/wgs.py
@@ -111,6 +111,10 @@
     @property
     def raw_bytes(self) -> int:
         return len(self._h) * self.entry_bytes if self._range else 0
+
+    @property
+    def raw_store(self):
+        return self._h if self._range else None
 
     def _becomes(self, struck):
         self._h.free()
@@ -527,7 +531,14 @@
                        if use_maps and os.environ.get("RFX_MAP_AHEAD") else {})
         for i_step, (sh, si) in enumerate(steps):
             t_c = time.perf_counter()
-            rec, h = self.count_shard(samples[si], sh, si, binned)
+            raw = st.cands[sh].raw_store if binned and self.world == 1 and si != 0 and sh in st.cands else None
+            if raw is not None:
+                self.ctx.strike_next = raw
+            try:
+                rec, h = self.count_shard(samples[si], sh, si, binned)
+            finally:
+                if raw is not None:
+                    self.ctx.strike_next = None
             self.count_wall_s += time.perf_counter() - t_c
             st.recs[sh].append(rec)
             st.histos[si] += h
```

New measurement: 1.116 billion reads/s, median of 6. Within noise of the previous version (+0.7%).
